# youssefg7/dl-sound-classification

Measured on AMD Instinct MI355X. Metric: training clips/sec (EnvNet-v2, ESC-50 shape), higher is better.
Workload: dtype bf16; 1 GPU; EnvNet-v2 train step (BC-mix, fwd, soft-CE, bwd, clip, Adam), ESC-50 shape; global_batch=256, per_gpu_batch=256, clip_samples=220500, parallelism=dp1, model=envnet_v2

## Files before the change

dl-sound-classification_amd/csrc/conv3w.hip:

```cpp
#include "common.h"

namespace {

typedef unsigned u32x4 __attribute__((ext_vector_type(4)));
typedef unsigned u32x2 __attribute__((ext_vector_type(2)));
typedef short s16x8 __attribute__((ext_vector_type(8)));

struct W3Args {
  const bf16* x;
  const bf16* dy;
  float* part;
  int n, h, wd, oh, ow, nseg;
  const bf16* ya;
  bf16* dyo;
  float* bpart;
  const float *gamma, *scale, *shift, *mean, *invstd, *dgamma, *dbeta;
  int64_t P;
};

__device__ __forceinline__ bf16x8 tr_frag(const char* p0, int stride) {
  const s16x4 lo = __builtin_amdgcn_ds_read_tr16_b64_v4i16((MIA_LDS s16x4*)(p0));
  const s16x4 hi = __builtin_amdgcn_ds_read_tr16_b64_v4i16((MIA_LDS s16x4*)(p0 + 4 * stride));
  const s16x8 c = {lo[0], lo[1], lo[2], lo[3], hi[0], hi[1], hi[2], hi[3]};
  return __builtin_bit_cast(bf16x8, c);
}

template <bool BN>
__global__ __launch_bounds__(256) void conv3_wgrad_kernel(W3Args g) {
  constexpr int ROWB = 80, CPYB = 704;
  __shared__ __attribute__((aligned(16))) char strip[4][4 * CPYB];
  __shared__ __attribute__((aligned(16))) char dyt[4][32 * 64];
  const int lane = threadIdx.x & 63, wv = threadIdx.x >> 6;
  const int gw = blockIdx.x * 4 + wv, nw = gridDim.x * 4;
  const int items = g.n * g.oh * g.nseg;
  char* sg = strip[wv];
  char* dt = dyt[wv];
  f32x16 acc[2];
#pragma unroll
  for (int i = 0; i < 16; ++i) { acc[0][i] = 0.f; acc[1][i] = 0.f; }

  struct Raw { u32x2 v[3]; u32x4 d[2]; u32x4 y[BN ? 2 : 1]; uint32_t ok; };
  __shared__ __attribute__((aligned(16))) float bnp[7][32];
  float bs1[8];
  if constexpr (BN) {
    if (threadIdx.x < 32) {
      const int c = threadIdx.x;
      const float invP = 1.f / (float)g.P;
      const float is = g.invstd[c];
      bnp[0][c] = g.scale[c];
      bnp[1][c] = g.shift[c];
      bnp[2][c] = (g.gamma ? g.gamma[c] : 1.f) * is;
      bnp[3][c] = g.mean[c];
      bnp[4][c] = is;
      bnp[5][c] = g.dbeta[c] * invP;
      bnp[6][c] = g.dgamma[c] * invP;
    }
#pragma unroll
    for (int i = 0; i < 8; ++i) bs1[i] = 0.f;
    __syncthreads();
  }
  auto load = [&](int it) __attribute__((always_inline)) {
    Raw R;
    it = it < items ? it : items - 1;
    const int seg = it % g.nseg, rest = it / g.nseg;
    const int oy = rest % g.oh, b = rest / g.oh;
    const int l = lane < 40 ? lane : lane - 40;
    const int r = l / 5, q = l % 5;
    const int col = seg * 32 + 8 * q;
    const bf16* src = g.x + ((int64_t)b * g.h + oy + r) * g.wd;
#pragma unroll
    for (int k = 0; k < 3; ++k) {
      const int c = col + 4 * k;
      R.v[k] = c + 4 <= g.wd ? *reinterpret_cast<const u32x2*>(src + c) : u32x2{0u, 0u};
    }
    const int64_t drow = ((int64_t)b * g.oh + oy) * g.ow * 32;
    R.ok = 0;
#pragma unroll
    for (int s = 0; s < 2; ++s) {
      const int qq = lane + 64 * s;
      const int px = seg * 32 + (qq >> 2);
      const int64_t off = drow + (int64_t)px * 32 + (qq & 3) * 8;
      R.d[s] = px < g.ow ? *reinterpret_cast<const u32x4*>(g.dy + off) : u32x4{0u, 0u, 0u, 0u};
      if constexpr (BN) R.y[s] = px < g.ow ? *reinterpret_cast<const u32x4*>(g.ya + off) : u32x4{0u, 0u, 0u, 0u};
      R.ok |= (uint32_t)(px < g.ow) << s;
    }
    (void)drow;
    return R;
  };
  const int i16 = lane & 15, gq = lane >> 4, h = lane >> 5;
  const int n = lane & 31;
  auto bn_chunk = [&](const Raw& R, int s, int it) __attribute__((always_inline)) -> u32x4 {
    if (!((R.ok >> s) & 1u)) return u32x4{0u, 0u, 0u, 0u};
    uint32_t o[4];
#pragma unroll
    for (int k = 0; k < 4; ++k) {
      const uint32_t dw = R.d[s][k], yw = R.y[s][k];
      float gv[2] = {__uint_as_float(dw << 16), __uint_as_float(dw & 0xffff0000u)};
      const float xv[2] = {__uint_as_float(yw << 16), __uint_as_float(yw & 0xffff0000u)};
#pragma unroll
      for (int j = 0; j < 2; ++j) {
        const int i = 2 * k + j, c = (lane & 3) * 8 + i;
        gv[j] = fmaf(xv[j], bnp[0][c], bnp[1][c]) > 0.f ? gv[j] : 0.f;
        gv[j] = bnp[2][c] * (gv[j] - bnp[5][c] - (xv[j] - bnp[3][c]) * bnp[4][c] * bnp[6][c]);
        bs1[i] += gv[j];
      }
      o[k] = pk_bf16(gv[0], gv[1]);
    }
    const int seg = it % g.nseg, rest = it / g.nseg;
    const int oy = rest % g.oh, b = rest / g.oh;
    const int qq = lane + 64 * s;
    const int px = seg * 32 + (qq >> 2);
    const u32x4 v = {o[0], o[1], o[2], o[3]};
    *reinterpret_cast<u32x4*>(g.dyo + (((int64_t)b * g.oh + oy) * g.ow + px) * 32 + (qq & 3) * 8) = v;
    return v;
  };
  auto run = [&](const Raw& R, int it) __attribute__((always_inline)) {
    u32x4 dv[2] = {R.d[0], R.d[1]};
    if constexpr (BN) {
      dv[0] = bn_chunk(R, 0, it);
      dv[1] = bn_chunk(R, 1, it);
    }
    wave_sync();
    if (lane < 40) {
      const int l = lane;
      const int r = l / 5, q = l % 5;
      const uint32_t d[6] = {R.v[0][0], R.v[0][1], R.v[1][0], R.v[1][1], R.v[2][0], R.v[2][1]};
#pragma unroll
      for (int c = 0; c < 4; ++c) {
        uint32_t o[4];
#pragma unroll
        for (int i = 0; i < 4; ++i) {
          const int e = c + 2 * i;
          o[i] = (e & 1) ? ((d[e >> 1] >> 16) | (d[(e >> 1) + 1] << 16)) : d[e >> 1];
        }
        *reinterpret_cast<u32x4*>(sg + c * CPYB + r * ROWB + 16 * q) = u32x4{o[0], o[1], o[2], o[3]};
      }
    }
#pragma unroll
    for (int s = 0; s < 2; ++s) {
      const int qq = lane + 64 * s;
      *reinterpret_cast<u32x4*>(dt + (qq >> 2) * 64 + (qq & 3) * 16) = dv[s];
    }
    wave_sync();
    const int kx = n & 7, cp = kx & 3;
#pragma unroll
    for (int ks = 0; ks < 2; ++ks) {
      const int kr = ks * 16 + 8 * (gq >> 1) + (i16 >> 2);
      const int c4 = 16 * (gq & 1) + 4 * (i16 & 3);
      const bf16x8 fa = tr_frag(dt + kr * 64 + c4 * 2, 64);
#pragma unroll
      for (int nt = 0; nt < 2; ++nt) {
        const int ky = 4 * nt + (n >> 3);
        const char* src = sg + cp * CPYB + ky * ROWB + 2 * (16 * ks + 8 * h + (kx & 4));
        const u32x2 p0 = *reinterpret_cast<const u32x2*>(src);
        const u32x2 p1 = *reinterpret_cast<const u32x2*>(src + 8);
        const u32x4 f = {p0[0], p0[1], p1[0], p1[1]};
        acc[nt] = __builtin_amdgcn_mfma_f32_32x32x16_bf16(fa, __builtin_bit_cast(bf16x8, f), acc[nt], 0, 0, 0);
      }
    }
  };

  int it = gw;
  if (it < items) {
    Raw ra = load(it), rb;
    for (;;) {
      rb = load(it + nw);
      run(ra, it);
      it += nw;
      if (it >= items) break;
      ra = load(it + nw);
      run(rb, it);
      it += nw;
      if (it >= items) break;
    }
  }
  float* dst = g.part + (int64_t)gw * 2048;
#pragma unroll
  for (int nt = 0; nt < 2; ++nt)
#pragma unroll
    for (int r = 0; r < 16; ++r) {
      const int co = (r & 3) + 8 * (r >> 2) + 4 * h;
      dst[co * 64 + nt * 32 + n] = acc[nt][r];
    }
  if constexpr (BN) {
#pragma unroll
    for (int i = 0; i < 8; ++i)
#pragma unroll
      for (int m = 4; m < 64; m <<= 1) bs1[i] += __shfl_xor(bs1[i], m, 64);
    if (lane < 4) {
#pragma unroll
      for (int i = 0; i < 8; ++i) g.bpart[(int64_t)gw * 32 + lane * 8 + i] = bs1[i];
    }
  }
}

__global__ void conv3_bias_final_kernel(const float* __restrict__ bpart, int nw, float* __restrict__ dbias) {
  const double s = block_sum_strided(bpart + blockIdx.x, nw, 32);
  if (threadIdx.x == 0) dbias[blockIdx.x] = (float)s;
}

constexpr int C3_G = 64;
__global__ __launch_bounds__(256) void conv3_wgrad_reduce1_kernel(const float* __restrict__ part, int nslab,
                                                                  double* __restrict__ tmp) {
  const int e = blockIdx.x * 256 + threadIdx.x, gi = blockIdx.y;
  const int per = (nslab + C3_G - 1) / C3_G;
  const int w0 = gi * per, w1 = min(nslab, w0 + per);
  double s = 0.0;
  for (int w = w0; w < w1; ++w) s += (double)part[(int64_t)w * 2048 + e];
  tmp[gi * 2048 + e] = s;
}
__global__ __launch_bounds__(256) void conv3_wgrad_reduce2_kernel(const double* __restrict__ tmp, float* __restrict__ dw) {
  const int e = blockIdx.x * 256 + threadIdx.x;
  double s = 0.0;
#pragma unroll 8
  for (int g = 0; g < C3_G; ++g) s += tmp[g * 2048 + e];
  dw[e] = (float)s;
}

}

extern "C" int mia_conv3_wgrad(const void* x, const void* dy, float* dw, float* part, int32_t nwaves, int32_t n,
                               int32_t h, int32_t wd, mia_stream_t stream) {
  MIA_CHECK_ARG(x && dy && dw && part && n > 0 && h >= 8 && wd >= 8, "conv3_wgrad: bad arguments");
  MIA_CHECK_ARG(nwaves > 0 && nwaves % 4 == 0, "conv3_wgrad: nwaves must be a positive multiple of 4");
  MIA_CHECK_ARG(wd % 4 == 0, "conv3_wgrad: image width must be a multiple of 4 (8-byte row alignment)");
  MIA_CHECK_ARG((reinterpret_cast<uintptr_t>(dy) & 15) == 0 && (reinterpret_cast<uintptr_t>(x) & 7) == 0,
                "conv3_wgrad: dy must be 16-byte and x 8-byte aligned");
  W3Args a{reinterpret_cast<const bf16*>(x), reinterpret_cast<const bf16*>(dy), part, n, h, wd, h - 7, wd - 7,
           (int)cdiv(wd - 7, 32)};
  MIA_CHECK_ARG((int64_t)n * a.oh * a.nseg < (1ll << 31), "conv3_wgrad: too many items");
  hipStream_t s = as_stream(stream);
  conv3_wgrad_kernel<false><<<nwaves / 4, 256, 0, s>>>(a);
  MIA_LAUNCH_CHECK("conv3_wgrad");
  double* tmp = reinterpret_cast<double*>(part + (int64_t)nwaves * 2048);
  conv3_wgrad_reduce1_kernel<<<dim3(8, C3_G), 256, 0, s>>>(part, nwaves, tmp);
  conv3_wgrad_reduce2_kernel<<<8, 256, 0, s>>>(tmp, dw);
  MIA_LAUNCH_CHECK("conv3_wgrad_reduce");
  return 0;
}

extern "C" int64_t mia_conv3_wgrad_workspace_bytes(int32_t nwaves) {
  return (int64_t)nwaves * 2048 * 4 + (int64_t)C3_G * 2048 * 8 + (int64_t)nwaves * 32 * 4;
}

extern "C" int mia_conv3_wgrad_bn(const void* x, const void* da, const void* ya, void* dy, float* dw, float* dbias,
                                  float* part, int32_t nwaves, int32_t n, int32_t h, int32_t wd, const float* gamma,
                                  const float* scale, const float* shift, const float* mean, const float* invstd,
                                  const float* dgamma, const float* dbeta, mia_stream_t stream) {
  MIA_CHECK_ARG(x && da && ya && dy && dw && dbias && part && n > 0 && h >= 8 && wd >= 8,
                "conv3_wgrad_bn: bad arguments");
  MIA_CHECK_ARG(scale && shift && mean && invstd && dgamma && dbeta, "conv3_wgrad_bn: null BN statistics");
  MIA_CHECK_ARG(nwaves > 0 && nwaves % 4 == 0, "conv3_wgrad_bn: nwaves must be a positive multiple of 4");
  MIA_CHECK_ARG(wd % 4 == 0, "conv3_wgrad_bn: image width must be a multiple of 4 (8-byte row alignment)");
  MIA_CHECK_ARG(((reinterpret_cast<uintptr_t>(da) | reinterpret_cast<uintptr_t>(ya) | reinterpret_cast<uintptr_t>(dy)) &
                 15) == 0 && (reinterpret_cast<uintptr_t>(x) & 7) == 0,
                "conv3_wgrad_bn: da / ya / dy must be 16-byte and x 8-byte aligned");
  W3Args a{reinterpret_cast<const bf16*>(x), reinterpret_cast<const bf16*>(da), part, n, h, wd, h - 7, wd - 7,
           (int)cdiv(wd - 7, 32), reinterpret_cast<const bf16*>(ya), reinterpret_cast<bf16*>(dy), nullptr,
           gamma, scale, shift, mean, invstd, dgamma, dbeta, (int64_t)n * (h - 7) * (wd - 7)};
  MIA_CHECK_ARG((int64_t)n * a.oh * a.nseg < (1ll << 31), "conv3_wgrad_bn: too many items");
  double* tmp = reinterpret_cast<double*>(part + (int64_t)nwaves * 2048);
  a.bpart = reinterpret_cast<float*>(tmp + (int64_t)C3_G * 2048);
  hipStream_t s = as_stream(stream);
  conv3_wgrad_kernel<true><<<nwaves / 4, 256, 0, s>>>(a);
  MIA_LAUNCH_CHECK("conv3_wgrad_bn");
  conv3_wgrad_reduce1_kernel<<<dim3(8, C3_G), 256, 0, s>>>(part, nwaves, tmp);
  conv3_wgrad_reduce2_kernel<<<8, 256, 0, s>>>(tmp, dw);
  conv3_bias_final_kernel<<<32, 256, 0, s>>>(a.bpart, nwaves, dbias);
  MIA_LAUNCH_CHECK("conv3_wgrad_bn reduce");
  return 0;
}
```

dl-sound-classification_amd/csrc/feconv.hip:

```cpp
#include "common.h"

#include <type_traits>

namespace {

constexpr int F1_DEPTH = 4;
constexpr int FE_NT = 256;
constexpr int FE_BM = 128;
constexpr int FE_N = 64;

typedef unsigned u32x4 __attribute__((ext_vector_type(4)));

template <int CIN, int KW, int S>
struct FeCfg {
  static constexpr int CG = CIN / 8;
  static constexpr int WPX = (FE_BM - 1) * S + KW;
  static constexpr int HALF = (WPX + 1) / 2;
  static constexpr int NSLOT = S == 1 ? WPX : 2 * HALF;
  static constexpr int PSB = CIN * 2 + 16;
  static constexpr int WBYTES = NSLOT * PSB;
  static constexpr int NCH = WPX * CG;
  static constexpr int LCH = (NCH + FE_NT - 1) / FE_NT;
  static constexpr int KS = KW * CIN / 16;
  static_assert(FE_NT % CG == 0, "channel chunk must be constant per thread");
// ... 624 lines not shown
      }
    const int seg = it % g.nseg, rest = it / g.nseg;
    const int oy = rest % g.oh, b = rest / g.oh;
    const int ox0 = seg * 32, ox = ox0 + o;
    char* stg = stage[wv];
#pragma unroll
    for (int h = 0; h < 2; ++h) {
      uint32_t w4[4];
#pragma unroll
      for (int i = 0; i < 4; ++i) {
        const int e = 8 * h + 2 * i;
        w4[i] = pk_bf16(v[e] + bv[e], v[e + 1] + bv[e + 1]);
        if constexpr (STATS) {
          if (ox < g.ow) {
            const float d0 = __uint_as_float(w4[i] << 16) - bv[e], d1 = __uint_as_float(w4[i] & 0xffff0000u) - bv[e + 1];
            s1[e] += d0; s2[e] = fmaf(d0, d0, s2[e]);
            s1[e + 1] += d1; s2[e + 1] = fmaf(d1, d1, s2[e + 1]);
          }
        }
      }
      const int k = (lane >> 5) + 2 * h;
      *reinterpret_cast<u32x4*>(stg + o * 64 + ((k ^ ((o >> 1) & 3)) << 4)) = u32x4{w4[0], w4[1], w4[2], w4[3]};
    }
    wave_sync();
    bf16* yrow = g.y + (((int64_t)b * g.oh + oy) * g.ow + ox0) * 32;
#pragma unroll
    for (int h = 0; h < 2; ++h) {
      const int r = 16 * h + (lane >> 2), k = lane & 3;
      const u32x4 q = *reinterpret_cast<const u32x4*>(stg + r * 64 + ((k ^ ((r >> 1) & 3)) << 4));
      if (ox0 + r < g.ow) __builtin_nontemporal_store(q, reinterpret_cast<u32x4*>(yrow + r * 32 + 8 * k));
    }
  };

  int it = gw;
  if (it < items) {
    Raw ra = load(it), rb;
    for (;;) {
      rb = load(it + nw);
      run(it, ra);
      it += nw;
      if (it >= items) break;
      ra = load(it + nw);
      run(it, rb);
      it += nw;
      if (it >= items) break;
    }
  }
  if constexpr (STATS) {
#pragma unroll
    for (int i = 0; i < 16; ++i) {
#pragma unroll
      for (int m = 1; m < 32; m <<= 1) {
        s1[i] += __shfl_xor(s1[i], m, 64);
        s2[i] += __shfl_xor(s2[i], m, 64);
      }
    }
    if ((lane & 31) == 0) {
      float* dst = g.part + (int64_t)gw * 64;
#pragma unroll
      for (int i = 0; i < 8; ++i) {
        dst[(c0 + i) * 2] = s1[i];
        dst[(c0 + i) * 2 + 1] = s2[i];
        dst[(c0 + 16 + i) * 2] = s1[8 + i];
        dst[(c0 + 16 + i) * 2 + 1] = s2[8 + i];
      }
    }
  }
}

constexpr int FW_NT = 512;
constexpr int FW_BP = 128;

struct FwArgs {
  const bf16* dy;
  const bf16* x;
  const float* ps;
  const float* pt;
  int n, win, wout, nitem;
  float* ws;
};

typedef short s16x8 __attribute__((ext_vector_type(8)));

__device__ __forceinline__ bf16x8 fw_tr(const char* p0, int stride) {
  const s16x4 lo = __builtin_amdgcn_ds_read_tr16_b64_v4i16((MIA_LDS s16x4*)(p0));
  const s16x4 hi = __builtin_amdgcn_ds_read_tr16_b64_v4i16((MIA_LDS s16x4*)(p0 + 4 * stride));
  const s16x8 c = {lo[0], lo[1], lo[2], lo[3], hi[0], hi[1], hi[2], hi[3]};
  return __builtin_bit_cast(bf16x8, c);
}

template <bool PRE>
__global__ __launch_bounds__(FW_NT) __attribute__((amdgpu_waves_per_eu(2, 2))) void fe_wgrad_kernel(FwArgs g) {
  constexpr int C = 32, KW = 16;
  constexpr int WPX = (FW_BP - 1) * 2 + KW;
  constexpr int HALF = (WPX + 1) / 2;
  constexpr int PSB = 64;
  constexpr int DSB = 192;
  constexpr int WBY = 2 * HALF * PSB;
  constexpr int DBY = FW_BP * DSB;
  constexpr int BUF = WBY + DBY;
  constexpr int WCH = WPX * 4;
  constexpr int WL = (WCH + FW_NT - 1) / FW_NT;
  constexpr int DL = FW_BP * 8 / FW_NT;
  __shared__ __attribute__((aligned(16))) char smem[2 * BUF];
  __shared__ __attribute__((aligned(16))) float spre[2][C];
  const int t = threadIdx.x, lane = t & 63, wave = t >> 6;
  const int items = g.n * g.nitem;
  if (PRE && t < C) {
    spre[0][t] = g.ps[t];
    spre[1][t] = g.pt[t];
  }
  const int cgw = t & 3;
  const __amdgpu_buffer_rsrc_t xr = __builtin_amdgcn_make_buffer_rsrc(
      const_cast<bf16*>(g.x), (short)0, (int)((int64_t)g.n * g.win * C * 2), 0x00020000);
  const __amdgpu_buffer_rsrc_t dr = __builtin_amdgcn_make_buffer_rsrc(
      const_cast<bf16*>(g.dy), (short)0, (int)((int64_t)g.n * g.wout * 64 * 2), 0x00020000);

  u32x4 wa[WL], wb[WL], da[DL], db[DL];
  auto load = [&](int it, u32x4 (&w)[WL], u32x4 (&d)[DL]) __attribute__((always_inline)) {
    it = it < items ? it : items - 1;
    const int b = it / g.nitem;
    const int o0 = (it - b * g.nitem) * FW_BP;
#pragma unroll
    for (int s = 0; s < WL; ++s) {
      const int q = t + FW_NT * s;
      const int p = q >> 2;
      const int ix = 2 * o0 + p;
      const bool ok = q < WCH && ix < g.win;
      const unsigned off = ok ? (unsigned)((b * g.win + ix) * 4 + cgw) * 16u : 0x80000000u;
      w[s] = __builtin_bit_cast(u32x4, __builtin_amdgcn_raw_buffer_load_b128(xr, off, 0, 0));
    }
#pragma unroll
    for (int s = 0; s < DL; ++s) {
      const int q = t + FW_NT * s;
      const int p = q >> 3, cc = q & 7;
      const bool ok = o0 + p < g.wout;
      const unsigned off = ok ? (unsigned)((b * g.wout + o0 + p) * 8 + cc) * 16u : 0x80000000u;
      d[s] = __builtin_bit_cast(u32x4, __builtin_amdgcn_raw_buffer_load_b128(dr, off, 0, 0));
    }
  };
  auto store = [&](int it, int buf, const u32x4 (&w)[WL], const u32x4 (&d)[DL]) __attribute__((always_inline)) {
    it = it < items ? it : items - 1;
    const int b = it / g.nitem;
    const int o0 = (it - b * g.nitem) * FW_BP;
    char* win = smem + buf * BUF;
    char* dyt = win + WBY;
    float sc[8], sh[8];
    if constexpr (PRE) {
#pragma unroll
      for (int h = 0; h < 2; ++h) {
        const f32x4 a = *reinterpret_cast<const f32x4*>(&spre[0][cgw * 8 + 4 * h]);
        const f32x4 c = *reinterpret_cast<const f32x4*>(&spre[1][cgw * 8 + 4 * h]);
#pragma unroll
        for (int q = 0; q < 4; ++q) { sc[4 * h + q] = a[q]; sh[4 * h + q] = c[q]; }
      }
    }
#pragma unroll
    for (int s = 0; s < WL; ++s) {
      const int q = t + FW_NT * s;
      const int p = q >> 2;
      if (q < WCH) {
        u32x4 v = w[s];
        if constexpr (PRE) {
          if (2 * o0 + p < g.win) {
            uint32_t w4[4];
#pragma unroll
            for (int i = 0; i < 4; ++i) {
              const float lo = fmaxf(fmaf(__uint_as_float(v[i] << 16), sc[2 * i], sh[2 * i]), 0.f);
              const float hi = fmaxf(fmaf(__uint_as_float(v[i] & 0xffff0000u), sc[2 * i + 1], sh[2 * i + 1]), 0.f);
              w4[i] = pk_bf16(lo, hi);
            }
            v = u32x4{w4[0], w4[1], w4[2], w4[3]};
          }
        }
        const int slot = (p & 1) * HALF + (p >> 1);
        *reinterpret_cast<u32x4*>(win + slot * PSB + cgw * 16) = v;
      }
    }
#pragma unroll
    for (int s = 0; s < DL; ++s) {
      const int q = t + FW_NT * s;
      *reinterpret_cast<u32x4*>(dyt + (q >> 3) * DSB + (q & 7) * 16) = d[s];
    }
  };

  f32x16 acc[2][2];
#pragma unroll
  for (int i = 0; i < 2; ++i)
#pragma unroll
    for (int j = 0; j < 2; ++j)
#pragma unroll
      for (int r = 0; r < 16; ++r) acc[i][j][r] = 0.f;

  const int i16 = lane & 15, gq = lane >> 4;
  auto compute = [&](int buf) __attribute__((always_inline)) {
    const char* win = smem + buf * BUF;
    const char* dyt = win + WBY;
    constexpr int KS = FW_BP / 16;
    auto frags = [&](int ks, bf16x8 (&fa)[2], bf16x8 (&fb)[2]) __attribute__((always_inline)) {
      const int kr = ks * 16 + 8 * (gq >> 1) + (i16 >> 2);
#pragma unroll
      for (int mt = 0; mt < 2; ++mt)
        fa[mt] = fw_tr(dyt + kr * DSB + (mt * 32 + 16 * (gq & 1) + 4 * (i16 & 3)) * 2, DSB);
#pragma unroll
      for (int j = 0; j < 2; ++j) {
        const int kx = 2 * wave + j;
        const int ci = 16 * (gq & 1) + 4 * (i16 & 3);
        const int slot = (kx & 1) * HALF + kr + (kx >> 1);
        fb[j] = fw_tr(win + slot * PSB + ci * 2, PSB);
      }
    };
    bf16x8 fa[2][2], fb[2][2];
    frags(0, fa[0], fb[0]);
#pragma unroll
    for (int ks = 0; ks < KS; ++ks) {
      const int c = ks & 1;
      if (ks + 1 < KS) frags(ks + 1, fa[c ^ 1], fb[c ^ 1]);
#pragma unroll
      for (int mt = 0; mt < 2; ++mt)
#pragma unroll
        for (int j = 0; j < 2; ++j)
          acc[mt][j] = __builtin_amdgcn_mfma_f32_32x32x16_bf16(fa[c][mt], fb[c][j], acc[mt][j], 0, 0, 0);
    }
    __builtin_amdgcn_sched_group_barrier(0x100, 8, 0);
#pragma unroll
    for (int ks = 0; ks < KS; ++ks) {
      if (ks + 1 < KS) {
#pragma unroll
        for (int q = 0; q < 4; ++q) {
          __builtin_amdgcn_sched_group_barrier(0x008, 1, 0);
          __builtin_amdgcn_sched_group_barrier(0x100, 2, 0);
        }
      } else {
        __builtin_amdgcn_sched_group_barrier(0x008, 4, 0);
      }
    }
  };

  const int G = gridDim.x;
  int item = blockIdx.x;
  if (item < items) {
    load(item, wa, da);
    load(item + G, wb, db);
    __syncthreads();
    store(item, 0, wa, da);
    __syncthreads();
    for (;;) {
      load(item + 2 * G, wa, da);
      compute(0);
      store(item + G, 1, wb, db);
      __builtin_amdgcn_s_waitcnt(0xC07F);
      __builtin_amdgcn_s_barrier();
      item += G;
      if (item >= items) break;
      load(item + 2 * G, wb, db);
      compute(1);
      store(item + G, 0, wa, da);
      __builtin_amdgcn_s_waitcnt(0xC07F);
      __builtin_amdgcn_s_barrier();
      item += G;
      if (item >= items) break;
    }
  }
  float* dst = g.ws + (int64_t)blockIdx.x * 64 * 512;
#pragma unroll
  for (int mt = 0; mt < 2; ++mt)
#pragma unroll
    for (int j = 0; j < 2; ++j) {
      const int n = (2 * wave + j) * 32 + (lane & 31);
#pragma unroll
      for (int r = 0; r < 16; ++r) {
        const int m = mt * 32 + (r & 3) + 8 * (r >> 2) + 4 * (lane >> 5);
        dst[(int64_t)m * 512 + n] = acc[mt][j][r];
      }
    }
}

int fe_grid(int items) {
  static int ncu = 0;
  if (!ncu) {
    int dev = 0;
    if (hipGetDevice(&dev) != hipSuccess || hipDeviceGetAttribute(&ncu, hipDeviceAttributeMultiprocessorCount, dev) != hipSuccess)
      ncu = 256;
  }
  return items < 2 * ncu ? items : 2 * ncu;
}

int fe_clips_per_launch(int64_t clip_bytes) { return (int)(((1ll << 31) - 1) / clip_bytes); }

int fe_grid1(int items) {
  const int two = fe_grid(1 << 30);
  return items < two / 2 ? items : two / 2;
}

__global__ __launch_bounds__(256) void fw_reduce_kernel(const float* __restrict__ ws, int slabs, int len,
                                                        float* __restrict__ out) {
  const int e = blockIdx.x * 256 + threadIdx.x;
  if (e >= len) return;
  float acc = 0.f;
  for (int k = 0; k < slabs; ++k) acc += ws[(int64_t)k * len + e];
  out[e] = acc;
}

bool aligned16(const void* p) { return (reinterpret_cast<uintptr_t>(p) & 15) == 0; }

bool fe_ws() { const char* e = getenv("MIA_FECONV_WS"); return !(e && e[0] == '0'); }

}

extern "C" int mia_fe_conv2_fwd(const void* y1, const float* scale, const float* shift, const void* w,
                                const float* bias, void* y2, int32_t n, int32_t w1, int32_t w2,
                                mia_stream_t stream) {
  MIA_CHECK_ARG(y1 && w && y2 && n > 0 && w1 >= 16, "fe_conv2_fwd: bad arguments");
  MIA_CHECK_ARG(!scale == !shift, "fe_conv2_fwd: scale and shift go together");
  MIA_CHECK_ARG(w2 == (w1 - 16) / 2 + 1, "fe_conv2_fwd: w2 must be (w1-16)/2+1 (got w1=%d w2=%d)", w1, w2);
  MIA_CHECK_ARG(aligned16(y1) && aligned16(w) && aligned16(y2), "fe_conv2_fwd: operands must be 16-byte aligned");
  hipStream_t s = as_stream(stream);
  const int per = fe_clips_per_launch((int64_t)w1 * 32 * 2);
  MIA_CHECK_ARG(per > 0, "fe_conv2_fwd: one clip exceeds 2 GB");
  for (int c = 0; c < n; c += per) {
    const int nc = n - c < per ? n - c : per;
    FeArgs a{reinterpret_cast<const bf16*>(y1) + (int64_t)c * w1 * 32, scale, shift, reinterpret_cast<const bf16*>(w),
             bias, reinterpret_cast<bf16*>(y2) + (int64_t)c * w2 * FE_N, nc, w1, w2, 0, (int)cdiv(w2, FE_BM),
             (int64_t)w2 * FE_N, (int64_t)w2 * FE_N};
    if (fe_ws()) {
      const int grid = fe_grid1(nc * a.nitem);
      if (scale) feconv_ws_kernel<32, 16, 2, true><<<grid, FS_NT, 0, s>>>(a);
      else feconv_ws_kernel<32, 16, 2, false><<<grid, FS_NT, 0, s>>>(a);
    } else {
      const int grid = fe_grid(nc * a.nitem);
      if (scale) feconv_kernel<32, 16, 2, true><<<grid, FE_NT, 0, s>>>(a);
      else feconv_kernel<32, 16, 2, false><<<grid, FE_NT, 0, s>>>(a);
    }
    MIA_LAUNCH_CHECK("fe_conv2_fwd");
  }
  return 0;
}

extern "C" int mia_fe_conv2_dgrad(const void* dy2, const void* wpar, void* da1, int32_t n, int32_t w1,
                                  int32_t w2, mia_stream_t stream) {
  MIA_CHECK_ARG(dy2 && wpar && da1 && n > 0 && w1 >= 16, "fe_conv2_dgrad: bad arguments");
  MIA_CHECK_ARG(w2 == (w1 - 16) / 2 + 1, "fe_conv2_dgrad: w2 must be (w1-16)/2+1 (got w1=%d w2=%d)", w1, w2);
  MIA_CHECK_ARG(aligned16(dy2) && aligned16(wpar) && aligned16(da1), "fe_conv2_dgrad: operands must be 16-byte aligned");
  MIA_CHECK_ARG(((int64_t)w1 * 32) % 8 == 0, "fe_conv2_dgrad: clip stride must keep 16-byte alignment");
  const int wout = (w1 + 1) / 2;
  const int per = fe_clips_per_launch((int64_t)w2 * 64 * 2);
  MIA_CHECK_ARG(per > 0, "fe_conv2_dgrad: one clip exceeds 2 GB");
  for (int c = 0; c < n; c += per) {
    const int nc = n - c < per ? n - c : per;
    FeArgs a{reinterpret_cast<const bf16*>(dy2) + (int64_t)c * w2 * 64, nullptr, nullptr,
             reinterpret_cast<const bf16*>(wpar), nullptr, reinterpret_cast<bf16*>(da1) + (int64_t)c * w1 * 32, nc,
             w2, wout, 7, (int)cdiv(wout, FE_BM), (int64_t)w1 * 32, (int64_t)w1 * 32};
#ifdef FS_DGRAD
    feconv_ws_kernel<64, 8, 1, false><<<fe_grid1(nc * a.nitem), FS_NT, 0, as_stream(stream)>>>(a);
#else
    feconv_kernel<64, 8, 1, false><<<fe_grid(nc * a.nitem), FE_NT, 0, as_stream(stream)>>>(a);
#endif
    MIA_LAUNCH_CHECK("fe_conv2_dgrad");
  }
  return 0;
}

extern "C" int mia_fe_conv2_wgrad(const void* dy2, const void* y1, const float* scale, const float* shift,
                                  float* dw, int32_t n, int32_t w1, int32_t w2, void* workspace, int64_t ws_bytes,
                                  mia_stream_t stream) {
  MIA_CHECK_ARG(dy2 && y1 && dw && workspace && n > 0 && w1 >= 16, "fe_conv2_wgrad: bad arguments");
  MIA_CHECK_ARG(!scale == !shift, "fe_conv2_wgrad: scale and shift go together");
  MIA_CHECK_ARG(w2 == (w1 - 16) / 2 + 1, "fe_conv2_wgrad: w2 must be (w1-16)/2+1 (got w1=%d w2=%d)", w1, w2);
  MIA_CHECK_ARG(aligned16(dy2) && aligned16(y1), "fe_conv2_wgrad: operands must be 16-byte aligned");
  hipStream_t s = as_stream(stream);
  const int per = fe_clips_per_launch((int64_t)w1 * 32 * 2);
  MIA_CHECK_ARG(per > 0, "fe_conv2_wgrad: one clip exceeds 2 GB");
  const int nitem = (int)cdiv(w2, FW_BP);
  int slabs = 0;
  for (int c = 0; c < n; c += per) slabs += fe_grid1(((n - c) < per ? (n - c) : per) * nitem);
  MIA_CHECK_ARG((int64_t)slabs * 64 * 512 * 4 <= ws_bytes, "fe_conv2_wgrad: workspace too small (%lld B needed)",
                (long long)slabs * 64 * 512 * 4);
  int slab0 = 0;
  for (int c = 0; c < n; c += per) {
    const int nc = n - c < per ? n - c : per;
    FwArgs a{reinterpret_cast<const bf16*>(dy2) + (int64_t)c * w2 * 64, reinterpret_cast<const bf16*>(y1) + (int64_t)c * w1 * 32,
             scale, shift, nc, w1, w2, nitem, reinterpret_cast<float*>(workspace) + (int64_t)slab0 * 64 * 512};
    const int grid = fe_grid1(nc * nitem);
    if (scale) fe_wgrad_kernel<true><<<grid, FW_NT, 0, s>>>(a);
    else fe_wgrad_kernel<false><<<grid, FW_NT, 0, s>>>(a);
    MIA_LAUNCH_CHECK("fe_conv2_wgrad");
    slab0 += grid;
  }
  fw_reduce_kernel<<<64 * 512 / 256, 256, 0, s>>>(reinterpret_cast<const float*>(workspace), slabs, 64 * 512, dw);
  MIA_LAUNCH_CHECK("fe_conv2_wgrad reduce");
  return 0;
}

extern "C" int mia_fe_conv1_fwd(const float* x, const void* w, const float* bias, void* y1, float* partial,
                                int32_t nwaves, int32_t n, int32_t t, mia_stream_t stream) {
  MIA_CHECK_ARG(x && w && bias && y1 && n > 0 && t >= 64 && t % 2 == 0, "fe_conv1_fwd: bad arguments");
  MIA_CHECK_ARG(nwaves > 0 && nwaves % 4 == 0, "fe_conv1_fwd: nwaves must be a positive multiple of 4");
  MIA_CHECK_ARG(aligned16(w) && aligned16(y1) && (reinterpret_cast<uintptr_t>(x) & 7) == 0,
                "fe_conv1_fwd: y1/w must be 16-byte and x 8-byte aligned");
  const int w1 = (t - 64) / 2 + 1;
  F1Args a{x, reinterpret_cast<const bf16*>(w), bias, reinterpret_cast<bf16*>(y1), partial, n, t, w1,
           (int)cdiv(w1, 32)};
  MIA_CHECK_ARG((int64_t)n * a.nitem < (1ll << 31), "fe_conv1_fwd: too many items");
  if (partial) fe_conv1_kernel<true><<<nwaves / 4, 256, 0, as_stream(stream)>>>(a);
  else fe_conv1_kernel<false><<<nwaves / 4, 256, 0, as_stream(stream)>>>(a);
  MIA_LAUNCH_CHECK("fe_conv1_fwd");
  return 0;
}

extern "C" int mia_fe_conv3_fwd(const void* x, const void* w, const float* bias, void* y, float* partial,
                                int32_t nwaves, int32_t n, int32_t h, int32_t wd, mia_stream_t stream) {
  MIA_CHECK_ARG(x && w && bias && y && n > 0 && h >= 8 && wd >= 8, "fe_conv3_fwd: bad arguments");
  MIA_CHECK_ARG(nwaves > 0 && nwaves % 4 == 0, "fe_conv3_fwd: nwaves must be a positive multiple of 4");
  MIA_CHECK_ARG(wd % 4 == 0, "fe_conv3_fwd: image width must be a multiple of 4 (8-byte row alignment)");
  MIA_CHECK_ARG(aligned16(w) && aligned16(y) && (reinterpret_cast<uintptr_t>(x) & 7) == 0,
                "fe_conv3_fwd: w/y must be 16-byte and x 8-byte aligned");
  F3Args a{reinterpret_cast<const bf16*>(x), reinterpret_cast<const bf16*>(w), bias, reinterpret_cast<bf16*>(y),
           partial, n, h, wd, h - 7, wd - 7, (int)cdiv(wd - 7, 32)};
  MIA_CHECK_ARG((int64_t)n * a.oh * a.nseg < (1ll << 31), "fe_conv3_fwd: too many items");
  if (partial) fe_conv3_kernel<true><<<nwaves / 4, 256, 0, as_stream(stream)>>>(a);
  else fe_conv3_kernel<false><<<nwaves / 4, 256, 0, as_stream(stream)>>>(a);
  MIA_LAUNCH_CHECK("fe_conv3_fwd");
  return 0;
}

#ifdef FE_STAMP
extern "C" int mia_fe_stamps_copy(void* dst, int64_t bytes) {
  return hipMemcpyFromSymbol(dst, HIP_SYMBOL(g_fe_st), (size_t)bytes, 0, hipMemcpyDeviceToHost) == hipSuccess ? 0 : -1;
}
#endif
```

dl-sound-classification_amd/csrc/mgemm.hip:

```cpp
#include "common.h"
#include "gemm_common.h"

namespace {

constexpr int MG_NT = 512;
constexpr int MG_BM = 256, MG_BN = 256, MG_BK = 64;
constexpr int MG_HALF = 16384;
constexpr int MG_STAGE = 4 * MG_HALF;
constexpr int MG_LDS = 2 * MG_STAGE;

enum { MG_KC = MIA_LAYOUT_KC, MG_RC = MIA_LAYOUT_RC };
enum { EPI_PLAIN = 0, EPI_GELU = 1, EPI_GELU_SAVE = 2, EPI_ADD_AUX = 3, EPI_DGELU = 4, EPI_SLAB = 5, EPI_GELU_SAVE_D = 6,
       EPI_DMUL = 7 };

typedef short s16x8 __attribute__((ext_vector_type(8)));
typedef __attribute__((address_space(3))) void* lds_vp;

struct MArgs {
  const bf16* a;
  const bf16* b;
  int64_t lda, ldb, M, N, K, kper;
  int nbm, nbn, split;
  void* out;
  int64_t ldc;
  int out_f32;
  const float* bias;
  const void* aux;
  int64_t ldaux;
  float* ws;
  float* colsum_part;
  float* acs_part;
  uint8_t* mxq;
  uint8_t* mxs;
  int64_t drop_w;
  int group_m;
};

typedef unsigned mg_u32x4 __attribute__((ext_vector_type(4)));
__device__ __forceinline__ void mg_st16(void* p, uint4 v) {
  __builtin_nontemporal_store(__builtin_bit_cast(mg_u32x4, v), reinterpret_cast<mg_u32x4*>(p));
}

__device__ __forceinline__ __amdgpu_buffer_rsrc_t rsrc_of(const void* base, int64_t bytes) {
  const uint32_t n = bytes <= 0 ? 0u : (bytes >= 0xFFFFFFFFll ? 0xFFFFFFFFu : (uint32_t)bytes);
  return __builtin_amdgcn_make_buffer_rsrc(const_cast<void*>(base), 0, (int)n, 0x00020000);
}

__device__ __forceinline__ int rc_swz(int k) { return (k & 3) | (((k >> 3) & 1) << 2); }

template <int L>
struct Loader {
  __amdgpu_buffer_rsrc_t rsrc;
  uint32_t voff[4];
  uint32_t kstep;
  __device__ __forceinline__ void init(const bf16* p, int64_t ld, int64_t rows, int64_t r0, int64_t kbeg,
                                       int64_t kend, int wave, int lane) {
    if constexpr (L == MG_KC) {
      const bf16* base = p + r0 * ld + kbeg;
      const int64_t nrows = rows - r0 < 256 ? rows - r0 : 256;
      rsrc = rsrc_of(base, ((nrows - 1) * ld + (kend - kbeg)) * 2);
#pragma unroll
      for (int i = 0; i < 4; ++i) {
        const int hh = i >> 1, j = 2 * wave + (i & 1);
        const int r = hh * 128 + 8 * j + (lane >> 3);
        const int c = (lane & 7) ^ (r & 7);
        voff[i] = (uint32_t)(((int64_t)r * ld + c * 8) * 2);
      }
      kstep = 128;
    } else {
      const bf16* base = p + kbeg * ld + r0;
      const int64_t ncols = rows - r0 < 256 ? rows - r0 : 256;
      rsrc = rsrc_of(base, ((kend - kbeg - 1) * ld + ncols) * 2);
#pragma unroll
      for (int i = 0; i < 4; ++i) {
        const int hh = i >> 1, j = 2 * wave + (i & 1);
        const int k = 4 * j + (lane >> 4);
        const int s = lane & 15;
        const int c = (s >> 1) ^ rc_swz(k);
        voff[i] = (uint32_t)(((int64_t)k * ld + hh * 128 + c * 16 + (s & 1) * 8) * 2);
      }
      kstep = (uint32_t)(64 * ld * 2);
    }
  }
  __device__ __forceinline__ void issue(char* tile, int kt, int wave) const {
#pragma unroll
    for (int i = 0; i < 4; ++i)
      __builtin_amdgcn_raw_ptr_buffer_load_lds(rsrc, (lds_vp)(tile + (i >> 1) * MG_HALF + (2 * wave + (i & 1)) * 1024),
                                               16, voff[i], kt * kstep, 0, 0);
  }
};

template <int L>
__device__ __forceinline__ bf16x8 frag(const char* half, int r0, int ks, int lane) {
  if constexpr (L == MG_KC) {
    const int r = r0 + (lane & 15);
    const int c = 4 * ks + (lane >> 4);
    return *reinterpret_cast<const bf16x8*>(half + r * 128 + ((c ^ (r & 7)) << 4));
  } else {
    const int i = lane & 15, g = lane >> 4;
    const int k = 32 * ks + 8 * g + (i >> 2);
    const int ch = r0 >> 4;
    const char* p0 = half + k * 256 + ((ch ^ rc_swz(k)) << 5) + (i & 3) * 8;
    const char* p1 = half + (k + 4) * 256 + ((ch ^ rc_swz(k + 4)) << 5) + (i & 3) * 8;
    const s16x4 lo = __builtin_amdgcn_ds_read_tr16_b64_v4i16((MIA_LDS s16x4*)(p0));
    const s16x4 hi = __builtin_amdgcn_ds_read_tr16_b64_v4i16((MIA_LDS s16x4*)(p1));
    const s16x8 cc = {lo[0], lo[1], lo[2], lo[3], hi[0], hi[1], hi[2], hi[3]};
    return __builtin_bit_cast(bf16x8, cc);
  }
}

__device__ __forceinline__ f32x4 mfma_t(bf16x8 a, bf16x8 b, f32x4 c) {
  return __builtin_amdgcn_mfma_f32_16x16x32_bf16(b, a, c, 0, 0, 0);
}

__device__ __forceinline__ float gelu_cdf(float x) {
  const float z = fabsf(x) * 0.70710678118654752f;
  const float t = __builtin_amdgcn_rcpf(fmaf(0.5f, z, 1.f));
  float p = 0.17087277f;
  p = fmaf(p, t, -0.82215223f);
  p = fmaf(p, t, 1.48851587f);
  p = fmaf(p, t, -1.13520398f);
  p = fmaf(p, t, 0.27886807f);
  p = fmaf(p, t, -0.18628806f);
  p = fmaf(p, t, 0.09678418f);
  p = fmaf(p, t, 0.37409196f);
  p = fmaf(p, t, 1.00002368f);
  p = fmaf(p, t, -1.26551223f);
  const float half_erfc = 0.5f * t * __expf(fmaf(-z, z, p));
  return x >= 0.f ? 1.f - half_erfc : half_erfc;
}
__device__ __forceinline__ float gelu_f(float x) { return x * gelu_cdf(x); }
__device__ __forceinline__ float gelu_grad_f(float x) {
  return fmaf(x * 0.39894228040143268f, __expf(-0.5f * x * x), gelu_cdf(x));
}

typedef float f2 __attribute__((ext_vector_type(2)));
__device__ __forceinline__ f2 pfma(f2 a, f2 b, f2 c) { return __builtin_elementwise_fma(a, b, c); }
constexpr float L2E = 1.4426950408889634f;
__device__ __forceinline__ f2 gelu_cdf2(f2 x, f2& zz) {
  const f2 z = __builtin_elementwise_abs(x) * 0.70710678118654752f;
  const f2 d = pfma(z, f2{0.5f, 0.5f}, f2{1.f, 1.f});
  const f2 t = {__builtin_amdgcn_rcpf(d.x), __builtin_amdgcn_rcpf(d.y)};
  f2 p = f2{0.17087277f * L2E, 0.17087277f * L2E};
  p = pfma(p, t, f2{-0.82215223f * L2E, -0.82215223f * L2E});
  p = pfma(p, t, f2{1.48851587f * L2E, 1.48851587f * L2E});
  p = pfma(p, t, f2{-1.13520398f * L2E, -1.13520398f * L2E});
  p = pfma(p, t, f2{0.27886807f * L2E, 0.27886807f * L2E});
  p = pfma(p, t, f2{-0.18628806f * L2E, -0.18628806f * L2E});
  p = pfma(p, t, f2{0.09678418f * L2E, 0.09678418f * L2E});
  p = pfma(p, t, f2{0.37409196f * L2E, 0.37409196f * L2E});
  p = pfma(p, t, f2{1.00002368f * L2E, 1.00002368f * L2E});
  p = pfma(p, t, f2{-1.26551223f * L2E, -1.26551223f * L2E});
  zz = z * z;
  const f2 a = pfma(-zz, f2{L2E, L2E}, p);
  const f2 he = t * f2{0.5f * __builtin_amdgcn_exp2f(a.x), 0.5f * __builtin_amdgcn_exp2f(a.y)};
  return f2{x.x >= 0.f ? 1.f - he.x : he.x, x.y >= 0.f ? 1.f - he.y : he.y};
}
__device__ __forceinline__ f2 gelu2(f2 x) {
  f2 zz;
  return x * gelu_cdf2(x, zz);
}
__device__ __forceinline__ f2 gelu_grad2(f2 x) {
  const f2 z = __builtin_elementwise_abs(x) * 0.70710678118654752f;
  const f2 d = pfma(z, f2{0.3275911f, 0.3275911f}, f2{1.f, 1.f});
  const f2 t = {__builtin_amdgcn_rcpf(d.x), __builtin_amdgcn_rcpf(d.y)};
  f2 p = f2{0.5f * 1.061405429f, 0.5f * 1.061405429f};
  p = pfma(p, t, f2{0.5f * -1.453152027f, 0.5f * -1.453152027f});
  p = pfma(p, t, f2{0.5f * 1.421413741f, 0.5f * 1.421413741f});
  p = pfma(p, t, f2{0.5f * -0.284496736f, 0.5f * -0.284496736f});
  p = pfma(p, t, f2{0.5f * 0.254829592f, 0.5f * 0.254829592f});
  const f2 a = -(z * z) * L2E;
  const f2 e = {__builtin_amdgcn_exp2f(a.x), __builtin_amdgcn_exp2f(a.y)};
  const f2 he = p * t * e;
  const f2 c = {x.x >= 0.f ? 1.f - he.x : he.x, x.y >= 0.f ? 1.f - he.y : he.y};
  return pfma(x * 0.39894228040143268f, e, c);
}
__device__ __forceinline__ f2 gelu_and_grad2(f2 x, f2& d) {
  const f2 z = __builtin_elementwise_abs(x) * 0.70710678118654752f;
  const f2 dd = pfma(z, f2{0.3275911f, 0.3275911f}, f2{1.f, 1.f});
  const f2 t = {__builtin_amdgcn_rcpf(dd.x), __builtin_amdgcn_rcpf(dd.y)};
  f2 p = f2{0.5f * 1.061405429f, 0.5f * 1.061405429f};
  p = pfma(p, t, f2{0.5f * -1.453152027f, 0.5f * -1.453152027f});
  p = pfma(p, t, f2{0.5f * 1.421413741f, 0.5f * 1.421413741f});
  p = pfma(p, t, f2{0.5f * -0.284496736f, 0.5f * -0.284496736f});
  p = pfma(p, t, f2{0.5f * 0.254829592f, 0.5f * 0.254829592f});
  const f2 a = -(z * z) * L2E;
  const f2 e = {__builtin_amdgcn_exp2f(a.x), __builtin_amdgcn_exp2f(a.y)};
  const f2 he = p * t * e;
  const f2 c = {x.x >= 0.f ? 1.f - he.x : he.x, x.y >= 0.f ? 1.f - he.y : he.y};
  d = pfma(x * 0.39894228040143268f, e, c);
  return x * c;
}
__device__ __forceinline__ void gelu4(f32x4& v) {
  const f2 a = gelu2(f2{v[0], v[1]}), b = gelu2(f2{v[2], v[3]});
  v = f32x4{a.x, a.y, b.x, b.y};
}
__device__ __forceinline__ void gelu_d4(f32x4& v, f32x4& d) {
  f2 da, db;
  const f2 a = gelu_and_grad2(f2{v[0], v[1]}, da), b = gelu_and_grad2(f2{v[2], v[3]}, db);
  v = f32x4{a.x, a.y, b.x, b.y};
  d = f32x4{da.x, da.y, db.x, db.y};
}
__device__ __forceinline__ void dgelu4(f32x4& v, f32x4 u) {
  const f2 a = gelu_grad2(f2{u[0], u[1]}), b = gelu_grad2(f2{u[2], u[3]});
  v = f32x4{v[0] * a.x, v[1] * a.y, v[2] * b.x, v[3] * b.y};
}

__device__ __forceinline__ uint2 pack4(f32x4 v) {
  return make_uint2(pk_bf16(v[0], v[1]), pk_bf16(v[2], v[3]));
}
__device__ __forceinline__ f32x4 unpack4(uint2 u) {
  return f32x4{__uint_as_float(u.x << 16), __uint_as_float(u.x & 0xffff0000u), __uint_as_float(u.y << 16),
               __uint_as_float(u.y & 0xffff0000u)};
}

template <int EPI>
__device__ __forceinline__ void mg_epilogue(const MArgs& g, f32x4 (&acc)[8][4], char* smem, int wave, int lane,
                                            int bm, int z, int64_t m0, int64_t n0) {
  const int wr = wave >> 2, wc = wave & 3;
  f32x4 bias4[4];
#pragma unroll
  for (int j = 0; j < 4; ++j) {
    const int64_t n = n0 + wc * 64 + 16 * j + 4 * (lane >> 4);
    if (EPI != EPI_SLAB && EPI != EPI_DGELU && EPI != EPI_DMUL && g.bias && n < g.N)
      bias4[j] = *reinterpret_cast<const f32x4*>(g.bias + n);
    else
      bias4[j] = f32x4{0.f, 0.f, 0.f, 0.f};
  }
  constexpr bool DG = EPI == EPI_DGELU || EPI == EPI_DMUL;
  const bool bf_out = EPI == EPI_GELU || EPI == EPI_GELU_SAVE || EPI == EPI_GELU_SAVE_D || DG ||
                      (EPI == EPI_PLAIN && !g.out_f32);
  if (!bf_out) {
    f32x4 ax[8][4];
    auto ld_row = [&](int i) __attribute__((always_inline)) {
      const int64_t m = m0 + wr * 128 + 16 * i + (lane & 15);
#pragma unroll
      for (int j = 0; j < 4; ++j) {
        const int64_t n = n0 + wc * 64 + 16 * j + 4 * (lane >> 4);
        ax[i][j] = (m < g.M && n < g.N)
                       ? *reinterpret_cast<const f32x4*>(reinterpret_cast<const float*>(g.aux) + m * g.ldaux + n)
                       : f32x4{0.f, 0.f, 0.f, 0.f};
      }
    };
    if constexpr (EPI == EPI_ADD_AUX) {
      ld_row(0);
      ld_row(1);
    }
#pragma unroll
    for (int i = 0; i < 8; ++i) {
      if constexpr (EPI == EPI_ADD_AUX) {
        if (i + 2 < 8) ld_row(i + 2);
      }
      const int64_t m = m0 + wr * 128 + 16 * i + (lane & 15);
      if (m >= g.M) continue;
#pragma unroll
      for (int j = 0; j < 4; ++j) {
        const int64_t n = n0 + wc * 64 + 16 * j + 4 * (lane >> 4);
        if (n >= g.N) continue;
        f32x4 v = acc[i][j] + bias4[j];
        if constexpr (EPI == EPI_ADD_AUX) v += ax[i][j];
        float* dst = EPI == EPI_SLAB ? g.ws + ((int64_t)z * g.M + m) * g.N + n
                                     : reinterpret_cast<float*>(g.out) + m * g.ldc + n;
        *reinterpret_cast<f32x4*>(dst) = v;
      }
    }
    return;
  }
  if constexpr (EPI != EPI_SLAB && EPI != EPI_ADD_AUX) {
    __syncthreads();
    char* img = smem + wave * 16384;
    uint4 ua[16];
    if constexpr (DG) {
#pragma unroll
      for (int it = 0; it < 16; ++it) {
        const int r = 8 * it + (lane >> 3);
        const int64_t m = m0 + wr * 128 + r, n = n0 + wc * 64 + 8 * (lane & 7);
        ua[it] = (m < g.M && n < g.N)
                     ? __builtin_bit_cast(uint4, __builtin_nontemporal_load(reinterpret_cast<const mg_u32x4*>(
                           reinterpret_cast<const bf16*>(g.aux) + m * g.ldaux + n)))
                     : make_uint4(0, 0, 0, 0);
      }
    }
#pragma unroll
    for (int i = 0; i < 8; ++i)
#pragma unroll
      for (int j = 0; j < 4; ++j) {
        const int r = 16 * i + (lane & 15), g4 = lane >> 4;
        const int c = 2 * j + (g4 >> 1);
        *reinterpret_cast<uint2*>(img + r * 128 + ((c ^ (r & 7) ^ ((r >> 3) & 1)) << 4) + (g4 & 1) * 8) =
            pack4(acc[i][j] + bias4[j]);
      }
    asm volatile("s_waitcnt lgkmcnt(0)" ::: "memory");
    __builtin_amdgcn_sched_barrier(0);
    float cs[8];
#pragma unroll
    for (int c = 0; c < 8; ++c) cs[c] = 0.f;
    const int cc = lane & 7;
#pragma unroll
    for (int it = 0; it < 16; ++it) {
      const int r = 8 * it + (lane >> 3);
      const uint4 q = *reinterpret_cast<const uint4*>(img + r * 128 + ((cc ^ (r & 7) ^ ((r >> 3) & 1)) << 4));
      const int64_t m = m0 + wr * 128 + r, n = n0 + wc * 64 + 8 * cc;
// ... 167 lines not shown
    }
    if constexpr (ACS) {
#pragma unroll
      for (int ks = 0; ks < 2; ++ks) {
        acs0 = frag_sum(frag<LA>(ah, 16 * wc, ks, lane), acs0);
        acs1 = frag_sum(frag<LA>(ah, 64 + 16 * wc, ks, lane), acs1);
      }
    }
    if (t + 1 < nk) {
      la.issue((t & 1) ? st0 : st1, t + 1, wave);
      asm volatile("s_waitcnt vmcnt(4) lgkmcnt(0)" ::: "memory");
    } else {
      asm volatile("s_waitcnt vmcnt(0) lgkmcnt(0)" ::: "memory");
    }
    __builtin_amdgcn_sched_barrier(0);
    __builtin_amdgcn_s_barrier();
    __builtin_amdgcn_sched_barrier(0);
    __builtin_amdgcn_s_setprio(1);
#pragma unroll
    for (int ks = 0; ks < 2; ++ks)
#pragma unroll
      for (int i = 0; i < 4; ++i)
#pragma unroll
        for (int j = 0; j < 4; ++j) acc[i][j] = mfma_t(af[ks][i], bfr[ks][j], acc[i][j]);
    __builtin_amdgcn_s_setprio(0);
    __builtin_amdgcn_sched_barrier(0);
    __builtin_amdgcn_s_barrier();
    __builtin_amdgcn_sched_barrier(0);
#pragma unroll
    for (int ks = 0; ks < 2; ++ks)
#pragma unroll
      for (int i = 0; i < 4; ++i) af[ks][i] = frag<LA>(ah, 64 + 16 * i, ks, lane);
    if (t + 2 < nk) {
      lb.issue(const_cast<char*>(cur) + 2 * MG_HALF, t + 2, wave);
      asm volatile("s_waitcnt vmcnt(4) lgkmcnt(0)" ::: "memory");
    } else {
      asm volatile("s_waitcnt vmcnt(0) lgkmcnt(0)" ::: "memory");
    }
    __builtin_amdgcn_sched_barrier(0);
    __builtin_amdgcn_s_barrier();
    __builtin_amdgcn_sched_barrier(0);
    __builtin_amdgcn_s_setprio(1);
#pragma unroll
    for (int ks = 0; ks < 2; ++ks)
#pragma unroll
      for (int i = 0; i < 4; ++i)
#pragma unroll
        for (int j = 0; j < 4; ++j) acc[4 + i][j] = mfma_t(af[ks][i], bfr[ks][j], acc[4 + i][j]);
    __builtin_amdgcn_s_setprio(0);
    __builtin_amdgcn_sched_barrier(0);
    __builtin_amdgcn_s_barrier();
    __builtin_amdgcn_sched_barrier(0);
  }
  if (wr == 0) __builtin_amdgcn_s_barrier();
  if constexpr (ACS) {
    acs0 += __shfl_xor(acs0, 16, 64);
    acs0 += __shfl_xor(acs0, 32, 64);
    acs1 += __shfl_xor(acs1, 16, 64);
    acs1 += __shfl_xor(acs1, 32, 64);
    if (bn == 0 && lane < 16) {
      const int64_t m = m0 + wr * 128 + 16 * wc + lane;
      if (m < g.M) g.acs_part[(int64_t)z * g.M + m] = acs0;
      if (m + 64 < g.M) g.acs_part[(int64_t)z * g.M + m + 64] = acs1;
    }
  }
  mg_epilogue<EPI>(g, acc, smem, wave, lane, bm, z, m0, n0);
}

template __global__ void mgemm_kernel<0, 0, 0>(MArgs);
template __global__ void mgemm_kernel<0, 0, 1>(MArgs);
template __global__ void mgemm_kernel<0, 0, 2>(MArgs);
template __global__ void mgemm_kernel<0, 0, 3>(MArgs);
template __global__ void mgemm_kernel<0, 0, 4>(MArgs);
template __global__ void mgemm_kernel<0, 0, 5>(MArgs);
template __global__ void mgemm_kernel<0, 1, 0>(MArgs);
template __global__ void mgemm_kernel<0, 1, 1>(MArgs);
template __global__ void mgemm_kernel<0, 1, 2>(MArgs);
template __global__ void mgemm_kernel<0, 1, 3>(MArgs);
template __global__ void mgemm_kernel<0, 1, 4>(MArgs);
template __global__ void mgemm_kernel<0, 1, 5>(MArgs);
template __global__ void mgemm_kernel<1, 0, 0>(MArgs);
template __global__ void mgemm_kernel<1, 0, 1>(MArgs);
template __global__ void mgemm_kernel<1, 0, 2>(MArgs);
template __global__ void mgemm_kernel<1, 0, 3>(MArgs);
template __global__ void mgemm_kernel<1, 0, 4>(MArgs);
template __global__ void mgemm_kernel<1, 0, 5>(MArgs);
template __global__ void mgemm_kernel<1, 1, 0>(MArgs);
template __global__ void mgemm_kernel<1, 1, 1>(MArgs);
template __global__ void mgemm_kernel<1, 1, 2>(MArgs);
template __global__ void mgemm_kernel<1, 1, 3>(MArgs);
template __global__ void mgemm_kernel<1, 1, 4>(MArgs);
template __global__ void mgemm_kernel<1, 1, 5>(MArgs);
template __global__ void mgemm_kernel<1, 1, 5, true>(MArgs);
template __global__ void mgemm_kernel<1, 0, 5, true>(MArgs);
template __global__ void mgemm_kernel<1, 1, 0, true>(MArgs);
template __global__ void mgemm_kernel<1, 0, 0, true>(MArgs);

typedef int i32x8 __attribute__((ext_vector_type(8)));
typedef int i32x4v __attribute__((ext_vector_type(4)));
constexpr int MX_SC = MG_LDS;

struct MxArgs {
  const uint8_t* sa;
  const uint8_t* sb;
};

__device__ __forceinline__ i32x8 mx_frag(const char* half, int r0, int lane) {
  const int r = r0 + (lane & 15), g = lane >> 4;
  const i32x4v lo = *reinterpret_cast<const i32x4v*>(half + r * 128 + ((g ^ (r & 7)) << 4));
  const i32x4v hi = *reinterpret_cast<const i32x4v*>(half + r * 128 + (((4 + g) ^ (r & 7)) << 4));
  return i32x8{lo[0], lo[1], lo[2], lo[3], hi[0], hi[1], hi[2], hi[3]};
}
__device__ __forceinline__ int mx_scale(const char* sbuf, int r0, int lane) {
  return *reinterpret_cast<const uint8_t*>(sbuf + (r0 + (lane & 15)) * 4 + (lane >> 4));
}

template <int EPI>
__global__ __launch_bounds__(MG_NT, 2) void mxgemm_kernel(MArgs g, MxArgs x) {
  __shared__ __attribute__((aligned(1024))) char smem[MG_LDS + 4096];
  const int lane = threadIdx.x & 63;
  const int wave = __builtin_amdgcn_readfirstlane(threadIdx.x >> 6);
  const int wr = wave >> 2, wc = wave & 3;
  const int nwg = (int)gridDim.x;
  const int orig = blockIdx.x;
  const int xcd = orig & 7, q8 = nwg >> 3, r8 = nwg & 7;
  const int lid = (xcd < r8 ? xcd * (q8 + 1) : r8 * (q8 + 1) + (xcd - r8) * q8) + (orig >> 3);
  int bm, bn;
  mg_tile_of(g, lid, bm, bn);
  const int64_t m0 = (int64_t)bm * MG_BM, n0 = (int64_t)bn * MG_BN;
  const int nk = (int)(g.K >> 7);
  Loader<MG_KC> la, lb;
  la.init(g.a, g.lda, g.M, m0, 0, g.K >> 1, wave, lane);
  lb.init(g.b, g.ldb, g.N, n0, 0, g.K >> 1, wave, lane);
  const int64_t kb32 = g.K >> 5;
  const int srow = 64 * (wave & 3) + lane;
  const uint8_t* sbase = wr == 0 ? x.sa + m0 * kb32 : x.sb + n0 * kb32;
  const int64_t srows = wr == 0 ? g.M - m0 : g.N - n0;
  const __amdgpu_buffer_rsrc_t srsrc = rsrc_of(sbase, (srows < 256 ? srows : 256) * kb32);
  const uint32_t svoff = (uint32_t)(srow * kb32);
  char* const sdst0 = smem + MX_SC + wr * 1024 + (wave & 3) * 256;
  auto sissue = [&](int kt) __attribute__((always_inline)) {
    __builtin_amdgcn_raw_ptr_buffer_load_lds(srsrc, (lds_vp)(sdst0 + (kt & 1) * 2048), 4, svoff, kt * 4, 0, 0);
  };

  f32x4 acc[8][4];
#pragma unroll
  for (int i = 0; i < 8; ++i)
#pragma unroll
    for (int j = 0; j < 4; ++j) acc[i][j] = f32x4{0.f, 0.f, 0.f, 0.f};

  char* const st0 = smem;
  char* const st1 = smem + MG_STAGE;
  if (nk > 0) {
    la.issue(st0, 0, wave);
    sissue(0);
    lb.issue(st0 + 2 * MG_HALF, 0, wave);
  }
  if (nk > 1) {
    lb.issue(st1 + 2 * MG_HALF, 1, wave);
    asm volatile("s_waitcnt vmcnt(4)" ::: "memory");
  } else {
    asm volatile("s_waitcnt vmcnt(0)" ::: "memory");
  }
  __builtin_amdgcn_s_barrier();
  if (wr == 1) __builtin_amdgcn_s_barrier();
  __builtin_amdgcn_sched_barrier(0);

  const int bhalf = wc >> 1;
  const int bcol = 64 * (wc & 1);
  i32x8 af[4], bfr[4];
  int sa[4], sb[4];
  for (int t = 0; t < nk; ++t) {
    const char* cur = (t & 1) ? st1 : st0;
    const char* ah = cur + wr * MG_HALF;
    const char* bh = cur + (2 + bhalf) * MG_HALF;
    const char* scur = smem + MX_SC + (t & 1) * 2048;
#pragma unroll
    for (int i = 0; i < 4; ++i) { af[i] = mx_frag(ah, 16 * i, lane); sa[i] = mx_scale(scur, 128 * wr + 16 * i, lane); }
#pragma unroll
    for (int j = 0; j < 4; ++j) {
      bfr[j] = mx_frag(bh, bcol + 16 * j, lane);
      sb[j] = mx_scale(scur + 1024, 128 * bhalf + bcol + 16 * j, lane);
    }
    if (t + 1 < nk) {
      la.issue((t & 1) ? st0 : st1, t + 1, wave);
      sissue(t + 1);
      asm volatile("s_waitcnt vmcnt(5) lgkmcnt(0)" ::: "memory");
    } else {
      asm volatile("s_waitcnt vmcnt(0) lgkmcnt(0)" ::: "memory");
    }
    __builtin_amdgcn_sched_barrier(0);
    __builtin_amdgcn_s_barrier();
    __builtin_amdgcn_sched_barrier(0);
    __builtin_amdgcn_s_setprio(1);
#pragma unroll
    for (int i = 0; i < 4; ++i)
#pragma unroll
      for (int j = 0; j < 4; ++j)
        acc[i][j] = __builtin_amdgcn_mfma_scale_f32_16x16x128_f8f6f4(bfr[j], af[i], acc[i][j], 0, 0, 0, sb[j], 0, sa[i]);
    __builtin_amdgcn_s_setprio(0);
    __builtin_amdgcn_sched_barrier(0);
    __builtin_amdgcn_s_barrier();
    __builtin_amdgcn_sched_barrier(0);
#pragma unroll
    for (int i = 0; i < 4; ++i) {
      af[i] = mx_frag(ah, 64 + 16 * i, lane);
      sa[i] = mx_scale(scur, 128 * wr + 64 + 16 * i, lane);
    }
    if (t + 2 < nk) {
      lb.issue(const_cast<char*>(cur) + 2 * MG_HALF, t + 2, wave);
      asm volatile("s_waitcnt vmcnt(4) lgkmcnt(0)" ::: "memory");
    } else {
      asm volatile("s_waitcnt vmcnt(0) lgkmcnt(0)" ::: "memory");
    }
    __builtin_amdgcn_sched_barrier(0);
    __builtin_amdgcn_s_barrier();
    __builtin_amdgcn_sched_barrier(0);
    __builtin_amdgcn_s_setprio(1);
#pragma unroll
    for (int i = 0; i < 4; ++i)
#pragma unroll
      for (int j = 0; j < 4; ++j)
        acc[4 + i][j] =
            __builtin_amdgcn_mfma_scale_f32_16x16x128_f8f6f4(bfr[j], af[i], acc[4 + i][j], 0, 0, 0, sb[j], 0, sa[i]);
    __builtin_amdgcn_s_setprio(0);
    __builtin_amdgcn_sched_barrier(0);
    __builtin_amdgcn_s_barrier();
    __builtin_amdgcn_sched_barrier(0);
  }
  if (wr == 0) __builtin_amdgcn_s_barrier();
  mg_epilogue<EPI>(g, acc, smem, wave, lane, bm, 0, m0, n0);
}
template __global__ void mxgemm_kernel<0>(MArgs, MxArgs);
template __global__ void mxgemm_kernel<1>(MArgs, MxArgs);
template __global__ void mxgemm_kernel<2>(MArgs, MxArgs);
template __global__ void mxgemm_kernel<3>(MArgs, MxArgs);
template __global__ void mxgemm_kernel<7>(MArgs, MxArgs);

template <typename T>
__global__ __launch_bounds__(256) void mx_quant_kernel(const T* __restrict__ x, int64_t rows, int64_t cols, int64_t ldx,
                                                       uint8_t* __restrict__ q, int64_t ldq, uint8_t* __restrict__ sc) {
  const int64_t per_row = cols >> 3;
  const int64_t total = rows * per_row;
  for (int64_t i = (int64_t)blockIdx.x * 256 + threadIdx.x; i < total; i += (int64_t)gridDim.x * 256) {
    const int64_t r = i / per_row, c = (i - r * per_row) * 8;
    float v[8];
    if constexpr (sizeof(T) == 2) {
      const uint4 u = *reinterpret_cast<const uint4*>(x + r * ldx + c);
      const uint32_t w[4] = {u.x, u.y, u.z, u.w};
#pragma unroll
      for (int k = 0; k < 4; ++k) { v[2 * k] = __uint_as_float(w[k] << 16); v[2 * k + 1] = __uint_as_float(w[k] & 0xffff0000u); }
    } else {
      const float4 a = *reinterpret_cast<const float4*>(x + r * ldx + c);
      const float4 b = *reinterpret_cast<const float4*>(x + r * ldx + c + 4);
      v[0] = a.x; v[1] = a.y; v[2] = a.z; v[3] = a.w; v[4] = b.x; v[5] = b.y; v[6] = b.z; v[7] = b.w;
    }
    const int e = mx_exponent_4lanes(v);
    *reinterpret_cast<uint2*>(q + r * ldq + c) = mx_pack8(v, e);
    if ((c & 31) == 0) sc[r * (cols >> 5) + (c >> 5)] = (uint8_t)(e + 127);
  }
}

template <typename T>
__global__ __launch_bounds__(256) void mx_quant_t_kernel(const T* __restrict__ x, int64_t rows, int64_t cols,
                                                         int64_t ldx, uint8_t* __restrict__ q, int64_t ldq,
                                                         uint8_t* __restrict__ sc) {
  const int64_t nb = rows >> 5;
  const int64_t total = nb * cols;
  for (int64_t i = (int64_t)blockIdx.x * 256 + threadIdx.x; i < total; i += (int64_t)gridDim.x * 256) {
    const int64_t blk = i / cols, c = i - blk * cols;
    float v[32];
    float am = 0.f;
#pragma unroll
    for (int k = 0; k < 32; ++k) {
      v[k] = (float)x[(blk * 32 + k) * ldx + c];
      am = fmaxf(am, fabsf(v[k]));
    }
    const int e = mx_exponent(am);
    uint2* dst = reinterpret_cast<uint2*>(q + c * ldq + blk * 32);
#pragma unroll
    for (int k = 0; k < 4; ++k) dst[k] = mx_pack8(v + 8 * k, e);
    sc[c * nb + blk] = (uint8_t)(e + 127);
  }
}

__global__ __launch_bounds__(256) void mg_splitk_reduce_kernel(const float* __restrict__ ws, int split, int64_t M,
                                                               int64_t N, void* out, int64_t ldc, int out_f32,
                                                               const float* __restrict__ bias) {
  const int64_t n4 = N >> 2;
  const int64_t total = M * n4;
  for (int64_t i = (int64_t)blockIdx.x * 256 + threadIdx.x; i < total; i += (int64_t)gridDim.x * 256) {
    const int64_t m = i / n4, n = (i - m * n4) * 4;
    f32x4 s = *reinterpret_cast<const f32x4*>(ws + m * N + n);
    for (int zz = 1; zz < split; ++zz) s += *reinterpret_cast<const f32x4*>(ws + ((int64_t)zz * M + m) * N + n);
    if (bias) {
#pragma unroll
      for (int c = 0; c < 4; ++c) s[c] += bias[n + c];
    }
    if (out_f32) *reinterpret_cast<f32x4*>(reinterpret_cast<float*>(out) + m * ldc + n) = s;
    else *reinterpret_cast<uint2*>(reinterpret_cast<bf16*>(out) + m * ldc + n) = pack4(s);
  }
}

__global__ __launch_bounds__(256) void mg_acs_reduce_kernel(const float* __restrict__ part, int split, int64_t M,
                                                            float* __restrict__ out) {
  const int64_t m = (int64_t)blockIdx.x * 256 + threadIdx.x;
  if (m >= M) return;
  float acc = 0.f;
  for (int z = 0; z < split; ++z) acc += part[(int64_t)z * M + m];
  out[m] = acc;
}

__global__ __launch_bounds__(256) void mg_colsum_final_kernel(const double* __restrict__ part2, int N, float* out) {
  const int c = blockIdx.x * 256 + threadIdx.x;
  if (c < N) out[c] = (float)colsum_slices(part2, N, c);
}

template <int LA, int LB>
hipError_t launch_epi(const MArgs& a, int epi, hipStream_t s) {
  const unsigned grid = (unsigned)((int64_t)a.nbm * a.nbn * a.split);
  if constexpr (LA == MG_RC) {
    if (a.acs_part) {
      if (epi == EPI_SLAB) mgemm_kernel<LA, LB, EPI_SLAB, true><<<grid, MG_NT, 0, s>>>(a);
      else mgemm_kernel<LA, LB, EPI_PLAIN, true><<<grid, MG_NT, 0, s>>>(a);
      return hipGetLastError();
    }
  }
  switch (epi) {
    case EPI_PLAIN: mgemm_kernel<LA, LB, EPI_PLAIN><<<grid, MG_NT, 0, s>>>(a); break;
    case EPI_GELU: mgemm_kernel<LA, LB, EPI_GELU><<<grid, MG_NT, 0, s>>>(a); break;
    case EPI_GELU_SAVE: mgemm_kernel<LA, LB, EPI_GELU_SAVE><<<grid, MG_NT, 0, s>>>(a); break;
    case EPI_ADD_AUX: mgemm_kernel<LA, LB, EPI_ADD_AUX><<<grid, MG_NT, 0, s>>>(a); break;
    case EPI_DGELU: mgemm_kernel<LA, LB, EPI_DGELU><<<grid, MG_NT, 0, s>>>(a); break;
    case EPI_GELU_SAVE_D: mgemm_kernel<LA, LB, EPI_GELU_SAVE_D><<<grid, MG_NT, 0, s>>>(a); break;
    case EPI_DMUL: mgemm_kernel<LA, LB, EPI_DMUL><<<grid, MG_NT, 0, s>>>(a); break;
    default: mgemm_kernel<LA, LB, EPI_SLAB><<<grid, MG_NT, 0, s>>>(a); break;
  }
  return hipGetLastError();
}

bool aligned16(const void* p) { return (reinterpret_cast<uintptr_t>(p) & 15) == 0; }

}

namespace mgemm {

int mg_group_m(int nbm, int nbn, int split, int lb) {
  return split == 1 && lb == MIA_LAYOUT_RC && nbn >= 9 && nbm >= 16 ? 8 : 0;
}

int mg_epi_kind(const MiaEpilogue& E, int64_t N) {
  const bool drop = E.rm_inner && E.rm_offset == MIA_RM_DROP && E.rm_istride == 1 && E.rm_outer == E.rm_inner - 1 &&
                    E.act == MIA_ACT_NONE && E.dtype == MIA_BF16 && !E.mx_q && !E.colsum;
  if (E.accumulate || (E.rm_inner && !drop) || E.sqsum || E.alpha != 1.f || !E.ptr) return -1;
  if (E.mx_q && (!E.mx_scales || E.dtype != MIA_BF16 || E.ldc != N || N % 32 ||
                 (E.colsum && E.act != MIA_DACT_MUL) ||
                 !(E.act == MIA_ACT_NONE || E.act == MIA_ACT_GELU || E.act == MIA_ACT_GELU_SAVE ||
                   E.act == MIA_ACT_GELU_SAVE_D || E.act == MIA_DACT_MUL)))
    return -1;
  const bool bf = E.dtype == MIA_BF16, f32 = E.dtype == MIA_F32;
  if ((E.ldc & 3) || E.ldc < N || (reinterpret_cast<uintptr_t>(E.ptr) & (bf ? 7 : 15)) != 0) return -1;
  if (bf && N % 8) return -1;
  if (E.bias && (reinterpret_cast<uintptr_t>(E.bias) & 15)) return -1;
  const bool aux_ok = E.aux && aligned16(E.aux) && (E.ldaux & 3) == 0 && E.ldaux >= N;
  switch (E.act) {
    case MIA_ACT_NONE: return (bf || f32) && !E.colsum ? EPI_PLAIN : -1;
    case MIA_ACT_GELU: return bf && !E.colsum ? EPI_GELU : -1;
    case MIA_ACT_GELU_SAVE: return bf && aux_ok && E.aux_dtype == MIA_BF16 && !E.colsum ? EPI_GELU_SAVE : -1;
    case MIA_ACT_ADD_AUX: return f32 && aux_ok && E.aux_dtype == MIA_F32 && !E.colsum ? EPI_ADD_AUX : -1;
    case MIA_DACT_GELU: return bf && aux_ok && E.aux_dtype == MIA_BF16 && !E.bias ? EPI_DGELU : -1;
    case MIA_ACT_GELU_SAVE_D: return bf && aux_ok && E.aux_dtype == MIA_BF16 && !E.colsum ? EPI_GELU_SAVE_D : -1;
    case MIA_DACT_MUL: return bf && aux_ok && E.aux_dtype == MIA_BF16 && !E.bias ? EPI_DMUL : -1;
    default: return -1;
  }
}

bool mg_ok(const MiaOperand& A, const MiaOperand& B, const MiaEpilogue& E, int64_t M, int64_t N, int64_t K,
           int compute) {
  if (compute != MIA_BF16 || M < 256 || N < 256 || N % 4 || K < 64) return false;
  if (cdiv(M, MG_BM) * cdiv(N, MG_BN) < 32 && K < 16384) return false;
  if (A.kind != MIA_OP_DENSE || B.kind != MIA_OP_DENSE || A.dtype != MIA_BF16 || B.dtype != MIA_BF16) return false;
  if (A.pre != MIA_PRE_NONE || B.pre != MIA_PRE_NONE || A.ld % 8 || B.ld % 8 || !aligned16(A.ptr) || !aligned16(B.ptr))
    return false;
  if (A.layout == MIA_LAYOUT_KC) { if (A.rows != M || A.cols < K || K % MG_BK) return false; }
  else if (A.rows < K || A.cols != M || M % 8) return false;
  if (B.layout == MIA_LAYOUT_KC) { if (B.rows != N || B.cols < K || K % MG_BK) return false; }
  else if (B.rows < K || B.cols != N || N % 8) return false;
  if (cdiv(M, MG_BM) * cdiv(N, MG_BN) >= (1ll << 24)) return false;
  if (E.a_colsum && (A.layout != MIA_LAYOUT_RC || mg_epi_kind(E, N) != EPI_PLAIN)) return false;
  return mg_epi_kind(E, N) >= 0;
}

int mg_split(int64_t M, int64_t N, int64_t K) {
  const int64_t tiles = cdiv(M, MG_BM) * cdiv(N, MG_BN);
  if (tiles >= 512 || K < 4096) return 1;
  int64_t s = 256 / tiles;
  const int64_t smax = K / 1024;
  if (s > smax) s = smax;
  return (int)(s < 1 ? 1 : s);
}

static void mg_geometry(int64_t M, int64_t N, int64_t K, int& split, int64_t& kper) {
  split = mg_split(M, N, K);
  kper = cdiv(cdiv(K, split), 64) * 64;
  split = (int)cdiv(K, kper);
}

int64_t mg_workspace_bytes(int64_t M, int64_t N, int64_t K, int colsum, int a_colsum) {
  int split;
  int64_t kper;
  mg_geometry(M, N, K, split, kper);
  int64_t b = split > 1 ? (int64_t)split * M * N * 4 : 0;
  b = cdiv(b, 256) * 256;
  if (colsum) b += cdiv(cdiv(M, MG_BM) * N * 4, 256) * 256 + colsum_part2_bytes((int)N);
  if (a_colsum) b += cdiv((int64_t)split * M * 4, 256) * 256;
  return b;
}

int mg_run(const MiaOperand& A, const MiaOperand& B, const MiaEpilogue& E, int64_t M, int64_t N, int64_t K,
           void* workspace, hipStream_t s) {
  const int epi = mg_epi_kind(E, N);
  MArgs a;
  memset(&a, 0, sizeof(a));
  a.a = reinterpret_cast<const bf16*>(A.ptr);
  a.b = reinterpret_cast<const bf16*>(B.ptr);
  a.lda = A.ld; a.ldb = B.ld; a.M = M; a.N = N; a.K = K;
  mg_geometry(M, N, K, a.split, a.kper);
  a.nbm = (int)cdiv(M, MG_BM); a.nbn = (int)cdiv(N, MG_BN);
  a.group_m = mg_group_m(a.nbm, a.nbn, a.split, B.layout);
  a.out = E.ptr; a.ldc = E.ldc; a.out_f32 = E.dtype == MIA_F32;
  a.drop_w = E.rm_inner && E.rm_offset == MIA_RM_DROP ? E.rm_inner : 0;
  a.bias = E.bias; a.aux = E.aux; a.ldaux = E.ldaux;
  a.mxq = reinterpret_cast<uint8_t*>(E.mx_q); a.mxs = reinterpret_cast<uint8_t*>(E.mx_scales);
  const int need_ws = a.split > 1 || E.colsum || E.a_colsum;
  MIA_CHECK_ARG(!need_ws || workspace, "gemm: the 256x128 path needs the workspace of mia_gemm_workspace_bytes_ex");
  char* ws = reinterpret_cast<char*>(workspace);
  int kind = epi;
  if (a.split > 1) {
    MIA_CHECK_ARG(epi == EPI_PLAIN && !E.colsum, "gemm: split-K weight gradients take a plain epilogue");
    a.ws = reinterpret_cast<float*>(ws);
    a.bias = nullptr;
    kind = EPI_SLAB;
    ws += cdiv((int64_t)a.split * M * N * 4, 256) * 256;
  }
  if (E.colsum) {
    a.colsum_part = reinterpret_cast<float*>(ws);
    ws += cdiv((int64_t)a.nbm * N * 4, 256) * 256;
  }
  if (E.a_colsum) a.acs_part = reinterpret_cast<float*>(ws);
  hipError_t err;
  const int la = A.layout, lb = B.layout;
  if (la == MIA_LAYOUT_KC && lb == MIA_LAYOUT_KC) err = launch_epi<MG_KC, MG_KC>(a, kind, s);
  else if (la == MIA_LAYOUT_KC) err = launch_epi<MG_KC, MG_RC>(a, kind, s);
  else if (lb == MIA_LAYOUT_RC) err = launch_epi<MG_RC, MG_RC>(a, kind, s);
  else err = launch_epi<MG_RC, MG_KC>(a, kind, s);
  if (err != hipSuccess) return mia::fail(-(int)err, "mgemm launch: %s", hipGetErrorString(err));
  if (a.split > 1) {
    const int64_t total = M * (N / 4);
    const int blocks = (int)std::min<int64_t>(cdiv(total, 256), 4096);
    mg_splitk_reduce_kernel<<<blocks, 256, 0, s>>>(a.ws, a.split, M, N, E.ptr, E.ldc, E.dtype == MIA_F32, E.bias);
    MIA_LAUNCH_CHECK("mgemm splitk reduce");
  }
  if (E.a_colsum) {
    mg_acs_reduce_kernel<<<(unsigned)cdiv(M, 256), 256, 0, s>>>(a.acs_part, a.split, M, E.a_colsum);
    MIA_LAUNCH_CHECK("mgemm a_colsum");
  }
  if (E.colsum && (kind == EPI_DGELU || kind == EPI_DMUL)) {
    double* part2 = reinterpret_cast<double*>(ws);
    colsum_pass1(a.colsum_part, a.nbm, (int)N, N, part2, s);
    mg_colsum_final_kernel<<<(unsigned)cdiv(N, 256), 256, 0, s>>>(part2, (int)N, E.colsum);
    MIA_LAUNCH_CHECK("mgemm colsum");
  }
  return 0;
}

}

extern "C" int mia_mx_quantize(const void* x, int32_t x_dtype, int64_t rows, int64_t cols, int64_t ldx, void* q,
                               int64_t ldq, void* scales, mia_stream_t stream) {
  MIA_CHECK_ARG(x_dtype == MIA_BF16 || x_dtype == MIA_F32, "mx_quantize: input must be bf16 or f32");
  MIA_CHECK_ARG(rows >= 0 && cols >= 0 && cols % 32 == 0, "mx_quantize: cols must be a multiple of 32");
  MIA_CHECK_ARG(ldx >= cols && ldq >= cols && ldq % 8 == 0 && ldx % 8 == 0, "mx_quantize: bad leading dimension");
  MIA_CHECK_ARG((reinterpret_cast<uintptr_t>(x) & 15) == 0 && (reinterpret_cast<uintptr_t>(q) & 7) == 0,
                "mx_quantize: x must be 16-B and q 8-B aligned");
  if (rows == 0 || cols == 0) return 0;
  const int64_t total = rows * (cols / 8);
  const unsigned blocks = (unsigned)std::min<int64_t>(cdiv(total, 256), 16384);
  hipStream_t s = as_stream(stream);
  if (x_dtype == MIA_BF16)
    mx_quant_kernel<bf16><<<blocks, 256, 0, s>>>(reinterpret_cast<const bf16*>(x), rows, cols, ldx,
                                                 reinterpret_cast<uint8_t*>(q), ldq, reinterpret_cast<uint8_t*>(scales));
  else
    mx_quant_kernel<float><<<blocks, 256, 0, s>>>(reinterpret_cast<const float*>(x), rows, cols, ldx,
                                                  reinterpret_cast<uint8_t*>(q), ldq, reinterpret_cast<uint8_t*>(scales));
  MIA_LAUNCH_CHECK("mx_quantize");
  return 0;
}

extern "C" int mia_mx_quantize_t(const void* x, int32_t x_dtype, int64_t rows, int64_t cols, int64_t ldx, void* q,
                                 int64_t ldq, void* scales, mia_stream_t stream) {
  MIA_CHECK_ARG(x_dtype == MIA_BF16 || x_dtype == MIA_F32, "mx_quantize_t: input must be bf16 or f32");
  MIA_CHECK_ARG(rows >= 0 && cols >= 0 && rows % 32 == 0, "mx_quantize_t: rows must be a multiple of 32");
  MIA_CHECK_ARG(ldx >= cols && ldq >= rows && ldq % 8 == 0, "mx_quantize_t: bad leading dimension");
  MIA_CHECK_ARG((reinterpret_cast<uintptr_t>(q) & 7) == 0, "mx_quantize_t: q must be 8-B aligned");
  if (rows == 0 || cols == 0) return 0;
  const int64_t total = (rows / 32) * cols;
  const unsigned blocks = (unsigned)std::min<int64_t>(cdiv(total, 256), 16384);
  hipStream_t s = as_stream(stream);
  if (x_dtype == MIA_BF16)
    mx_quant_t_kernel<bf16><<<blocks, 256, 0, s>>>(reinterpret_cast<const bf16*>(x), rows, cols, ldx,
                                                   reinterpret_cast<uint8_t*>(q), ldq, reinterpret_cast<uint8_t*>(scales));
  else
    mx_quant_t_kernel<float><<<blocks, 256, 0, s>>>(reinterpret_cast<const float*>(x), rows, cols, ldx,
                                                    reinterpret_cast<uint8_t*>(q), ldq, reinterpret_cast<uint8_t*>(scales));
  MIA_LAUNCH_CHECK("mx_quantize_t");
  return 0;
}

extern "C" int64_t mia_gemm_mxfp8_workspace_bytes(int64_t M, int64_t N, int32_t colsum) {
  return colsum ? cdiv(cdiv(M, MG_BM) * N * 4, 256) * 256 + colsum_part2_bytes((int)N) : 0;
}

extern "C" int mia_gemm_mxfp8(const void* a, const void* a_scales, int64_t lda, const void* b, const void* b_scales,
                              int64_t ldb, const MiaEpilogue* E, int64_t M, int64_t N, int64_t K, mia_stream_t stream) {
  return mia_gemm_mxfp8_ex(a, a_scales, lda, b, b_scales, ldb, E, M, N, K, nullptr, stream);
}

extern "C" int mia_gemm_mxfp8_ex(const void* a, const void* a_scales, int64_t lda, const void* b, const void* b_scales,
                                 int64_t ldb, const MiaEpilogue* E, int64_t M, int64_t N, int64_t K, void* workspace,
                                 mia_stream_t stream) {
  MIA_CHECK_ARG(a && b && a_scales && b_scales && E && E->ptr, "gemm_mxfp8: null operand");
  MIA_CHECK_ARG(M > 0 && N > 0 && K > 0 && K % 128 == 0, "gemm_mxfp8: K must be a positive multiple of 128");
  MIA_CHECK_ARG(lda >= K && ldb >= K && lda % 16 == 0 && ldb % 16 == 0, "gemm_mxfp8: lda / ldb (bytes) must be >= K and 16-B multiples");
  MIA_CHECK_ARG((reinterpret_cast<uintptr_t>(a) & 15) == 0 && (reinterpret_cast<uintptr_t>(b) & 15) == 0 &&
                    (reinterpret_cast<uintptr_t>(a_scales) & 3) == 0 && (reinterpret_cast<uintptr_t>(b_scales) & 3) == 0,
                "gemm_mxfp8: operands 16-B and scales 4-B aligned");
  MIA_CHECK_ARG(N % 4 == 0 && (E->dtype != MIA_BF16 || N % 8 == 0) && cdiv(M, MG_BM) * cdiv(N, MG_BN) < (1ll << 24),
                "gemm_mxfp8: N must be a multiple of 4 (of 8 for a bf16 output)");
  const int epi = mgemm::mg_epi_kind(*E, N);
  MIA_CHECK_ARG(epi == EPI_PLAIN || epi == EPI_GELU || epi == EPI_GELU_SAVE || epi == EPI_GELU_SAVE_D || epi == EPI_ADD_AUX ||
                    epi == EPI_DMUL,
                "gemm_mxfp8: epilogue must be plain / bias / GELU / GELU_SAVE(_D) / f32 residual / x saved gelu' "
                "(row-major, aligned)");
  MIA_CHECK_ARG(!E->colsum || (epi == EPI_DMUL && workspace),
                "gemm_mxfp8: column sums ride the x-gelu' epilogue and need mia_gemm_mxfp8_workspace_bytes");
  MArgs g;
  memset(&g, 0, sizeof(g));
  g.a = reinterpret_cast<const bf16*>(a);
  g.b = reinterpret_cast<const bf16*>(b);
  g.lda = lda / 2; g.ldb = ldb / 2;
  g.M = M; g.N = N; g.K = K; g.kper = K; g.split = 1;
  g.nbm = (int)cdiv(M, MG_BM); g.nbn = (int)cdiv(N, MG_BN);
  g.group_m = 0;
  g.out = E->ptr; g.ldc = E->ldc; g.out_f32 = E->dtype == MIA_F32;
  g.bias = E->bias; g.aux = E->aux; g.ldaux = E->ldaux;
  g.mxq = reinterpret_cast<uint8_t*>(E->mx_q); g.mxs = reinterpret_cast<uint8_t*>(E->mx_scales);
  MxArgs x{reinterpret_cast<const uint8_t*>(a_scales), reinterpret_cast<const uint8_t*>(b_scales)};
  const unsigned grid = (unsigned)((int64_t)g.nbm * g.nbn);
  hipStream_t s = as_stream(stream);
  if (E->colsum) g.colsum_part = reinterpret_cast<float*>(workspace);
  switch (epi) {
    case EPI_PLAIN: mxgemm_kernel<EPI_PLAIN><<<grid, MG_NT, 0, s>>>(g, x); break;
    case EPI_GELU: mxgemm_kernel<EPI_GELU><<<grid, MG_NT, 0, s>>>(g, x); break;
    case EPI_GELU_SAVE: mxgemm_kernel<EPI_GELU_SAVE><<<grid, MG_NT, 0, s>>>(g, x); break;
    case EPI_GELU_SAVE_D: mxgemm_kernel<EPI_GELU_SAVE_D><<<grid, MG_NT, 0, s>>>(g, x); break;
    case EPI_DMUL: mxgemm_kernel<EPI_DMUL><<<grid, MG_NT, 0, s>>>(g, x); break;
    default: mxgemm_kernel<EPI_ADD_AUX><<<grid, MG_NT, 0, s>>>(g, x); break;
  }
  MIA_LAUNCH_CHECK("gemm_mxfp8");
  if (E->colsum) {
    double* part2 = reinterpret_cast<double*>(reinterpret_cast<char*>(workspace) + cdiv((int64_t)g.nbm * N * 4, 256) * 256);
    colsum_pass1(g.colsum_part, g.nbm, (int)N, N, part2, s);
    mg_colsum_final_kernel<<<(unsigned)cdiv(N, 256), 256, 0, s>>>(part2, (int)N, E->colsum);
    MIA_LAUNCH_CHECK("gemm_mxfp8 colsum");
  }
  return 0;
}
```

dl-sound-classification_amd/csrc/misc.hip:

```cpp
#include "common.h"

namespace {

constexpr int NT = 256;

__global__ void pack_weight_kernel(const float* __restrict__ src, void* dst, int dtype, int cout, int cin, int kh,
                                   int kw, int mode) {
  const int64_t total = (int64_t)cout * cin * kh * kw;
  for (int64_t i = (int64_t)blockIdx.x * blockDim.x + threadIdx.x; i < total; i += (int64_t)gridDim.x * blockDim.x) {
    if (mode == 0) {
      const int ci = (int)(i % cin); int64_t q = i / cin;
      const int kx = (int)(q % kw); q /= kw;
      const int ky = (int)(q % kh); const int co = (int)(q / kh);
      st_elem(dst, dtype, i, src[(((int64_t)co * cin + ci) * kh + ky) * kw + kx]);
    } else if (mode == 1) {
      const int co = (int)(i % cout); int64_t q = i / cout;
      const int kx = (int)(q % kw); q /= kw;
      const int ky = (int)(q % kh); const int ci = (int)(q / kh);
      st_elem(dst, dtype, i, src[(((int64_t)co * cin + ci) * kh + (kh - 1 - ky)) * kw + (kw - 1 - kx)]);
    } else if (mode == 2) {
      const int half = kw / 2;
      const int co = (int)(i % cout); int64_t q = i / cout;
      const int j = (int)(q % half); q /= half;
      const int ci = (int)(q % cin); const int p = (int)(q / cin);
      st_elem(dst, dtype, i, src[((int64_t)co * cin + ci) * kw + 2 * (half - 1 - j) + p]);
    } else if (mode == 3) {
      const int co = (int)(i % cout); int64_t q = i / cout;
      const int j = (int)(q % kw); const int ky = (int)(q / kw);
      st_elem(dst, dtype, i, src[((int64_t)co * kh + ky) * kw + (kw - 1 - j)]);
    } else {
      const int kx = (int)(i % kw); int64_t q = i / kw;
      const int ky = (int)(q % kh); q /= kh;
      const int ci = (int)(q % cin); const int co = (int)(q / cin);
      st_elem(dst, dtype, i, src[(((int64_t)co * kh + ky) * kw + kx) * cin + ci]);
    }
  }
}

struct PackBatch {
  MiaPackJob job[MIA_PACK_BATCH];
  int64_t begin[MIA_PACK_BATCH + 1];
  int n;
};
__global__ void pack_weight_batch_kernel(PackBatch b) {
  const int64_t total = b.begin[b.n];
  for (int64_t i = (int64_t)blockIdx.x * blockDim.x + threadIdx.x; i < total; i += (int64_t)gridDim.x * blockDim.x) {
    int j = 0;
    while (j + 1 < b.n && i >= b.begin[j + 1]) ++j;
    const MiaPackJob& J = b.job[j];
    const int64_t e = i - b.begin[j];
    const int cout = J.cout, cin = J.cin, kh = J.kh, kw = J.kw;
    const float* src = J.src;
    float v;
    if (J.mode == 0) {
      const int ci = (int)(e % cin); int64_t q = e / cin;
      const int kx = (int)(q % kw); q /= kw;
      const int ky = (int)(q % kh); const int co = (int)(q / kh);
      v = src[(((int64_t)co * cin + ci) * kh + ky) * kw + kx];
    } else if (J.mode == 1) {
      const int co = (int)(e % cout); int64_t q = e / cout;
      const int kx = (int)(q % kw); q /= kw;
      const int ky = (int)(q % kh); const int ci = (int)(q / kh);
      v = src[(((int64_t)co * cin + ci) * kh + (kh - 1 - ky)) * kw + (kw - 1 - kx)];
    } else if (J.mode == 2) {
      const int half = kw / 2;
      const int co = (int)(e % cout); int64_t q = e / cout;
      const int jj = (int)(q % half); q /= half;
      const int ci = (int)(q % cin); const int p = (int)(q / cin);
      v = src[((int64_t)co * cin + ci) * kw + 2 * (half - 1 - jj) + p];
    } else {
      const int co = (int)(e % cout); int64_t q = e / cout;
      const int jj = (int)(q % kw); const int ky = (int)(q / kw);
      v = src[((int64_t)co * kh + ky) * kw + (kw - 1 - jj)];
    }
    st_elem(J.dst, J.dtype, e, v);
  }
}

constexpr int CE_NT = 1024;
__global__ __launch_bounds__(CE_NT) void soft_ce_kernel(const float* __restrict__ logits, const float* __restrict__ y,
                                                        int B, int C, int input_sigmoid, float* loss_out,
                                                        float* __restrict__ dlogits, int* correct_out) {
  __shared__ double wl[CE_NT / 64];
  __shared__ int wc[CE_NT / 64];
  const int lane = threadIdx.x & 63, wave = threadIdx.x >> 6;
  double lsum = 0.0;
  int hits = 0;
  const float invB = 1.f / (float)B;
  for (int b = wave; b < B; b += CE_NT / 64) {
    const float* zr = logits + (int64_t)b * C;
    const float* yr = y + (int64_t)b * C;
    float mx = -INFINITY, bestz = -INFINITY, besty = -INFINITY;
    int az = 1 << 30, ay = 1 << 30;
    for (int c = lane; c < C; c += 64) {
      const float l = zr[c];
      const float z = input_sigmoid ? 1.f / (1.f + __expf(-l)) : l;
      mx = fmaxf(mx, z);
      if (l > bestz) { bestz = l; az = c; }
      if (yr[c] > besty) { besty = yr[c]; ay = c; }
    }
    mx = wave_max(mx);
#pragma unroll
    for (int o = 32; o > 0; o >>= 1) {
      const float bz = __shfl_xor(bestz, o, 64); const int iz = __shfl_xor(az, o, 64);
      if (bz > bestz || (bz == bestz && iz < az)) { bestz = bz; az = iz; }
      const float by = __shfl_xor(besty, o, 64); const int iy = __shfl_xor(ay, o, 64);
      if (by > besty || (by == besty && iy < ay)) { besty = by; ay = iy; }
    }
    float se = 0.f;
    for (int c = lane; c < C; c += 64) {
      const float l = zr[c];
      const float z = input_sigmoid ? 1.f / (1.f + __expf(-l)) : l;
      se += expf(z - mx);
    }
    se = wave_sum(se);
    float lrow = 0.f, R = 0.f;
    for (int c = lane; c < C; c += 64) {
      const float l = zr[c];
      const float z = input_sigmoid ? 1.f / (1.f + __expf(-l)) : l;
      const float p = expf(z - mx) / se;
      lrow += yr[c] * logf(p + 1e-8f);
      R += yr[c] * p / (p + 1e-8f);
    }
    lrow = wave_sum(lrow);
    R = wave_sum(R);
    for (int c = lane; c < C; c += 64) {
      const float l = zr[c];
      const float s = input_sigmoid ? 1.f / (1.f + __expf(-l)) : l;
      const float p = expf(s - mx) / se;
      float g = (p * R - yr[c] * p / (p + 1e-8f)) * invB;
      if (input_sigmoid) g *= s * (1.f - s);
      dlogits[(int64_t)b * C + c] = g;
    }
    if (lane == 0) { lsum += -(double)lrow; hits += (az == ay); }
  }
  if (lane == 0) { wl[wave] = lsum; wc[wave] = hits; }
  __syncthreads();
  if (threadIdx.x == 0) {
    double tl = 0.0;
    int tc = 0;
    for (int w = 0; w < CE_NT / 64; ++w) { tl += wl[w]; tc += wc[w]; }
    loss_out[0] = (float)(tl / (double)B);
    if (correct_out) correct_out[0] = tc;
  }
}

constexpr int ADAM_PARTS = 1024;
constexpr int NF_NT = 1024;

__global__ __launch_bounds__(NT) void sqnorm_kernel(void* const* __restrict__ grads, const int64_t* __restrict__ sizes,
                                                    const void* const* __restrict__ pre_sq,
                                                    const int64_t* __restrict__ pre_n, float* __restrict__ ws) {
  const int tsr = blockIdx.y;
  const float* g = reinterpret_cast<const float*>(grads[tsr]);
  const int64_t n = sizes[tsr];
  const int64_t tid = (int64_t)blockIdx.x * NT + threadIdx.x, nthr = (int64_t)gridDim.x * NT;
  const double* pre = pre_sq ? reinterpret_cast<const double*>(pre_sq[tsr]) : nullptr;
  double s = 0.0;
  float fs = 0.f;
  int cnt = 0;
  if (pre) {
    for (int64_t i = tid; i < pre_n[tsr]; i += nthr) s += pre[i];
  } else if ((reinterpret_cast<uintptr_t>(g) & 15) == 0) {
    const int64_t n4 = n >> 2;
    const float4* g4 = reinterpret_cast<const float4*>(g);
    for (int64_t i = tid; i < n4; i += nthr) {
      const float4 v = g4[i];
      fs = fmaf(v.x, v.x, fs); fs = fmaf(v.y, v.y, fs); fs = fmaf(v.z, v.z, fs); fs = fmaf(v.w, v.w, fs);
      if (++cnt == 64) { s += fs; fs = 0.f; cnt = 0; }
    }
    for (int64_t i = (n4 << 2) + tid; i < n; i += nthr) fs = fmaf(g[i], g[i], fs);
  } else {
    for (int64_t i = tid; i < n; i += nthr) {
      fs = fmaf(g[i], g[i], fs);
      if (++cnt == 256) { s += fs; fs = 0.f; cnt = 0; }
    }
  }
  s += fs;
  s = wave_sum_d(s);
  __shared__ double red[4];
  if ((threadIdx.x & 63) == 0) red[threadIdx.x >> 6] = s;
  __syncthreads();
  if (threadIdx.x == 0)
    reinterpret_cast<double*>(ws)[(int64_t)tsr * ADAM_PARTS + blockIdx.x] = red[0] + red[1] + red[2] + red[3];
}

__global__ __launch_bounds__(NF_NT) void norm_final_kernel(double* ws, int ntensors, int nparts, float clip,
                                                           float* total_out, float* coef_out) {
  double s = 0.0;
  const int total = ntensors * nparts;
  for (int i = threadIdx.x; i < total; i += NF_NT) {
    const int tsr = i / nparts, p = i % nparts;
    s += ws[(int64_t)tsr * ADAM_PARTS + p];
  }
  s = wave_sum_d(s);
  __shared__ double red[NF_NT / 64];
  if ((threadIdx.x & 63) == 0) red[threadIdx.x >> 6] = s;
  __syncthreads();
  if (threadIdx.x == 0) {
    double acc = 0.0;
    for (int w = 0; w < NF_NT / 64; ++w) acc += red[w];
    const double tot = sqrt(acc);
    const float totalf = (float)tot;
    float coef = 1.f;
    if (clip > 0.f) {
      coef = clip / (totalf + 1e-6f);
      if (coef > 1.f) coef = 1.f;
    }
    if (total_out) total_out[0] = totalf;
    coef_out[0] = coef;
  }
}

__global__ __launch_bounds__(NT) void adam_kernel(void* const* __restrict__ params, void* const* __restrict__ grads,
                                                  void* const* __restrict__ m1, void* const* __restrict__ m2,
                                                  void* const* __restrict__ shadow,
                                                  const int64_t* __restrict__ sizes, const float* __restrict__ coef_p,
                                                  float lr_over_bc1, float bc2_sqrt, float beta1, float beta2, float eps,
                                                  float wd, const int32_t* __restrict__ steps, float lr) {
  const int tsr = blockIdx.y;
  if (!grads[tsr]) return;
  if (steps) {
    const double st = (double)steps[tsr];
    lr_over_bc1 = (float)(lr / (1.0 - pow((double)beta1, st)));
    bc2_sqrt = (float)sqrt(1.0 - pow((double)beta2, st));
  }
  float* p = reinterpret_cast<float*>(params[tsr]);
  const float* g = reinterpret_cast<const float*>(grads[tsr]);
  float* m = reinterpret_cast<float*>(m1[tsr]);
  float* v = reinterpret_cast<float*>(m2[tsr]);
  bf16* sw = shadow ? reinterpret_cast<bf16*>(shadow[tsr]) : nullptr;
  const int64_t n = sizes[tsr];
  const float coef = coef_p[0];
  auto upd = [&](float pv, float gv, float& mv, float& vv) {
    gv = fmaf(wd, pv, gv * coef);
    mv = mv + (1.f - beta1) * (gv - mv);
    vv = fmaf((1.f - beta2) * gv, gv, vv * beta2);
    const float denom = sqrtf(vv) / bc2_sqrt + eps;
    return pv - lr_over_bc1 * (mv / denom);
  };
  const int64_t tid = (int64_t)blockIdx.x * NT + threadIdx.x, nthr = (int64_t)gridDim.x * NT;
  const bool al = ((reinterpret_cast<uintptr_t>(p) | reinterpret_cast<uintptr_t>(g) | reinterpret_cast<uintptr_t>(m) |
                    reinterpret_cast<uintptr_t>(v)) & 15) == 0 && (reinterpret_cast<uintptr_t>(sw) & 7) == 0;
  int64_t done = 0;
  if (al) {
    const int64_t n4 = n >> 2;
    constexpr int U = 4;
    f32x4* p4 = reinterpret_cast<f32x4*>(p);
    const f32x4* g4 = reinterpret_cast<const f32x4*>(g);
    f32x4* m4 = reinterpret_cast<f32x4*>(m);
    f32x4* v4 = reinterpret_cast<f32x4*>(v);
    auto step4 = [&](int64_t i, f32x4 pv, f32x4 gv, f32x4 mv, f32x4 vv) __attribute__((always_inline)) {
#pragma unroll
      for (int e = 0; e < 4; ++e) {
        float a = mv[e], b = vv[e];
        pv[e] = upd(pv[e], gv[e], a, b);
        mv[e] = a;
        vv[e] = b;
      }
      __builtin_nontemporal_store(pv, p4 + i);
      __builtin_nontemporal_store(mv, m4 + i);
      __builtin_nontemporal_store(vv, v4 + i);
      if (sw) {
        const bf16x4 b4 = {(bf16)pv[0], (bf16)pv[1], (bf16)pv[2], (bf16)pv[3]};
        __builtin_nontemporal_store(b4, reinterpret_cast<bf16x4*>(sw) + i);
      }
    };
    int64_t i = tid;
    for (; i + (U - 1) * nthr < n4; i += U * nthr) {
      f32x4 pv[U], gv[U], mv[U], vv[U];
#pragma unroll
      for (int u = 0; u < U; ++u) {
        const int64_t j = i + u * nthr;
        pv[u] = __builtin_nontemporal_load(p4 + j);
        gv[u] = __builtin_nontemporal_load(g4 + j);
        mv[u] = __builtin_nontemporal_load(m4 + j);
        vv[u] = __builtin_nontemporal_load(v4 + j);
      }
#pragma unroll
      for (int u = 0; u < U; ++u) step4(i + u * nthr, pv[u], gv[u], mv[u], vv[u]);
    }
    for (; i < n4; i += nthr) step4(i, p4[i], g4[i], m4[i], v4[i]);
    done = n4 << 2;
  }
  for (int64_t i = done + tid; i < n; i += nthr) {
    float mv = m[i], vv = v[i];
    p[i] = upd(p[i], g[i], mv, vv);
    m[i] = mv;
    v[i] = vv;
    if (sw) sw[i] = (bf16)p[i];
  }
}

__global__ void dropout_kernel(void* x, int dtype, int64_t n, float p, uint64_t seed) {
  const float scale = 1.f / (1.f - p);
  for (int64_t i = (int64_t)blockIdx.x * blockDim.x + threadIdx.x; i < n; i += (int64_t)gridDim.x * blockDim.x) {
    const float u = hash_u01(seed, (uint64_t)i);
    const float v = u >= p ? ld_elem(x, dtype, i) * scale : 0.f;
    st_elem(x, dtype, i, v);
  }
}

__global__ void dropout_apply_kernel(const void* src, int sd, const float* res, void* dst, int dd, int64_t n, float p,
                                     uint64_t seed) {
  const float scale = 1.f / (1.f - p);
  for (int64_t i = (int64_t)blockIdx.x * blockDim.x + threadIdx.x; i < n; i += (int64_t)gridDim.x * blockDim.x) {
    const float u = hash_u01(seed, (uint64_t)i);
    float v = u >= p ? ld_elem(src, sd, i) * scale : 0.f;
    if (res) v += res[i];
    st_elem(dst, dd, i, v);
  }
}

__global__ void cast_kernel(const void* src, int sd, void* dst, int dd, int64_t n) {
  for (int64_t i = (int64_t)blockIdx.x * blockDim.x + threadIdx.x; i < n; i += (int64_t)gridDim.x * blockDim.x)
    st_elem(dst, dd, i, ld_elem(src, sd, i));
}

__global__ void add_inplace_kernel(float* x, const void* y, int yd, int64_t n) {
  for (int64_t i = (int64_t)blockIdx.x * blockDim.x + threadIdx.x; i < n; i += (int64_t)gridDim.x * blockDim.x)
    x[i] += ld_elem(y, yd, i);
}

__global__ void tokens_fwd_kernel(const float* __restrict__ patches, const float* __restrict__ cls,
                                  const float* __restrict__ pos, float* __restrict__ out, int B, int Np, int D) {
  const int64_t total = (int64_t)B * (Np + 1) * D;
  for (int64_t i = (int64_t)blockIdx.x * blockDim.x + threadIdx.x; i < total; i += (int64_t)gridDim.x * blockDim.x) {
    const int d = (int)(i % D);
    const int64_t q = i / D;
    const int tkn = (int)(q % (Np + 1));
    const int b = (int)(q / (Np + 1));
    const float base = tkn == 0 ? cls[d] : patches[((int64_t)b * Np + tkn - 1) * D + d];
    out[i] = base + pos[(int64_t)tkn * D + d];
  }
}

__global__ void tokens_fwd_inplace_kernel(float4* __restrict__ x, const float4* __restrict__ cls,
                                          const float4* __restrict__ pos, int N, int D4) {
  const int64_t row = blockIdx.x;
  const int tkn = (int)(row % N), d = threadIdx.x;
  const float4 p = pos[(int64_t)tkn * D4 + d];
  float4 v = tkn == 0 ? cls[d] : x[row * D4 + d];
  v.x += p.x; v.y += p.y; v.z += p.z; v.w += p.w;
  x[row * D4 + d] = v;
}

__global__ void ast_patches_kernel(const float* __restrict__ spec, int B, int Fm, int Tf, int ps, int st, int gw,
                                   int N, uint4* __restrict__ out) {
  const int k8 = ps * ps / 8;
  const int64_t total = (int64_t)B * N * k8;
  for (int64_t i = (int64_t)blockIdx.x * blockDim.x + threadIdx.x; i < total; i += (int64_t)gridDim.x * blockDim.x) {
    const int c = (int)(i % k8);
    const int64_t row = i / k8;
    const int tkn = (int)(row % N);
    const int b = (int)(row / N);
    uint32_t w[4] = {0u, 0u, 0u, 0u};
    if (tkn > 0) {
      const int p = tkn - 1, gy = p / gw, gx = p - gy * gw;
      const int k0 = 8 * c, ky = k0 / ps, kx = k0 - ky * ps;
      const float* src = spec + ((int64_t)b * Fm + gy * st + ky) * Tf + gx * st + kx;
#pragma unroll
      for (int j = 0; j < 4; ++j) {
        w[j] = pk_bf16(src[2 * j], src[2 * j + 1]);
      }
    }
    out[i] = uint4{w[0], w[1], w[2], w[3]};
  }
}

__global__ void tokens_bwd_kernel(const float* __restrict__ dout, float* __restrict__ dpatches, float* __restrict__ dcls,
                                  float* __restrict__ dpos, int B, int Np, int D) {
  const int64_t total = (int64_t)(Np + 1) * D;
  for (int64_t i = (int64_t)blockIdx.x * blockDim.x + threadIdx.x; i < total; i += (int64_t)gridDim.x * blockDim.x) {
    const int d = (int)(i % D);
    const int tkn = (int)(i / D);
    float s = 0.f;
    for (int b = 0; b < B; ++b) {
      const float v = dout[((int64_t)b * (Np + 1) + tkn) * D + d];
      s += v;
      if (tkn > 0 && dpatches) dpatches[((int64_t)b * Np + tkn - 1) * D + d] = v;
    }
    if (dpos) dpos[i] = s;
    if (tkn == 0 && dcls) dcls[d] = s;
  }
}

__global__ void tokens_bwd_vec_kernel(const float4* __restrict__ dout, float4* __restrict__ dpatches,
                                      float4* __restrict__ dcls, float4* __restrict__ dpos, int B, int Np, int D4) {
  const int64_t total = (int64_t)(Np + 1) * D4;
  for (int64_t i = (int64_t)blockIdx.x * blockDim.x + threadIdx.x; i < total; i += (int64_t)gridDim.x * blockDim.x) {
    const int d = (int)(i % D4);
    const int tkn = (int)(i / D4);
    float4 s = {0.f, 0.f, 0.f, 0.f};
#pragma unroll 4
    for (int b = 0; b < B; ++b) {
      const float4 v = dout[((int64_t)b * (Np + 1) + tkn) * D4 + d];
      s.x += v.x; s.y += v.y; s.z += v.z; s.w += v.w;
      if (tkn > 0 && dpatches) dpatches[((int64_t)b * Np + tkn - 1) * D4 + d] = v;
    }
    if (dpos) dpos[i] = s;
    if (tkn == 0 && dcls) dcls[d] = s;
  }
}

constexpr int MS_NT = 1024;
__global__ __launch_bounds__(MS_NT) void clip_ms_kernel(const float* __restrict__ x, int64_t T, const int* __restrict__ idx,
                                                        float* __restrict__ ms) {
  int row = blockIdx.x;
  if (idx) {
    row = idx[blockIdx.x];
    if (row < 0) { if (threadIdx.x == 0) ms[blockIdx.x] = 0.f; return; }
  }
  const float* r = x + (int64_t)row * T;
  float fs = 0.f;
  if ((reinterpret_cast<uintptr_t>(r) & 15) == 0) {
    const int64_t n4 = T >> 2;
    for (int64_t i = threadIdx.x; i < n4; i += MS_NT) {
      const float4 v = reinterpret_cast<const float4*>(r)[i];
      fs = fmaf(v.x, v.x, fs); fs = fmaf(v.y, v.y, fs); fs = fmaf(v.z, v.z, fs); fs = fmaf(v.w, v.w, fs);
    }
    for (int64_t i = (n4 << 2) + threadIdx.x; i < T; i += MS_NT) fs = fmaf(r[i], r[i], fs);
  } else {
    for (int64_t i = threadIdx.x; i < T; i += MS_NT) fs = fmaf(r[i], r[i], fs);
  }
  double s = wave_sum_d((double)fs);
  __shared__ double red[MS_NT / 64];
  if ((threadIdx.x & 63) == 0) red[threadIdx.x >> 6] = s;
  __syncthreads();
  if (threadIdx.x == 0) {
    double t = 0.0;
    for (int w = 0; w < MS_NT / 64; ++w) t += red[w];
    ms[blockIdx.x] = (float)(t / (double)T);
  }
}

__device__ __forceinline__ float spl_db(float ms) {
  const float rms = __fsqrt_rn(ms);
  return rms > 0.f ? __fadd_rn(__fmul_rn(20.f, log10f(rms)), 94.f) : -80.f;
}

__global__ void bc_coef_kernel(const float* __restrict__ ms, const float* __restrict__ msq,
                               const int* __restrict__ partner, const float* __restrict__ r,
                               const int64_t* __restrict__ labels, const int64_t* __restrict__ pool_labels, int B,
                               int C, float* __restrict__ p_out, float* __restrict__ yout) {
  const int b = blockIdx.x * blockDim.x + threadIdx.x;
  if (b >= B) return;
  const int q = partner[b];
  const float rr = r[b];
  float p = 1.f;
  if (q >= 0) {
    const double d = (double)spl_db(ms[b]) - (double)spl_db(msq[b]);
    double pd = (double)rr;
    if (fabs(d) > 10.0) {
      const double adj = fmin(fabs(d) / 40.0, 0.3);
      pd = d > 0.0 ? pd * (1.0 - adj) : pd * (1.0 + adj);
    }
    p = fminf(fmaxf((float)pd, 0.f), 1.f);
  }
  p_out[b] = p;
  if (yout) {
    for (int c = 0; c < C; ++c) yout[(int64_t)b * C + c] = 0.f;
    if (q >= 0) {
      yout[(int64_t)b * C + labels[b]] = rr;
      yout[(int64_t)b * C + pool_labels[q]] = 1.f - rr;
    } else {
      yout[(int64_t)b * C + labels[b]] = 1.f;
    }
  }
}

__global__ void bc_mix_kernel(const float* __restrict__ x, const float* __restrict__ pool, int64_t T, int B,
                              const int* __restrict__ partner, const float* __restrict__ p_in, float* __restrict__ out) {
  const int b = blockIdx.y;
  const int q = partner[b];
  const float p = p_in[b];
  const double pd = (double)p;
  const float norm = __fsqrt_rn((float)(pd * pd + (1.0 - pd) * (1.0 - pd)));
  const float q1 = 1.f - p;
  const float* xa = x + (int64_t)b * T;
  const float* xb = pool + (int64_t)(q >= 0 ? q : 0) * T;
  float* o = out + (int64_t)b * T;
  for (int64_t i = (int64_t)blockIdx.x * blockDim.x + threadIdx.x; i < T; i += (int64_t)gridDim.x * blockDim.x)
    o[i] = q >= 0 ? __fdiv_rn(__fadd_rn(__fmul_rn(p, xa[i]), __fmul_rn(q1, xb[i])), norm) : xa[i];
}

constexpr int PT_NT = 256;
__global__ __launch_bounds__(PT_NT) void bc_partner_kernel(const int64_t* __restrict__ labels,
                                                           const int64_t* __restrict__ pool_labels, int N,
                                                           const float* __restrict__ u, int* __restrict__ partner) {
  __shared__ int wcnt[PT_NT / 64];
  const int b = blockIdx.x, lane = threadIdx.x & 63, wave = threadIdx.x >> 6;
  const int64_t l = labels[b];
  int ndiff = 0;
  for (int c = 0; c < N; c += PT_NT) {
    const int i = c + threadIdx.x;
    ndiff += __syncthreads_count(i < N && pool_labels[i] != l);
  }
  if (ndiff == 0) {
    if (threadIdx.x == 0) partner[b] = -1;
    return;
  }
  const int k = min((int)floorf(u[b] * (float)ndiff), ndiff - 1);
  int base = 0;
  for (int c = 0; c < N; c += PT_NT) {
    const int i = c + threadIdx.x;
    const bool f = i < N && pool_labels[i] != l;
    const uint64_t m = __ballot(f);
    if (lane == 0) wcnt[wave] = __popcll(m);
    __syncthreads();
    int before = base;
    for (int w = 0; w < wave; ++w) before += wcnt[w];
    const int rank = before + __popcll(m & ((1ull << lane) - 1ull));
    if (f && rank == k) partner[b] = i;
    int tot = 0;
    for (int w = 0; w < PT_NT / 64; ++w) tot += wcnt[w];
    base += tot;
    __syncthreads();
    if (base > k) break;
  }
}

__global__ void stretch_gain_kernel(const float* __restrict__ x, int64_t T, const double* __restrict__ factor,
                                    const float* __restrict__ gain, float* __restrict__ out) {
  const int b = blockIdx.y;
  const double fac = factor ? factor[b] : 0.0;
  const int64_t m = fac > 0.0 ? (int64_t)((double)T / fac) : T;
  const float g = gain ? gain[b] : 1.f;
  const float scale = (float)T / (float)m;
  const float* xr = x + (int64_t)b * T;
  float* o = out + (int64_t)b * T;
  for (int64_t i = (int64_t)blockIdx.x * blockDim.x + threadIdx.x; i < T; i += (int64_t)gridDim.x * blockDim.x) {
    float v;
    if (i >= m) {
      v = 0.f;
    } else if (m == T) {
      v = xr[i];
    } else {
      float src = __fsub_rn(__fmul_rn(scale, (float)i + 0.5f), 0.5f);
      src = src < 0.f ? 0.f : src;
      const int64_t i0 = min((int64_t)floorf(src), T - 1);
      const float l1 = fminf(fmaxf(src - (float)i0, 0.f), 1.f);
      const float l0 = 1.f - l1;
      const int64_t i1 = i0 + (i0 < T - 1 ? 1 : 0);
      v = __fadd_rn(__fmul_rn(xr[i0], l0), __fmul_rn(xr[i1], l1));
    }
    o[i] = gain ? __fmul_rn(v, g) : v;
  }
}

__global__ void specaug_mixup_kernel(const float* __restrict__ spec, const float* __restrict__ pool,
                                     float* __restrict__ out, int B, int F, int T, const int* t0, const int* tl,
                                     const int* f0, const int* fl, const int* partner, const float* lam) {
  const int b = blockIdx.y;
  const int64_t per = (int64_t)F * T;
  const int q = partner ? partner[b] : -1;
  const float l = (lam && q >= 0) ? lam[b] : 1.f;
  const int ts = t0 ? t0[b] : 0, te = ts + (tl ? tl[b] : 0);
  const int fs = f0 ? f0[b] : 0, fe = fs + (fl ? fl[b] : 0);
  for (int64_t i = (int64_t)blockIdx.x * blockDim.x + threadIdx.x; i < per; i += (int64_t)gridDim.x * blockDim.x) {
    const int t = (int)(i % T), f = (int)(i / T);
    float v = spec[(int64_t)b * per + i];
    if ((t >= ts && t < te) || (f >= fs && f < fe)) v = 0.f;
    if (q >= 0) v = __fadd_rn(__fmul_rn(l, v), __fmul_rn(1.f - l, pool[(int64_t)q * per + i]));
    out[(int64_t)b * per + i] = v;
  }
}

int blocks_for(int64_t n, int per = 256, int cap = 16384) {
  int64_t b = cdiv(n, per);
  if (b > cap) b = cap;
  if (b < 1) b = 1;
  return (int)b;
}

}

extern "C" int mia_pack_weight(const float* src, void* dst, int32_t dtype, int32_t cout, int32_t cin, int32_t kh,
                               int32_t kw, int32_t mode, mia_stream_t stream) {
  MIA_CHECK_ARG(src && dst && cout > 0 && cin > 0 && kh > 0 && kw > 0 && mode >= 0 && mode <= 4, "pack_weight: args");
  if (mode == 2) MIA_CHECK_ARG(kh == 1 && kw % 2 == 0, "pack_weight: parity mode needs kh == 1 and even kw");
  if (mode == 3) MIA_CHECK_ARG(cin == 1, "pack_weight: row-split mode needs cin == 1");
  const int64_t total = (int64_t)cout * cin * kh * kw;
  pack_weight_kernel<<<blocks_for(total), 256, 0, as_stream(stream)>>>(src, dst, dtype, cout, cin, kh, kw, mode);
  MIA_LAUNCH_CHECK("pack_weight");
  return 0;
}

extern "C" int mia_pack_weights(const MiaPackJob* jobs, int32_t n, mia_stream_t stream) {
  MIA_CHECK_ARG(jobs && n > 0 && n <= MIA_PACK_BATCH, "pack_weights: 1..%d jobs", MIA_PACK_BATCH);
  PackBatch b;
  memset(&b, 0, sizeof(b));
  b.n = n;
  b.begin[0] = 0;
  for (int j = 0; j < n; ++j) {
    const MiaPackJob& J = jobs[j];
    MIA_CHECK_ARG(J.src && J.dst && J.cout > 0 && J.cin > 0 && J.kh > 0 && J.kw > 0 && J.mode >= 0 && J.mode <= 3 &&
                      (J.dtype == MIA_BF16 || J.dtype == MIA_F32),
                  "pack_weights: job %d: bad arguments (modes 0-3, bf16 / f32)", j);
    if (J.mode == 2) MIA_CHECK_ARG(J.kh == 1 && J.kw % 2 == 0, "pack_weights: job %d: parity mode needs kh == 1, even kw", j);
    if (J.mode == 3) MIA_CHECK_ARG(J.cin == 1, "pack_weights: job %d: row-split mode needs cin == 1", j);
    b.job[j] = J;
    b.begin[j + 1] = b.begin[j] + (int64_t)J.cout * J.cin * J.kh * J.kw;
  }
  pack_weight_batch_kernel<<<blocks_for(b.begin[n]), 256, 0, as_stream(stream)>>>(b);
  MIA_LAUNCH_CHECK("pack_weights");
  return 0;
}

extern "C" int mia_soft_ce(const float* logits, const float* y, int32_t B, int32_t C, int32_t input_sigmoid, float* loss,
                           float* dlogits, int32_t* correct, mia_stream_t stream) {
  MIA_CHECK_ARG(logits && y && loss && dlogits && B > 0 && C > 0, "soft_ce: args");
  soft_ce_kernel<<<1, CE_NT, 0, as_stream(stream)>>>(logits, y, B, C, input_sigmoid, loss, dlogits, correct);
  MIA_LAUNCH_CHECK("soft_ce");
  return 0;
}

extern "C" int64_t mia_adam_workspace_bytes(int32_t ntensors) {
  return ((int64_t)ntensors * ADAM_PARTS + 2) * 8;
}

extern "C" int64_t mia_adam_coef_offset(int32_t ntensors) { return (int64_t)ntensors * ADAM_PARTS * 8; }

extern "C" int mia_clip_adam(void* const* params, void* const* grads, void* const* exp_avg, void* const* exp_avg_sq,
                             void* const* shadow_bf16, const int64_t* sizes, int32_t ntensors, int64_t max_numel,
                             int64_t max_norm_numel, float lr, float beta1,
                             float beta2, float eps, float weight_decay, int32_t step, float clip,
                             float* total_norm_out, void* sqnorm_ws, const void* const* pre_sq,
                             const int64_t* pre_n, const int32_t* steps, mia_stream_t stream) {
  MIA_CHECK_ARG(params && grads && exp_avg && exp_avg_sq && sizes && sqnorm_ws, "clip_adam: null table");
  MIA_CHECK_ARG(ntensors > 0 && ntensors < 65536 && step >= 1, "clip_adam: ntensors/step");
  MIA_CHECK_ARG(!pre_sq || pre_n, "clip_adam: pre_sq needs pre_n");
  hipStream_t s = as_stream(stream);
  double* ws = reinterpret_cast<double*>(sqnorm_ws);
  float* coef = reinterpret_cast<float*>(ws + (int64_t)ntensors * ADAM_PARTS);
  const int parts = (int)std::min<int64_t>(ADAM_PARTS, std::max<int64_t>(1, cdiv(max_norm_numel, 256 * 256)));
  sqnorm_kernel<<<dim3(parts, ntensors), NT, 0, s>>>(grads, sizes, pre_sq, pre_n, reinterpret_cast<float*>(ws));
  MIA_LAUNCH_CHECK("sqnorm");
  norm_final_kernel<<<1, NF_NT, 0, s>>>(ws, ntensors, parts, clip, total_norm_out, coef);
  MIA_LAUNCH_CHECK("norm_final");
  const double bc1 = 1.0 - pow((double)beta1, (double)step);
  const double bc2 = 1.0 - pow((double)beta2, (double)step);
  const int ablocks = (int)std::min<int64_t>(8192, std::max<int64_t>(1, cdiv(max_numel, 256 * 32)));
  adam_kernel<<<dim3(ablocks, ntensors), NT, 0, s>>>(params, grads, exp_avg, exp_avg_sq, shadow_bf16, sizes, coef,
                                                     (float)(lr / bc1), (float)sqrt(bc2), beta1, beta2, eps,
                                                     weight_decay, steps, lr);
  MIA_LAUNCH_CHECK("adam");
  return 0;
}

extern "C" int mia_dropout(void* x, int32_t dtype, int64_t numel, float p, uint64_t seed, mia_stream_t stream) {
  MIA_CHECK_ARG(x && p >= 0.f && p < 1.f, "dropout: args");
  if (p == 0.f || numel == 0) return 0;
  dropout_kernel<<<blocks_for(numel), 256, 0, as_stream(stream)>>>(x, dtype, numel, p, seed);
  MIA_LAUNCH_CHECK("dropout");
  return 0;
}

extern "C" int mia_dropout_apply(const void* src, int32_t sdtype, const float* res, void* dst, int32_t ddtype,
                                 int64_t numel, float p, uint64_t seed, mia_stream_t stream) {
  MIA_CHECK_ARG(src && dst && p >= 0.f && p < 1.f, "dropout_apply: args");
  MIA_CHECK_ARG((sdtype == MIA_F32 || sdtype == MIA_BF16) && (ddtype == MIA_F32 || ddtype == MIA_BF16),
                "dropout_apply: dtype");
  if (numel == 0) return 0;
  dropout_apply_kernel<<<blocks_for(numel), 256, 0, as_stream(stream)>>>(src, sdtype, res, dst, ddtype, numel, p, seed);
  MIA_LAUNCH_CHECK("dropout_apply");
  return 0;
}

extern "C" int mia_cast(const void* src, int32_t sdtype, void* dst, int32_t ddtype, int64_t numel, mia_stream_t stream) {
  MIA_CHECK_ARG(src && dst, "cast: null");
  if (numel == 0) return 0;
  cast_kernel<<<blocks_for(numel), 256, 0, as_stream(stream)>>>(src, sdtype, dst, ddtype, numel);
  MIA_LAUNCH_CHECK("cast");
  return 0;
}

extern "C" int mia_add_inplace(float* x, const void* y, int32_t ydtype, int64_t numel, mia_stream_t stream) {
  MIA_CHECK_ARG(x && y, "add_inplace: null");
  if (numel == 0) return 0;
  add_inplace_kernel<<<blocks_for(numel), 256, 0, as_stream(stream)>>>(x, y, ydtype, numel);
  MIA_LAUNCH_CHECK("add_inplace");
  return 0;
}

extern "C" int mia_tokens_fwd(const float* patches, const float* cls, const float* pos, float* out, int32_t B,
                              int32_t Np, int32_t D, mia_stream_t stream) {
  MIA_CHECK_ARG(patches && cls && pos && out && B > 0 && Np > 0 && D > 0, "tokens_fwd: args");
  tokens_fwd_kernel<<<blocks_for((int64_t)B * (Np + 1) * D), 256, 0, as_stream(stream)>>>(patches, cls, pos, out, B, Np, D);
  MIA_LAUNCH_CHECK("tokens_fwd");
  return 0;
}

extern "C" int mia_tokens_fwd_inplace(float* x, const float* cls, const float* pos, int32_t B, int32_t N, int32_t D,
                                      mia_stream_t stream) {
  MIA_CHECK_ARG(x && cls && pos && B > 0 && N > 1 && D > 0 && D % 4 == 0, "tokens_fwd_inplace: args");
  MIA_CHECK_ARG(((reinterpret_cast<uintptr_t>(x) | reinterpret_cast<uintptr_t>(cls) | reinterpret_cast<uintptr_t>(pos)) & 15) == 0,
                "tokens_fwd_inplace: x / cls / pos must be 16-byte aligned");
  MIA_CHECK_ARG(D / 4 <= 1024 && (int64_t)B * N < (1ll << 31), "tokens_fwd_inplace: D <= 4096, B*N < 2^31");
  tokens_fwd_inplace_kernel<<<(unsigned)((int64_t)B * N), D / 4, 0, as_stream(stream)>>>(
      reinterpret_cast<float4*>(x), reinterpret_cast<const float4*>(cls), reinterpret_cast<const float4*>(pos), N, D / 4);
  MIA_LAUNCH_CHECK("tokens_fwd_inplace");
  return 0;
}

extern "C" int mia_ast_patches(const float* spec, int32_t B, int32_t Fm, int32_t Tf, int32_t ps, int32_t st, void* out,
                               mia_stream_t stream) {
  MIA_CHECK_ARG(spec && out && B > 0 && ps > 0 && st > 0 && Fm >= ps && Tf >= ps && ps % 8 == 0,
                "ast_patches: args (ps must be a multiple of 8)");
  MIA_CHECK_ARG((reinterpret_cast<uintptr_t>(out) & 15) == 0, "ast_patches: out must be 16-byte aligned");
  const int gh = (Fm - ps) / st + 1, gw = (Tf - ps) / st + 1, N = gh * gw + 1;
  ast_patches_kernel<<<blocks_for((int64_t)B * N * (ps * ps / 8)), 256, 0, as_stream(stream)>>>(
      spec, B, Fm, Tf, ps, st, gw, N, reinterpret_cast<uint4*>(out));
  MIA_LAUNCH_CHECK("ast_patches");
  return 0;
}

extern "C" int mia_tokens_bwd(const float* dout, float* dpatches, float* dcls, float* dpos, int32_t B, int32_t Np,
                              int32_t D, mia_stream_t stream) {
  MIA_CHECK_ARG(dout && B > 0 && Np > 0 && D > 0, "tokens_bwd: args");
  const bool vec = D % 4 == 0 && ((reinterpret_cast<uintptr_t>(dout) | reinterpret_cast<uintptr_t>(dpatches) |
                                   reinterpret_cast<uintptr_t>(dpos) | reinterpret_cast<uintptr_t>(dcls)) & 15) == 0;
  if (vec)
    tokens_bwd_vec_kernel<<<blocks_for((int64_t)(Np + 1) * (D / 4)), 256, 0, as_stream(stream)>>>(
        reinterpret_cast<const float4*>(dout), reinterpret_cast<float4*>(dpatches), reinterpret_cast<float4*>(dcls),
        reinterpret_cast<float4*>(dpos), B, Np, D / 4);
  else
    tokens_bwd_kernel<<<blocks_for((int64_t)(Np + 1) * D), 256, 0, as_stream(stream)>>>(dout, dpatches, dcls, dpos, B, Np, D);
  MIA_LAUNCH_CHECK("tokens_bwd");
  return 0;
}

extern "C" int mia_bc_mix(const float* x, const float* pool, int64_t T, int32_t B, const int32_t* partner,
                          const float* r, const int64_t* labels, const int64_t* pool_labels, int32_t num_classes,
                          float* out, float* yout, float* p_out, void* workspace, mia_stream_t stream) {
  MIA_CHECK_ARG(x && pool && partner && r && labels && pool_labels && out && p_out && workspace && B > 0 && T > 0,
                "bc_mix: args");
  MIA_CHECK_ARG(out != x && out != pool, "bc_mix: out must not alias the inputs");
  hipStream_t s = as_stream(stream);
  float* ms = reinterpret_cast<float*>(workspace);
  float* msq = ms + B;
  clip_ms_kernel<<<B, MS_NT, 0, s>>>(x, T, nullptr, ms);
  MIA_LAUNCH_CHECK("clip_ms");
  clip_ms_kernel<<<B, MS_NT, 0, s>>>(pool, T, partner, msq);
  MIA_LAUNCH_CHECK("clip_ms(partner)");
  bc_coef_kernel<<<(unsigned)cdiv(B, 256), 256, 0, s>>>(ms, msq, partner, r, labels, pool_labels, B, num_classes,
                                                        p_out, yout);
  MIA_LAUNCH_CHECK("bc_coef");
  bc_mix_kernel<<<dim3((unsigned)std::min<int64_t>(cdiv(T, 256), 512), B), 256, 0, s>>>(x, pool, T, B, partner, p_out,
                                                                                      out);
  MIA_LAUNCH_CHECK("bc_mix");
  return 0;
}

extern "C" int mia_bc_partner(const int64_t* labels, int32_t B, const int64_t* pool_labels, int32_t N, const float* u,
                              int32_t* partner, mia_stream_t stream) {
  MIA_CHECK_ARG(labels && pool_labels && u && partner && B > 0 && N > 0, "bc_partner: args");
  bc_partner_kernel<<<B, PT_NT, 0, as_stream(stream)>>>(labels, pool_labels, N, u, partner);
  MIA_LAUNCH_CHECK("bc_partner");
  return 0;
}

extern "C" int mia_stretch_gain(const float* x, int64_t T, int32_t B, const double* factor, const float* gain,
                                float* out, mia_stream_t stream) {
  MIA_CHECK_ARG(x && out && B > 0 && T > 0 && out != x, "stretch_gain: args");
  stretch_gain_kernel<<<dim3((unsigned)std::min<int64_t>(cdiv(T, 256), 512), B), 256, 0, as_stream(stream)>>>(
      x, T, factor, gain, out);
  MIA_LAUNCH_CHECK("stretch_gain");
  return 0;
}

extern "C" int mia_spec_augment_mixup(const float* spec, const float* pool, float* out, int32_t B, int32_t F,
                                      int32_t T, const int32_t* t0, const int32_t* tlen, const int32_t* f0,
                                      const int32_t* flen, const int32_t* partner, const float* lam,
                                      mia_stream_t stream) {
  MIA_CHECK_ARG(spec && out && B > 0 && F > 0 && T > 0, "spec_augment_mixup: args");
  MIA_CHECK_ARG(!partner || (pool && pool != out), "spec_augment_mixup: mixup needs a pool distinct from out");
  specaug_mixup_kernel<<<dim3((unsigned)std::min<int64_t>(cdiv((int64_t)F * T, 256), 512), B), 256, 0,
                         as_stream(stream)>>>(spec, pool ? pool : spec, out, B, F, T, t0, tlen, f0, flen, partner, lam);
  MIA_LAUNCH_CHECK("spec_augment_mixup");
  return 0;
}

__global__ __launch_bounds__(256) void stream_copy_kernel(const f32x4* __restrict__ src, f32x4* __restrict__ dst,
                                                          int64_t n16) {
  const int64_t stride = (int64_t)gridDim.x * 256 * 4;
  for (int64_t i = (int64_t)blockIdx.x * 1024 + threadIdx.x; i < n16; i += stride) {
    f32x4 v[4];
#pragma unroll
    for (int u = 0; u < 4; ++u)
      if (i + 256 * u < n16) v[u] = __builtin_nontemporal_load(src + i + 256 * u);
#pragma unroll
    for (int u = 0; u < 4; ++u)
      if (i + 256 * u < n16) __builtin_nontemporal_store(v[u], dst + i + 256 * u);
  }
}

extern "C" int mia_stream_copy(const void* src, void* dst, int64_t bytes, mia_stream_t stream) {
  MIA_CHECK_ARG(src && dst && bytes > 0 && bytes % 16 == 0, "stream_copy: bytes must be a positive multiple of 16");
  MIA_CHECK_ARG(((reinterpret_cast<uintptr_t>(src) | reinterpret_cast<uintptr_t>(dst)) & 15) == 0,
                "stream_copy: 16-B aligned pointers");
  const int64_t n16 = bytes / 16;
  const unsigned grid = (unsigned)std::min<int64_t>(cdiv(n16, 1024), (int64_t)mia::cu_count() * 16);
  stream_copy_kernel<<<grid, 256, 0, as_stream(stream)>>>((const f32x4*)src, (f32x4*)dst, n16);
  MIA_LAUNCH_CHECK("stream_copy");
  return 0;
}

__global__ __launch_bounds__(256) void mfma_rate_kernel(int iters, uint32_t seed, float* __restrict__ sink) {
  const int lane = threadIdx.x & 63;
  uint32_t h = seed ^ (blockIdx.x * 256u + threadIdx.x) * 2654435761u;
  bf16x8 a, b;
#pragma unroll
  for (int i = 0; i < 8; ++i) {
    h = h * 1664525u + 1013904223u;
    a[i] = (bf16)((float)(int)(h >> 16 & 0xff) * (1.f / 128.f) - 1.f);
    b[i] = (bf16)((float)(int)(h >> 24) * (1.f / 128.f) - 1.f);
  }
  f32x4 acc[4] = {};
  for (int it = 0; it < iters; ++it) {
#pragma unroll
    for (int r = 0; r < 4; ++r)
#pragma unroll
      for (int q = 0; q < 4; ++q) acc[q] = __builtin_amdgcn_mfma_f32_16x16x32_bf16(a, b, acc[q], 0, 0, 0);
  }
  float v = 0.f;
#pragma unroll
  for (int q = 0; q < 4; ++q) v += acc[q][0] + acc[q][1] + acc[q][2] + acc[q][3];
  sink[blockIdx.x * 256 + threadIdx.x] = v + (float)lane * 0.f;
}

extern "C" int64_t mia_mfma_rate_sink_floats(int32_t waves_per_simd) {
  return (int64_t)mia::cu_count() * (waves_per_simd > 0 ? waves_per_simd : 1) * 256;
}

extern "C" int mia_mfma_rate(float* sink, int32_t iters, int32_t waves_per_simd, mia_stream_t stream) {
  MIA_CHECK_ARG(sink && iters > 0 && waves_per_simd > 0 && waves_per_simd <= 8, "mfma_rate: bad arguments");
  const unsigned grid = (unsigned)(mia::cu_count() * waves_per_simd);
  mfma_rate_kernel<<<grid, 256, 0, as_stream(stream)>>>(iters, 0x9e3779b9u, sink);
  MIA_LAUNCH_CHECK("mfma_rate");
  return 0;
}
```

dl-sound-classification_amd/csrc/pool.hip:

```cpp
#include <cstdlib>

#include "common.h"

namespace {

constexpr int NT = 256;

struct FastDiv {
  uint32_t d, m, l;
};
static FastDiv make_fastdiv(uint32_t d) {
  uint32_t l = 0;
  while ((1u << l) < d) ++l;
  const uint32_t m = (uint32_t)((((uint64_t)1 << 32) * (((uint64_t)1 << l) - d)) / d + 1);
  return FastDiv{d, m, l};
}
__device__ __forceinline__ uint32_t fdiv(uint32_t n, const FastDiv& f) { return (__umulhi(n, f.m) + n) >> f.l; }

__device__ __forceinline__ int64_t out_index(int layout, int b, int oy, int ox, int c, int OH, int OW, int C) {
  if (layout == 0) return (((int64_t)b * OH + oy) * OW + ox) * C + c;
  if (layout == 1) return ((int64_t)b * C + c) * OW + ox;
  return (((int64_t)b * C + c) * OH + oy) * OW + ox;
}

__global__ __launch_bounds__(NT) void pool_fwd_kernel(const void* __restrict__ x, int dtype, int n, int H, int W,
                                                      int C, int kh, int kw, const float* __restrict__ scale,
                                                      const float* __restrict__ shift, void* out, int layout,
                                                      uint8_t* __restrict__ argmax, void* __restrict__ win) {
  const int OH = H / kh, OW = W / kw, G = C / 8;
  const int total = n * OH * OW * G;
  for (int idx = blockIdx.x * NT + threadIdx.x; idx < total; idx += gridDim.x * NT) {
    const int cg = idx % G;
    int p = idx / G;
    const int ox = p % OW;
    p /= OW;
    const int oy = p % OH;
    const int b = p / OH;
    float sc[8], sh[8], best[8], raw[8];
    int arg[8];
#pragma unroll
    for (int i = 0; i < 8; ++i) {
      sc[i] = scale ? scale[cg * 8 + i] : 1.f;
      sh[i] = shift ? shift[cg * 8 + i] : 0.f;
      best[i] = -INFINITY;
      raw[i] = 0.f;
      arg[i] = 0;
    }
    for (int dy = 0; dy < kh; ++dy) {
      const int iy = oy * kh + dy;
      for (int dx = 0; dx < kw; ++dx) {
        const int ix = ox * kw + dx;
        const int64_t off = (((int64_t)b * H + iy) * W + ix) * C + cg * 8;
        float f[8];
        if (dtype == MIA_BF16) {
          uint4 u = *reinterpret_cast<const uint4*>(reinterpret_cast<const bf16*>(x) + off);
          uint32_t w4[4] = {u.x, u.y, u.z, u.w};
#pragma unroll
          for (int i = 0; i < 4; ++i) { f[2 * i] = __uint_as_float(w4[i] << 16); f[2 * i + 1] = __uint_as_float(w4[i] & 0xffff0000u); }
        } else {
          const float4* q = reinterpret_cast<const float4*>(reinterpret_cast<const float*>(x) + off);
          float4 a = q[0], c4 = q[1];
          f[0] = a.x; f[1] = a.y; f[2] = a.z; f[3] = a.w; f[4] = c4.x; f[5] = c4.y; f[6] = c4.z; f[7] = c4.w;
        }
        const int pos = dy * kw + dx;
#pragma unroll
        for (int i = 0; i < 8; ++i) {
          const float v = fmaxf(fmaf(f[i], sc[i], sh[i]), 0.f);
          if (v > best[i]) { best[i] = v; raw[i] = f[i]; arg[i] = pos; }
        }
      }
    }
    const int64_t aoff = (((int64_t)b * OH + oy) * OW + ox) * C + cg * 8;
    uint32_t a0 = 0, a1 = 0;
#pragma unroll
    for (int i = 0; i < 4; ++i) { a0 |= (uint32_t)arg[i] << (8 * i); a1 |= (uint32_t)arg[i + 4] << (8 * i); }
    *reinterpret_cast<uint2*>(argmax + aoff) = make_uint2(a0, a1);
    if (win) store8(win, dtype, aoff, raw);
    if (layout == 0) {
      store8(out, dtype, aoff, best);
    } else {
#pragma unroll
      for (int i = 0; i < 8; ++i) st_elem(out, dtype, out_index(layout, b, oy, ox, cg * 8 + i, OH, OW, C), best[i]);
    }
  }
}

__global__ __launch_bounds__(NT) void pool_raw_stats_kernel(const bf16* __restrict__ x, int n, int H, int W, int C,
                                                            int kh, int kw, const float* __restrict__ gamma,
                                                            const float* __restrict__ kshift, bf16* __restrict__ win,
                                                            uint8_t* __restrict__ argmax, float* __restrict__ partial) {
  const int OH = H / kh, OW = W / kw, G = C / 8;
  const int total = n * OH * OW * G;
  const int cg = threadIdx.x % G;
  float dir[8], ks[8], s1[8], s2[8];
#pragma unroll
  for (int i = 0; i < 8; ++i) {
    const float gv = gamma[cg * 8 + i];
    dir[i] = gv > 0.f ? 1.f : (gv < 0.f ? -1.f : 0.f);
    ks[i] = kshift[cg * 8 + i];
    s1[i] = 0.f; s2[i] = 0.f;
  }
  for (int idx = blockIdx.x * NT + threadIdx.x; idx < total; idx += gridDim.x * NT) {
    int p = idx / G;
    const int ox = p % OW;
    p /= OW;
    const int oy = p % OH;
    const int b = p / OH;
    float best[8], bestraw[8];
    int arg[8];
#pragma unroll
    for (int i = 0; i < 8; ++i) { best[i] = -INFINITY; bestraw[i] = 0.f; arg[i] = 0; }
    for (int dy = 0; dy < kh; ++dy) {
      const int iy = oy * kh + dy;
      const bf16* row = x + (((int64_t)b * H + iy) * W + (int64_t)ox * kw) * C + cg * 8;
#pragma unroll 4
      for (int dx = 0; dx < kw; ++dx) {
        const uint4 u = *reinterpret_cast<const uint4*>(row + (int64_t)dx * C);
        const uint32_t w4[4] = {u.x, u.y, u.z, u.w};
        float f[8];
#pragma unroll
        for (int i = 0; i < 4; ++i) { f[2 * i] = __uint_as_float(w4[i] << 16); f[2 * i + 1] = __uint_as_float(w4[i] & 0xffff0000u); }
        const int pos = dy * kw + dx;
#pragma unroll
        for (int i = 0; i < 8; ++i) {
          const float d = f[i] - ks[i];
          s1[i] += d;
          s2[i] = fmaf(d, d, s2[i]);
          const float key = dir[i] * f[i];
          if (key > best[i]) { best[i] = key; bestraw[i] = f[i]; arg[i] = pos; }
        }
      }
    }
    const int64_t aoff = (((int64_t)b * OH + oy) * OW + ox) * C + cg * 8;
    uint32_t a0 = 0, a1 = 0;
#pragma unroll
    for (int i = 0; i < 4; ++i) { a0 |= (uint32_t)arg[i] << (8 * i); a1 |= (uint32_t)arg[i + 4] << (8 * i); }
    *reinterpret_cast<uint2*>(argmax + aoff) = make_uint2(a0, a1);
    uint32_t o4[4];
#pragma unroll
    for (int i = 0; i < 4; ++i) {
      o4[i] = pk_bf16(bestraw[2 * i], bestraw[2 * i + 1]);
    }
    *reinterpret_cast<uint4*>(win + aoff) = make_uint4(o4[0], o4[1], o4[2], o4[3]);
  }
  const int tailw = W - OW * kw;
  const int ttotal = n * H * tailw * G;
  for (int idx = blockIdx.x * NT + threadIdx.x; idx < ttotal; idx += gridDim.x * NT) {
    int p = idx / G;
    const int tx = p % tailw;
    const int r = p / tailw;
    const uint4 u = *reinterpret_cast<const uint4*>(x + ((int64_t)r * W + OW * kw + tx) * C + cg * 8);
    const uint32_t w4[4] = {u.x, u.y, u.z, u.w};
#pragma unroll
    for (int i = 0; i < 4; ++i) {
      const float lo = __uint_as_float(w4[i] << 16) - ks[2 * i], hi = __uint_as_float(w4[i] & 0xffff0000u) - ks[2 * i + 1];
      s1[2 * i] += lo; s2[2 * i] = fmaf(lo, lo, s2[2 * i]);
      s1[2 * i + 1] += hi; s2[2 * i + 1] = fmaf(hi, hi, s2[2 * i + 1]);
    }
  }
  __shared__ float red[NT][17];
#pragma unroll
  for (int i = 0; i < 8; ++i) { red[threadIdx.x][i] = s1[i]; red[threadIdx.x][8 + i] = s2[i]; }
  __syncthreads();
  if ((int)threadIdx.x < C * 2) {
    const int c = threadIdx.x >> 1, which = threadIdx.x & 1, g = c >> 3, i = c & 7;
    float a = 0.f;
    for (int t = g; t < NT; t += G) a += red[t][which * 8 + i];
    partial[((int64_t)blockIdx.x * C + c) * 2 + which] = a;
  }
}

__global__ __launch_bounds__(NT) void pool_apply_kernel(const bf16* __restrict__ win, int n, int OH, int OW, int C,
                                                        const float* __restrict__ scale, const float* __restrict__ shift,
                                                        void* out, int dtype, int layout) {
  const int64_t total = (int64_t)n * OH * OW * C;
  for (int64_t e = (int64_t)blockIdx.x * NT + threadIdx.x; e < total; e += (int64_t)gridDim.x * NT) {
    const int c = (int)(e % C);
    int64_t p = e / C;
    const int ox = (int)(p % OW);
    p /= OW;
    const int oy = (int)(p % OH), b = (int)(p / OH);
    const float v = fmaxf(fmaf((float)win[e], scale[c], shift[c]), 0.f);
    st_elem(out, dtype, out_index(layout, b, oy, ox, c, OH, OW, C), v);
  }
}

__global__ __launch_bounds__(256) void pool_apply_t64_kernel(const bf16* __restrict__ win, int OW,
                                                             const float* __restrict__ scale,
                                                             const float* __restrict__ shift, bf16* __restrict__ out) {
  __shared__ bf16 tile[64][64 + 4];
  const int tiles = (OW + 63) / 64;
  const int b = blockIdx.x / tiles, p0 = (blockIdx.x - b * tiles) * 64;
  const int t = threadIdx.x;
#pragma unroll
  for (int k = 0; k < 2; ++k) {
    const int q = t + 256 * k, r = q >> 3, ch = q & 7;
    bf16x8 v = {};
    if (p0 + r < OW) v = *reinterpret_cast<const bf16x8*>(win + ((int64_t)b * OW + p0 + r) * 64 + ch * 8);
#pragma unroll
    for (int i = 0; i < 8; ++i) {
      const int c = ch * 8 + i;
      tile[c][r] = (bf16)fmaxf(fmaf((float)v[i], scale[c], shift[c]), 0.f);
    }
  }
  __syncthreads();
#pragma unroll
  for (int k = 0; k < 4; ++k) {
    const int q = t + 256 * k, c = q >> 4, g = q & 15;
    const int p = p0 + 4 * g;
    bf16* dst = out + ((int64_t)b * 64 + c) * OW + p;
    const bf16x4 w4 = *reinterpret_cast<const bf16x4*>(&tile[c][4 * g]);
    if (p + 4 <= OW && (reinterpret_cast<uintptr_t>(dst) & 7) == 0) {
      *reinterpret_cast<bf16x4*>(dst) = w4;
    } else {
#pragma unroll
      for (int i = 0; i < 4; ++i)
        if (p + i < OW) dst[i] = w4[i];
    }
  }
}

__global__ __launch_bounds__(NT) void pool_bwd_kernel(const void* __restrict__ dout, int layout,
                                                      const uint8_t* __restrict__ argmax, const void* __restrict__ x,
                                                      int dtype, int n, int H, int W, int C, int kh, int kw,
                                                      const float* __restrict__ scale, const float* __restrict__ shift,
                                                      const float* __restrict__ mean,
                                                      const float* __restrict__ invstd, void* dz,
                                                      float* __restrict__ partial) {
  const int OH = H / kh, OW = W / kw, G = C / 8;
  const int t = threadIdx.x;
  const int cg = t % G, rs = t / G, rslots = NT / G;
  float sc[8], sh[8], mu[8], is[8];
#pragma unroll
  for (int i = 0; i < 8; ++i) {
    sc[i] = scale[cg * 8 + i]; sh[i] = shift[cg * 8 + i]; mu[i] = mean[cg * 8 + i]; is[i] = invstd[cg * 8 + i];
  }
  float s1[8] = {0}, s2[8] = {0};
  const int P = n * H * W;
  for (int r = blockIdx.x * rslots + rs; r < P; r += gridDim.x * rslots) {
    const int ix = r % W;
    const int q = r / W;
    const int iy = q % H;
    const int b = q / H;
    const int64_t off = (int64_t)r * C + cg * 8;
    float g[8];
#pragma unroll
    for (int i = 0; i < 8; ++i) g[i] = 0.f;
    const int oy = iy / kh, ox = ix / kw;
    if (oy < OH && ox < OW) {
      const int pos = (iy - oy * kh) * kw + (ix - ox * kw);
      const int64_t aoff = (((int64_t)b * OH + oy) * OW + ox) * C + cg * 8;
      const uint2 am = *reinterpret_cast<const uint2*>(argmax + aoff);
      float xv[8];
      if (dtype == MIA_BF16) {
        uint4 u = *reinterpret_cast<const uint4*>(reinterpret_cast<const bf16*>(x) + off);
        uint32_t w4[4] = {u.x, u.y, u.z, u.w};
#pragma unroll
        for (int i = 0; i < 4; ++i) { xv[2 * i] = __uint_as_float(w4[i] << 16); xv[2 * i + 1] = __uint_as_float(w4[i] & 0xffff0000u); }
      } else {
#pragma unroll
        for (int i = 0; i < 8; ++i) xv[i] = reinterpret_cast<const float*>(x)[off + i];
      }
#pragma unroll
      for (int i = 0; i < 8; ++i) {
        const uint32_t word = i < 4 ? am.x : am.y;
        const int a = (int)((word >> (8 * (i & 3))) & 0xffu);
        if (a == pos && fmaf(xv[i], sc[i], sh[i]) > 0.f) {
          g[i] = ld_elem(dout, dtype, out_index(layout, b, oy, ox, cg * 8 + i, OH, OW, C));
          s1[i] += g[i];
          s2[i] = fmaf(g[i], (xv[i] - mu[i]) * is[i], s2[i]);
        }
      }
    }
    store8(dz, dtype, off, g);
  }
  __shared__ float red[NT * 16];
#pragma unroll
  for (int i = 0; i < 8; ++i) { red[t * 16 + i] = s1[i]; red[t * 16 + 8 + i] = s2[i]; }
  __syncthreads();
  for (int e = t; e < 2 * C; e += NT) {
    const int qq = e / C, c = e % C, g2 = c / 8, ci = c % 8;
    float acc = 0.f;
    for (int r2 = 0; r2 < rslots; ++r2) acc += red[(r2 * G + g2) * 16 + qq * 8 + ci];
    partial[((int64_t)blockIdx.x * C + c) * 2 + qq] = acc;
  }
}

__global__ __launch_bounds__(NT) void pool_bwd_sparse_kernel(const void* __restrict__ dout, int layout,
                                                             const uint8_t* __restrict__ argmax,
                                                             const void* __restrict__ x,
                                                             const void* __restrict__ win, int dtype, int n, int H,
                                                             int W, int C, int kh, int kw,
                                                             const float* __restrict__ scale,
                                                             const float* __restrict__ shift,
                                                             const float* __restrict__ mean,
                                                             const float* __restrict__ invstd,
                                                             float* __restrict__ gm,
                                                             float* __restrict__ partial) {
  const int OH = H / kh, OW = W / kw, G = C / 8;
  const int t = threadIdx.x;
  const int cg = t % G, rs = t / G, rslots = NT / G;
  float sc[8], sh[8], mu[8], is[8];
#pragma unroll
  for (int i = 0; i < 8; ++i) {
    sc[i] = scale[cg * 8 + i]; sh[i] = shift[cg * 8 + i]; mu[i] = mean[cg * 8 + i]; is[i] = invstd[cg * 8 + i];
  }
  float s1[8] = {0}, s2[8] = {0};
  const int cells = n * OH * OW;
  for (int cell = blockIdx.x * rslots + rs; cell < cells; cell += gridDim.x * rslots) {
    const int ox = cell % OW;
    const int q = cell / OW;
    const int oy = q % OH;
    const int b = q / OH;
    float xv[8], dv[8];
    if (win) {
      const int64_t off = (int64_t)cell * C + cg * 8;
      load8(win, dtype, off, xv);
#pragma unroll
      for (int i = 0; i < 8; ++i) dv[i] = ld_elem(dout, dtype, out_index(layout, b, oy, ox, cg * 8 + i, OH, OW, C));
    } else {
      const uint2 am = *reinterpret_cast<const uint2*>(argmax + (int64_t)cell * C + cg * 8);
#pragma unroll
      for (int i = 0; i < 8; ++i) {
        const uint32_t word = i < 4 ? am.x : am.y;
        const int a = (int)((word >> (8 * (i & 3))) & 0xffu);
        const int iy = oy * kh + a / kw, ix = ox * kw + a % kw;
        xv[i] = ld_elem(x, dtype, (((int64_t)b * H + iy) * W + ix) * C + cg * 8 + i);
        dv[i] = ld_elem(dout, dtype, out_index(layout, b, oy, ox, cg * 8 + i, OH, OW, C));
      }
    }
    float gv[8];
#pragma unroll
    for (int i = 0; i < 8; ++i) {
      const float g = fmaf(xv[i], sc[i], sh[i]) > 0.f ? dv[i] : 0.f;
      gv[i] = g;
      s1[i] += g;
      s2[i] = fmaf(g, (xv[i] - mu[i]) * is[i], s2[i]);
    }
    float4* gq = reinterpret_cast<float4*>(gm + (int64_t)cell * C + cg * 8);
    gq[0] = make_float4(gv[0], gv[1], gv[2], gv[3]);
    gq[1] = make_float4(gv[4], gv[5], gv[6], gv[7]);
  }
  __shared__ float red[NT * 16];
#pragma unroll
  for (int i = 0; i < 8; ++i) { red[t * 16 + i] = s1[i]; red[t * 16 + 8 + i] = s2[i]; }
  __syncthreads();
  for (int e = t; e < 2 * C; e += NT) {
    const int qq = e / C, c = e % C, g2 = c / 8, ci = c % 8;
    float acc = 0.f;
    for (int r2 = 0; r2 < rslots; ++r2) acc += red[(r2 * G + g2) * 16 + qq * 8 + ci];
    partial[((int64_t)blockIdx.x * C + c) * 2 + qq] = acc;
  }
}

__global__ __launch_bounds__(NT) void pool_bn_bwd_apply_oct_kernel(const float* __restrict__ gm,
                                                                   const uint8_t* __restrict__ argmax,
                                                                   const bf16* __restrict__ x, int n, int H, int W,
                                                                   int C, int kh, int kw, FastDiv dNO, FastDiv dH,
                                                                   FastDiv dG, const float* __restrict__ gamma,
                                                                   const float* __restrict__ mean,
                                                                   const float* __restrict__ invstd,
                                                                   const float* __restrict__ dgamma,
                                                                   const float* __restrict__ dbeta, bf16* dx,
                                                                   float* __restrict__ partial) {
  const int OH = H / kh, OW = W / kw, G = C / 8, NO = (W + 7) / 8;
  const int t = threadIdx.x;
  const int cg = t % G;
  const int P = n * H * W;
  float mu[8], is[8], a[8], mb[8], mg[8];
  const float invP = 1.f / (float)P;
#pragma unroll
  for (int i = 0; i < 8; ++i) {
    const int c = cg * 8 + i;
    mu[i] = mean[c]; is[i] = invstd[c];
    a[i] = (gamma ? gamma[c] : 1.f) * is[i];
    mb[i] = dbeta[c] * invP;
    mg[i] = dgamma[c] * invP;
  }
  float s1[8] = {0};
  const int64_t units = (int64_t)n * H * NO * G;
  for (int64_t u = (int64_t)blockIdx.x * NT + t; u < units; u += (int64_t)gridDim.x * NT) {
    const int rest = (int)fdiv((uint32_t)(u), dG);
    const int rowi = (int)fdiv((uint32_t)rest, dNO);
    const int o8 = rest - rowi * NO;
    const int iy = rowi - (int)fdiv((uint32_t)rowi, dH) * H;
    const int b = (rowi - iy) / H;
    const int ix0 = o8 * 8;
    const int oy = iy / kh, ox = ix0 / kw;
    const bool cell = oy < OH && ox < OW;
    const int64_t coff = cell ? (((int64_t)b * OH + oy) * OW + ox) * C + cg * 8 : 0;
    const uint2 am = *reinterpret_cast<const uint2*>(argmax + coff);
    const float4 g0 = reinterpret_cast<const float4*>(gm + coff)[0];
    const float4 g1 = reinterpret_cast<const float4*>(gm + coff)[1];
    const int64_t xoff = ((int64_t)rowi * W + ix0) * C + cg * 8;
    uint4 xr[8];
#pragma unroll
    for (int j = 0; j < 8; ++j) {
      const int64_t o = ix0 + j < W ? xoff + (int64_t)j * C : xoff;
      xr[j] = *reinterpret_cast<const uint4*>(x + o);
    }
    const float gv[8] = {g0.x, g0.y, g0.z, g0.w, g1.x, g1.y, g1.z, g1.w};
    const int pos0 = (iy - oy * kh) * kw + (ix0 - ox * kw);
#pragma unroll
    for (int j = 0; j < 8; ++j) {
      if (ix0 + j >= W) break;
      const uint32_t w4[4] = {xr[j].x, xr[j].y, xr[j].z, xr[j].w};
      uint32_t o4[4];
#pragma unroll
      for (int q = 0; q < 4; ++q) {
        float g[2];
#pragma unroll
        for (int h = 0; h < 2; ++h) {
          const int i = 2 * q + h;
          const float xv = __uint_as_float(h ? (w4[q] & 0xffff0000u) : (w4[q] << 16));
          const uint32_t word = i < 4 ? am.x : am.y;
          const int av = (int)((word >> (8 * (i & 3))) & 0xffu);
          const float gi = cell && av == pos0 + j ? gv[i] : 0.f;
          g[h] = a[i] * (gi - mb[i] - (xv - mu[i]) * is[i] * mg[i]);
          s1[i] += g[h];
        }
        o4[q] = pk_bf16(g[0], g[1]);
      }
      *reinterpret_cast<uint4*>(dx + xoff + (int64_t)j * C) = uint4{o4[0], o4[1], o4[2], o4[3]};
    }
  }
  if (!partial) return;
  __shared__ float red[NT * 8];
#pragma unroll
  for (int i = 0; i < 8; ++i) red[t * 8 + i] = s1[i];
  __syncthreads();
  const int rslots = NT / G;
  for (int c = t; c < C; c += NT) {
    const int g2 = c / 8, ci = c % 8;
    float acc = 0.f;
    for (int r2 = 0; r2 < rslots; ++r2) acc += red[(r2 * G + g2) * 8 + ci];
    partial[((int64_t)blockIdx.x * C + c) * 2] = acc;
  }
}

template <int KW, int RU>
__global__ __launch_bounds__(NT) void pool_bn_bwd_apply_run_kernel(const float* __restrict__ gm,
                                                                   const uint8_t* __restrict__ argmax,
                                                                   const bf16* __restrict__ x, int n, int H, int W,
                                                                   int C, int kh, FastDiv dNR, FastDiv dH, FastDiv dG,
                                                                   const float* __restrict__ gamma,
                                                                   const float* __restrict__ mean,
                                                                   const float* __restrict__ invstd,
                                                                   const float* __restrict__ dgamma,
                                                                   const float* __restrict__ dbeta, bf16* dx,
                                                                   float* __restrict__ partial) {
  const int OH = H / kh, OW = W / KW, G = C / 8, NR = (W + KW - 1) / KW;
  const int t = threadIdx.x;
  const int cg = t % G;
  const int P = n * H * W;
  float mu[8], is[8], a[8], mb[8], mg[8];
  const float invP = 1.f / (float)P;
#pragma unroll
  for (int i = 0; i < 8; ++i) {
    const int c = cg * 8 + i;
    mu[i] = mean[c]; is[i] = invstd[c];
    a[i] = (gamma ? gamma[c] : 1.f) * is[i];
    mb[i] = dbeta[c] * invP;
    mg[i] = dgamma[c] * invP;
  }
  float s1[8] = {0};
  const int units = n * H * NR * G;
  const int stride = gridDim.x * NT;
  for (int u0 = blockIdx.x * NT + t; u0 < units; u0 += RU * stride) {
    uint4 xr[RU][KW];
    uint2 am[RU];
    float4 g0[RU], g1[RU];
    int64_t xoff[RU];
    int pos0[RU], ix0[RU];
#pragma unroll
    for (int v = 0; v < RU; ++v) {
      const int u = min(u0 + v * stride, units - 1);
      const int rest = (int)fdiv((uint32_t)u, dG);
      const int rowi = (int)fdiv((uint32_t)rest, dNR);
      const int run = rest - rowi * NR;
      const int b = (int)fdiv((uint32_t)rowi, dH);
      const int iy = rowi - b * H;
      ix0[v] = run * KW;
      const int oy = iy / kh;
      const bool cell = oy < OH && run < OW;
      const int64_t coff = cell ? (((int64_t)b * OH + oy) * OW + run) * C + cg * 8 : 0;
      pos0[v] = cell ? (iy - oy * kh) * KW : -256;
      am[v] = *reinterpret_cast<const uint2*>(argmax + coff);
      g0[v] = reinterpret_cast<const float4*>(gm + coff)[0];
      g1[v] = reinterpret_cast<const float4*>(gm + coff)[1];
      xoff[v] = ((int64_t)rowi * W + ix0[v]) * C + cg * 8;
#pragma unroll
      for (int j = 0; j < KW; ++j) {
        const int64_t o = ix0[v] + j < W ? xoff[v] + (int64_t)j * C : xoff[v];
        xr[v][j] = *reinterpret_cast<const uint4*>(x + o);
      }
    }
#pragma unroll
    for (int v = 0; v < RU; ++v) {
      if (u0 + v * stride >= units) break;
      const float gv[8] = {g0[v].x, g0[v].y, g0[v].z, g0[v].w, g1[v].x, g1[v].y, g1[v].z, g1[v].w};
#pragma unroll
      for (int j = 0; j < KW; ++j) {
        if (ix0[v] + j >= W) break;
        const uint32_t w4[4] = {xr[v][j].x, xr[v][j].y, xr[v][j].z, xr[v][j].w};
        uint32_t o4[4];
#pragma unroll
        for (int q = 0; q < 4; ++q) {
          float g[2];
#pragma unroll
          for (int h = 0; h < 2; ++h) {
            const int i = 2 * q + h;
            const float xv = __uint_as_float(h ? (w4[q] & 0xffff0000u) : (w4[q] << 16));
            const uint32_t word = i < 4 ? am[v].x : am[v].y;
            const int av = (int)((word >> (8 * (i & 3))) & 0xffu);
            const float gi = av == pos0[v] + j ? gv[i] : 0.f;
            g[h] = a[i] * (gi - mb[i] - (xv - mu[i]) * is[i] * mg[i]);
            s1[i] += g[h];
          }
          o4[q] = pk_bf16(g[0], g[1]);
        }
        *reinterpret_cast<uint4*>(dx + xoff[v] + (int64_t)j * C) = uint4{o4[0], o4[1], o4[2], o4[3]};
      }
    }
  }
  if (!partial) return;
  __shared__ float red[NT * 8];
#pragma unroll
  for (int i = 0; i < 8; ++i) red[t * 8 + i] = s1[i];
  __syncthreads();
  const int rslots = NT / G;
  for (int c = t; c < C; c += NT) {
    const int g2 = c / 8, ci = c % 8;
    float acc = 0.f;
    for (int r2 = 0; r2 < rslots; ++r2) acc += red[(r2 * G + g2) * 8 + ci];
    partial[((int64_t)blockIdx.x * C + c) * 2] = acc;
  }
}

#ifndef PB_UNROLL
#define PB_UNROLL 4
#endif
#ifndef PB_NB
#define PB_NB 1024
#endif
#ifndef PB_RUNS
#define PB_RUNS 1
#endif
__global__ __launch_bounds__(NT) void pool_bn_bwd_apply_kernel(const float* __restrict__ gm,
                                                               const uint8_t* __restrict__ argmax,
                                                               const void* __restrict__ x, int dtype, int n, int H,
                                                               int W, int C, int kh, int kw, FastDiv dW, FastDiv dH,
                                                               FastDiv dkw, FastDiv dkh,
                                                               const float* __restrict__ gamma,
                                                               const float* __restrict__ mean,
                                                               const float* __restrict__ invstd,
                                                               const float* __restrict__ dgamma,
                                                               const float* __restrict__ dbeta, void* dx,
                                                               float* __restrict__ partial) {
  const int OH = H / kh, OW = W / kw, G = C / 8;
  const int t = threadIdx.x;
  const int cg = t % G, rs = t / G, rslots = NT / G;
  const int P = n * H * W;
  float mu[8], is[8], a[8], mb[8], mg[8];
  const float invP = 1.f / (float)P;
#pragma unroll
  for (int i = 0; i < 8; ++i) {
    const int c = cg * 8 + i;
    mu[i] = mean[c]; is[i] = invstd[c];
    a[i] = (gamma ? gamma[c] : 1.f) * is[i];
    mb[i] = dbeta[c] * invP;
    mg[i] = dgamma[c] * invP;
  }
  float s1[8] = {0};
  const int stride = gridDim.x * rslots;
  for (int r0 = blockIdx.x * rslots + rs; r0 < P; r0 += PB_UNROLL * stride) {
    float xv[PB_UNROLL][8];
    uint2 am[PB_UNROLL];
    float4 g0[PB_UNROLL], g1[PB_UNROLL];
#pragma unroll
    for (int u = 0; u < PB_UNROLL; ++u) {
      const int r = min(r0 + u * stride, P - 1);
      load8(x, dtype, (int64_t)r * C + cg * 8, xv[u]);
      const int q = (int)fdiv(r, dW), ix = r - q * W;
      const int b = (int)fdiv(q, dH), iy = q - b * H;
      const int oy = min((int)fdiv(iy, dkh), OH - 1), ox = min((int)fdiv(ix, dkw), OW - 1);
      const int64_t coff = (((int64_t)b * OH + oy) * OW + ox) * C + cg * 8;
      am[u] = *reinterpret_cast<const uint2*>(argmax + coff);
      g0[u] = reinterpret_cast<const float4*>(gm + coff)[0];
      g1[u] = reinterpret_cast<const float4*>(gm + coff)[1];
    }
#pragma unroll
    for (int u = 0; u < PB_UNROLL; ++u) {
      const int r = r0 + u * stride;
      if (r >= P) break;
      const int q = (int)fdiv(r, dW), ix = r - q * W;
      const int iy = q - (int)fdiv(q, dH) * H;
      const int oy = (int)fdiv(iy, dkh), ox = (int)fdiv(ix, dkw);
      const int pos = oy < OH && ox < OW ? (iy - oy * kh) * kw + (ix - ox * kw) : -1;
      const float gv[8] = {g0[u].x, g0[u].y, g0[u].z, g0[u].w, g1[u].x, g1[u].y, g1[u].z, g1[u].w};
      float g[8];
#pragma unroll
      for (int i = 0; i < 8; ++i) {
        const uint32_t word = i < 4 ? am[u].x : am[u].y;
        const int av = (int)((word >> (8 * (i & 3))) & 0xffu);
        const float gi = av == pos ? gv[i] : 0.f;
        g[i] = a[i] * (gi - mb[i] - (xv[u][i] - mu[i]) * is[i] * mg[i]);
        s1[i] += g[i];
      }
      store8(dx, dtype, (int64_t)r * C + cg * 8, g);
    }
  }
  if (!partial) return;
  __shared__ float red[NT * 8];
#pragma unroll
  for (int i = 0; i < 8; ++i) red[t * 8 + i] = s1[i];
  __syncthreads();
  for (int c = t; c < C; c += NT) {
    const int g2 = c / 8, ci = c % 8;
    float acc = 0.f;
    for (int r2 = 0; r2 < rslots; ++r2) acc += red[(r2 * G + g2) * 8 + ci];
    partial[((int64_t)blockIdx.x * C + c) * 2] = acc;
  }
}

__global__ void partial_final_kernel(const float* __restrict__ partial, int nblk, int C, float* dgamma, float* dbeta) {
  const int c = blockIdx.x;
  const double a = block_sum_strided(partial + (int64_t)c * 2, nblk, (int64_t)C * 2);
  const double b = block_sum_strided(partial + (int64_t)c * 2 + 1, nblk, (int64_t)C * 2);
  if (threadIdx.x != 0) return;
  if (dbeta) dbeta[c] = (float)a;
  if (dgamma) dgamma[c] = (float)b;
}

__global__ void col2im_rows_kernel(const float* __restrict__ p, int n, int ph, int w, int kh, void* out, int dtype) {
  const int H = ph + kh - 1;
  const int total = n * H * w;
  for (int idx = blockIdx.x * blockDim.x + threadIdx.x; idx < total; idx += gridDim.x * blockDim.x) {
    const int iw = idx % w;
    const int q = idx / w;
    const int ih = q % H;
    const int b = q / H;
    float s = 0.f;
    for (int ky = 0; ky < kh; ++ky) {
      const int r = ih - ky;
      if (r >= 0 && r < ph) s += p[(((int64_t)b * ph + r) * w + iw) * kh + ky];
    }
    st_elem(out, dtype, idx, s);
  }
}

}

extern "C" int mia_pool_fwd(const void* x, int32_t dtype, int32_t n, int32_t h, int32_t w, int32_t c, int32_t kh,
                            int32_t kw, const float* scale, const float* shift, void* out, int32_t out_layout,
                            uint8_t* argmax, void* win, mia_stream_t stream) {
  MIA_CHECK_ARG(x && out && argmax, "pool_fwd: null pointer");
  MIA_CHECK_ARG(!win || (reinterpret_cast<uintptr_t>(win) & 15) == 0, "pool_fwd: win alignment");
  MIA_CHECK_ARG(((reinterpret_cast<uintptr_t>(x) | (out_layout == 0 ? reinterpret_cast<uintptr_t>(out) : 0)) & 15) == 0,
                "pool_fwd: x (and an NHWC out) must be 16-byte aligned");
  MIA_CHECK_ARG(c % 8 == 0 && kh > 0 && kw > 0 && kh * kw <= 256 && h >= kh && w >= kw, "pool_fwd: bad geometry");
  MIA_CHECK_ARG(out_layout >= 0 && out_layout <= 2 && (out_layout != 1 || h / kh == 1), "pool_fwd: bad layout");
  MIA_CHECK_ARG((int64_t)n * h * w * (c / 8) < (1ll << 31), "pool_fwd: too many elements for 32-bit indexing");
  const int64_t total = (int64_t)n * (h / kh) * (w / kw) * (c / 8);
  const int nb = (int)std::min<int64_t>(cdiv(total, NT), 16384);
  pool_fwd_kernel<<<nb, NT, 0, as_stream(stream)>>>(x, dtype, n, h, w, c, kh, kw, scale, shift, out, out_layout, argmax,
                                                    win);
  MIA_LAUNCH_CHECK("pool_fwd");
  return 0;
}

extern "C" int mia_pool_raw_stats(const void* x, int32_t n, int32_t h, int32_t w, int32_t c, int32_t kh, int32_t kw,
                                  const float* gamma, const float* kshift, void* win, uint8_t* argmax, float* partial,
                                  int32_t nblocks, mia_stream_t stream) {
  MIA_CHECK_ARG(x && gamma && kshift && win && argmax && partial && nblocks > 0, "pool_raw_stats: null pointer");
  MIA_CHECK_ARG(c % 8 == 0 && c >= 8 && c * 2 <= NT && (NT % (c / 8)) == 0, "pool_raw_stats: channels");
  MIA_CHECK_ARG(h % kh == 0 && w >= kw && kh * kw <= 256, "pool_raw_stats: window geometry");
  MIA_CHECK_ARG((int64_t)n * h * w * (c / 8) < (1ll << 31), "pool_raw_stats: too many elements for 32-bit indexing");
  MIA_CHECK_ARG((reinterpret_cast<uintptr_t>(x) | reinterpret_cast<uintptr_t>(win)) % 16 == 0 &&
                reinterpret_cast<uintptr_t>(argmax) % 8 == 0, "pool_raw_stats: alignment");
  pool_raw_stats_kernel<<<nblocks, NT, 0, as_stream(stream)>>>(reinterpret_cast<const bf16*>(x), n, h, w, c, kh, kw,
                                                               gamma, kshift, reinterpret_cast<bf16*>(win), argmax,
                                                               partial);
  MIA_LAUNCH_CHECK("pool_raw_stats");
  return 0;
}

extern "C" int mia_pool_apply(const void* win, int32_t n, int32_t oh, int32_t ow, int32_t c, const float* scale,
                              const float* shift, void* out, int32_t dtype, int32_t out_layout, mia_stream_t stream) {
  MIA_CHECK_ARG(win && scale && shift && out && n > 0 && oh > 0 && ow > 0 && c > 0, "pool_apply: bad arguments");
  if (out_layout == 1 && oh == 1 && c == 64 && dtype == MIA_BF16 && (reinterpret_cast<uintptr_t>(win) & 15) == 0 &&
      (int64_t)n * cdiv(ow, 64) < (1ll << 31)) {
    pool_apply_t64_kernel<<<(unsigned)(n * cdiv(ow, 64)), 256, 0, as_stream(stream)>>>(
        reinterpret_cast<const bf16*>(win), ow, scale, shift, reinterpret_cast<bf16*>(out));
    MIA_LAUNCH_CHECK("pool_apply_t64");
    return 0;
  }
  const int64_t total = (int64_t)n * oh * ow * c;
  const int nb = (int)std::min<int64_t>(cdiv(total, NT), 16384);
  pool_apply_kernel<<<nb, NT, 0, as_stream(stream)>>>(reinterpret_cast<const bf16*>(win), n, oh, ow, c, scale, shift,
                                                      out, dtype, out_layout);
  MIA_LAUNCH_CHECK("pool_apply");
  return 0;
}

extern "C" int mia_pool_bwd_bn_relu_reduce(const void* dout, int32_t out_layout, const uint8_t* argmax, const void* x,
                                           int32_t dtype, int32_t n, int32_t h, int32_t w, int32_t c, int32_t kh,
                                           int32_t kw, const float* scale, const float* shift, const float* mean,
                                           const float* invstd, void* dz, float* dgamma, float* dbeta, void* partial,
                                           mia_stream_t stream) {
  MIA_CHECK_ARG(dout && argmax && x && scale && shift && mean && invstd && dz && dgamma && dbeta && partial,
                "pool_bwd: null pointer");
  MIA_CHECK_ARG(c % 8 == 0 && c >= 8 && (NT % (c / 8)) == 0, "pool_bwd: channels");
  MIA_CHECK_ARG((int64_t)n * h * w < (1ll << 31), "pool_bwd: too many pixels for 32-bit indexing");
  const int rslots = NT / (c / 8);
  const int64_t P = (int64_t)n * h * w;
  hipStream_t s = as_stream(stream);
  const int nb = (int)std::max<int64_t>(1, std::min<int64_t>(cdiv(P, (int64_t)rslots * 8), 1024));
  pool_bwd_kernel<<<nb, NT, 0, s>>>(dout, out_layout, argmax, x, dtype, n, h, w, c, kh, kw, scale, shift, mean,
                                    invstd, dz, (float*)partial);
  MIA_LAUNCH_CHECK("pool_bwd");
  partial_final_kernel<<<(unsigned)c, 256, 0, s>>>((const float*)partial, nb, c, dgamma, dbeta);
  MIA_LAUNCH_CHECK("pool_bwd_final");
  return 0;
}

extern "C" int mia_pool_bwd_gather(const void* dout, int32_t out_layout, const uint8_t* argmax, const void* x,
                                   const void* win, int32_t dtype, int32_t n, int32_t h, int32_t w, int32_t c, int32_t kh, int32_t kw,
                                   const float* scale, const float* shift, const float* mean, const float* invstd,
                                   float* gm, float* dgamma, float* dbeta, void* partial, mia_stream_t stream) {
  MIA_CHECK_ARG(dout && argmax && x && scale && shift && mean && invstd && gm && dgamma && dbeta && partial,
                "pool_bwd_gather: null pointer");
  MIA_CHECK_ARG(c % 8 == 0 && c >= 8 && (NT % (c / 8)) == 0, "pool_bwd_gather: channels");
  MIA_CHECK_ARG((int64_t)n * h * w < (1ll << 31), "pool_bwd_gather: too many pixels for 32-bit indexing");
  MIA_CHECK_ARG(h >= kh && w >= kw && kh * kw <= 256 && (reinterpret_cast<uintptr_t>(gm) & 15) == 0,
                "pool_bwd_gather: bad geometry / alignment");
  const int rslots = NT / (c / 8);
  const int64_t cells = (int64_t)n * (h / kh) * (w / kw);
  const int nb = (int)std::max<int64_t>(1, std::min<int64_t>(cdiv(cells, (int64_t)rslots * 2), 1024));
  hipStream_t s = as_stream(stream);
  MIA_CHECK_ARG(!win || (reinterpret_cast<uintptr_t>(win) & 15) == 0, "pool_bwd_gather: win alignment");
  pool_bwd_sparse_kernel<<<nb, NT, 0, s>>>(dout, out_layout, argmax, x, win, dtype, n, h, w, c, kh, kw, scale, shift, mean,
                                           invstd, gm, (float*)partial);
  MIA_LAUNCH_CHECK("pool_bwd_gather");
  partial_final_kernel<<<(unsigned)c, 256, 0, s>>>((const float*)partial, nb, c, dgamma, dbeta);
  MIA_LAUNCH_CHECK("pool_bwd_gather_final");
  return 0;
}

extern "C" int mia_pool_bn_relu_bwd_apply(const float* gm, const uint8_t* argmax, const void* x, int32_t dtype,
                                          int32_t n, int32_t h, int32_t w, int32_t c, int32_t kh, int32_t kw,
                                          const float* gamma, const float* mean, const float* invstd,
                                          const float* dgamma, const float* dbeta, void* dx, float* dbias,
                                          void* partial, mia_stream_t stream) {
  MIA_CHECK_ARG(gm && argmax && x && mean && invstd && dgamma && dbeta && dx, "pool_bn_bwd_apply: null pointer");
  MIA_CHECK_ARG(!dbias || partial, "pool_bn_bwd_apply: dbias needs the partial workspace");
  MIA_CHECK_ARG(c % 8 == 0 && c >= 8 && (NT % (c / 8)) == 0, "pool_bn_bwd_apply: channels");
  MIA_CHECK_ARG((int64_t)n * h * w < (1ll << 31), "pool_bn_bwd_apply: too many pixels for 32-bit indexing");
  MIA_CHECK_ARG(h >= kh && w >= kw && kh * kw <= 256, "pool_bn_bwd_apply: bad geometry");
  const int rslots = NT / (c / 8);
  const int64_t P = (int64_t)n * h * w;
  hipStream_t s = as_stream(stream);
  const int64_t units = (int64_t)n * h * ((w + 7) / 8) * (c / 8);
  if (kw % 8 == 0 && dtype == MIA_BF16 && units < (1ll << 31) &&
      ((reinterpret_cast<uintptr_t>(x) | reinterpret_cast<uintptr_t>(dx)) & 15) == 0) {
    const int nb = (int)std::max<int64_t>(1, std::min<int64_t>(cdiv(units, NT), 1024));
    pool_bn_bwd_apply_oct_kernel<<<nb, NT, 0, s>>>(gm, argmax, reinterpret_cast<const bf16*>(x), n, h, w, c, kh, kw,
                                                   make_fastdiv((w + 7) / 8), make_fastdiv(h), make_fastdiv(c / 8),
                                                   gamma, mean, invstd, dgamma, dbeta, reinterpret_cast<bf16*>(dx),
                                                   dbias ? (float*)partial : nullptr);
    MIA_LAUNCH_CHECK("pool_bn_bwd_apply");
    if (dbias) {
      partial_final_kernel<<<(unsigned)c, 256, 0, s>>>((const float*)partial, nb, c, nullptr, dbias);
      MIA_LAUNCH_CHECK("pool_bn_bwd_apply_final");
    }
    return 0;
  }
  const int64_t runs = (int64_t)n * h * cdiv(w, kw) * (c / 8);
  static const bool per_pixel = getenv("MIA_POOL_BWD_PIXEL") != nullptr;
  if (kw >= 2 && kw <= 4 && dtype == MIA_BF16 && runs < (1ll << 31) && !per_pixel &&
      ((reinterpret_cast<uintptr_t>(x) | reinterpret_cast<uintptr_t>(dx)) & 15) == 0) {
    constexpr int RU = PB_RUNS;
    const int nb = (int)std::max<int64_t>(1, std::min<int64_t>(cdiv(runs, (int64_t)NT * RU), PB_NB));
    const FastDiv dNR = make_fastdiv((int)cdiv(w, kw)), dH = make_fastdiv(h), dG = make_fastdiv(c / 8);
    float* part = dbias ? (float*)partial : nullptr;
    const bf16* xb = reinterpret_cast<const bf16*>(x);
    bf16* dxb = reinterpret_cast<bf16*>(dx);
    if (kw == 2)
      pool_bn_bwd_apply_run_kernel<2, RU><<<nb, NT, 0, s>>>(gm, argmax, xb, n, h, w, c, kh, dNR, dH, dG, gamma, mean,
                                                            invstd, dgamma, dbeta, dxb, part);
    else if (kw == 3)
      pool_bn_bwd_apply_run_kernel<3, RU><<<nb, NT, 0, s>>>(gm, argmax, xb, n, h, w, c, kh, dNR, dH, dG, gamma, mean,
                                                            invstd, dgamma, dbeta, dxb, part);
    else
      pool_bn_bwd_apply_run_kernel<4, RU><<<nb, NT, 0, s>>>(gm, argmax, xb, n, h, w, c, kh, dNR, dH, dG, gamma, mean,
                                                            invstd, dgamma, dbeta, dxb, part);
    MIA_LAUNCH_CHECK("pool_bn_bwd_apply_run");
    if (dbias) {
      partial_final_kernel<<<(unsigned)c, 256, 0, s>>>((const float*)partial, nb, c, nullptr, dbias);
      MIA_LAUNCH_CHECK("pool_bn_bwd_apply_final");
    }
    return 0;
  }
  const int nb = (int)std::max<int64_t>(1, std::min<int64_t>(cdiv(P, (int64_t)rslots * 8), 1024));
  pool_bn_bwd_apply_kernel<<<nb, NT, 0, s>>>(gm, argmax, x, dtype, n, h, w, c, kh, kw, make_fastdiv(w), make_fastdiv(h),
                                             make_fastdiv(kw), make_fastdiv(kh), gamma, mean, invstd, dgamma,
                                             dbeta, dx, dbias ? (float*)partial : nullptr);
  MIA_LAUNCH_CHECK("pool_bn_bwd_apply");
  if (dbias) {
    partial_final_kernel<<<(unsigned)c, 256, 0, s>>>((const float*)partial, nb, c, nullptr, dbias);
    MIA_LAUNCH_CHECK("pool_bn_bwd_apply_final");
  }
  return 0;
}

extern "C" int mia_col2im_rows(const float* p, int32_t n, int32_t ph, int32_t w, int32_t kh, void* out, int32_t dtype,
                               mia_stream_t stream) {
  MIA_CHECK_ARG(p && out && n > 0 && ph > 0 && w > 0 && kh > 0, "col2im_rows: bad arguments");
  MIA_CHECK_ARG((int64_t)n * (ph + kh - 1) * w < (1ll << 31), "col2im_rows: too many elements");
  const int64_t total = (int64_t)n * (ph + kh - 1) * w;
  const int nb = (int)std::min<int64_t>(cdiv(total, 256), 16384);
  col2im_rows_kernel<<<nb, 256, 0, as_stream(stream)>>>(p, n, ph, w, kh, out, dtype);
  MIA_LAUNCH_CHECK("col2im_rows");
  return 0;
}
```

Baseline: 15440 clips/s.

## Unroll split reductions, parallelize soft-CE rows, add transposing pool kernels

Several reduction kernels (conv3 wgrad reduce1, feconv wgrad reduce, mgemm split-K reduce) are replaced by variants that issue 8–16 independent loads per thread before accumulating, so more memory requests are in flight. Soft cross-entropy moves from a single 1024-thread block to one wave per row across many blocks, followed by a small final reduction through device globals. The pool forward and backward-gather paths get templated fixed-window and transposing (tiled via LDS) kernels with XCD-aware block remapping, so NCHW/NHWC layout conversions are done in-kernel with coalesced access. Each new path sits behind env-var fallbacks to the old kernels. The cost is more code, an extra kernel launch for soft-CE, and the bookkeeping risk of the new pool tiling.

```diff
diff --git a/dl-sound-classification_amd/csrc/conv3w.hip b/dl-sound-classification_amd/csrc/conv3w.hip
--- a/dl-sound-classification_amd/csrc/conv3w.hip
+++ b/dl-sound-classification_amd/csrc/conv3w.hip
@@ -1,3 +1,5 @@
+#include <cstdlib>
+
 #include "common.h"
 
 namespace {
@@ -209,6 +211,29 @@
   for (int w = w0; w < w1; ++w) s += (double)part[(int64_t)w * 2048 + e];
   tmp[gi * 2048 + e] = s;
 }
+__global__ __launch_bounds__(256) void conv3_wgrad_reduce1x16_kernel(const float* __restrict__ part, int nslab,
+                                                                     double* __restrict__ tmp) {
+  const int e = blockIdx.x * 256 + threadIdx.x, gi = blockIdx.y;
+  const int per = (nslab + C3_G - 1) / C3_G;
+  const int w0 = gi * per, w1 = min(nslab, w0 + per);
+  const float* p = part + e;
+  double s = 0.0;
+  int w = w0;
+  for (; w + 16 <= w1; w += 16) {
+    float v[16];
+#pragma unroll
+    for (int u = 0; u < 16; ++u) v[u] = p[(int64_t)(w + u) * 2048];
+#pragma unroll
+    for (int u = 0; u < 16; ++u) s += (double)v[u];
+  }
+  for (; w < w1; ++w) s += (double)p[(int64_t)w * 2048];
+  tmp[gi * 2048 + e] = s;
+}
+void conv3_wgrad_reduce1(const float* part, int nslab, double* tmp, hipStream_t s) {
+  const char* v1 = getenv("MIA_REDUCE_V1");
+  if (v1 && v1[0] == '1') conv3_wgrad_reduce1_kernel<<<dim3(8, C3_G), 256, 0, s>>>(part, nslab, tmp);
+  else conv3_wgrad_reduce1x16_kernel<<<dim3(8, C3_G), 256, 0, s>>>(part, nslab, tmp);
+}
 __global__ __launch_bounds__(256) void conv3_wgrad_reduce2_kernel(const double* __restrict__ tmp, float* __restrict__ dw) {
   const int e = blockIdx.x * 256 + threadIdx.x;
   double s = 0.0;
@@ -233,7 +258,7 @@
   conv3_wgrad_kernel<false><<<nwaves / 4, 256, 0, s>>>(a);
   MIA_LAUNCH_CHECK("conv3_wgrad");
   double* tmp = reinterpret_cast<double*>(part + (int64_t)nwaves * 2048);
-  conv3_wgrad_reduce1_kernel<<<dim3(8, C3_G), 256, 0, s>>>(part, nwaves, tmp);
+  conv3_wgrad_reduce1(part, nwaves, tmp, s);
   conv3_wgrad_reduce2_kernel<<<8, 256, 0, s>>>(tmp, dw);
   MIA_LAUNCH_CHECK("conv3_wgrad_reduce");
   return 0;
@@ -264,7 +289,7 @@
   hipStream_t s = as_stream(stream);
   conv3_wgrad_kernel<true><<<nwaves / 4, 256, 0, s>>>(a);
   MIA_LAUNCH_CHECK("conv3_wgrad_bn");
-  conv3_wgrad_reduce1_kernel<<<dim3(8, C3_G), 256, 0, s>>>(part, nwaves, tmp);
+  conv3_wgrad_reduce1(part, nwaves, tmp, s);
   conv3_wgrad_reduce2_kernel<<<8, 256, 0, s>>>(tmp, dw);
   conv3_bias_final_kernel<<<32, 256, 0, s>>>(a.bpart, nwaves, dbias);
   MIA_LAUNCH_CHECK("conv3_wgrad_bn reduce");
diff --git a/dl-sound-classification_amd/csrc/feconv.hip b/dl-sound-classification_amd/csrc/feconv.hip
--- a/dl-sound-classification_amd/csrc/feconv.hip
+++ b/dl-sound-classification_amd/csrc/feconv.hip
@@ -950,6 +950,26 @@
   out[e] = acc;
 }
 
+__global__ __launch_bounds__(64) void fw_reduce16_kernel(const float* __restrict__ ws, int slabs, int len,
+                                                         float* __restrict__ out) {
+  const int e = blockIdx.x * 64 + threadIdx.x;
+  if (e >= len) return;
+  const float* p = ws + e;
+  float acc = 0.f;
+  int k = 0;
+  for (; k + 16 <= slabs; k += 16) {
+    float v[16];
+#pragma unroll
+    for (int u = 0; u < 16; ++u) v[u] = p[(int64_t)(k + u) * len];
+#pragma unroll
+    for (int u = 0; u < 16; ++u) acc += v[u];
+  }
+  for (; k < slabs; ++k) acc += p[(int64_t)k * len];
+  out[e] = acc;
+}
+
+bool reduce_v1() { const char* e = getenv("MIA_REDUCE_V1"); return e && e[0] == '1'; }
+
 bool aligned16(const void* p) { return (reinterpret_cast<uintptr_t>(p) & 15) == 0; }
 
 bool fe_ws() { const char* e = getenv("MIA_FECONV_WS"); return !(e && e[0] == '0'); }
@@ -1035,7 +1055,8 @@
     MIA_LAUNCH_CHECK("fe_conv2_wgrad");
     slab0 += grid;
   }
-  fw_reduce_kernel<<<64 * 512 / 256, 256, 0, s>>>(reinterpret_cast<const float*>(workspace), slabs, 64 * 512, dw);
+  if (reduce_v1()) fw_reduce_kernel<<<64 * 512 / 256, 256, 0, s>>>(reinterpret_cast<const float*>(workspace), slabs, 64 * 512, dw);
+  else fw_reduce16_kernel<<<64 * 512 / 64, 64, 0, s>>>(reinterpret_cast<const float*>(workspace), slabs, 64 * 512, dw);
   MIA_LAUNCH_CHECK("fe_conv2_wgrad reduce");
   return 0;
 }
diff --git a/dl-sound-classification_amd/csrc/mgemm.hip b/dl-sound-classification_amd/csrc/mgemm.hip
--- a/dl-sound-classification_amd/csrc/mgemm.hip
+++ b/dl-sound-classification_amd/csrc/mgemm.hip
@@ -1,3 +1,5 @@
+#include <cstdlib>
+
 #include "common.h"
 #include "gemm_common.h"
 
@@ -771,6 +773,33 @@
   }
 }
 
+__global__ __launch_bounds__(64) void mg_splitk_reduce8_kernel(const float* __restrict__ ws, int split, int64_t M,
+                                                               int64_t N, void* out, int64_t ldc, int out_f32,
+                                                               const float* __restrict__ bias) {
+  const int64_t n4 = N >> 2;
+  const int64_t i = (int64_t)blockIdx.x * 64 + threadIdx.x;
+  if (i >= M * n4) return;
+  const int64_t m = i / n4, n = (i - m * n4) * 4;
+  const float* p = ws + m * N + n;
+  const int64_t slab = M * N;
+  f32x4 s = *reinterpret_cast<const f32x4*>(p);
+  int zz = 1;
+  for (; zz + 8 <= split; zz += 8) {
+    f32x4 v[8];
+#pragma unroll
+    for (int u = 0; u < 8; ++u) v[u] = *reinterpret_cast<const f32x4*>(p + (int64_t)(zz + u) * slab);
+#pragma unroll
+    for (int u = 0; u < 8; ++u) s += v[u];
+  }
+  for (; zz < split; ++zz) s += *reinterpret_cast<const f32x4*>(p + (int64_t)zz * slab);
+  if (bias) {
+#pragma unroll
+    for (int c = 0; c < 4; ++c) s[c] += bias[n + c];
+  }
+  if (out_f32) *reinterpret_cast<f32x4*>(reinterpret_cast<float*>(out) + m * ldc + n) = s;
+  else *reinterpret_cast<uint2*>(reinterpret_cast<bf16*>(out) + m * ldc + n) = pack4(s);
+}
+
 __global__ __launch_bounds__(256) void mg_acs_reduce_kernel(const float* __restrict__ part, int split, int64_t M,
                                                             float* __restrict__ out) {
   const int64_t m = (int64_t)blockIdx.x * 256 + threadIdx.x;
@@ -927,7 +956,12 @@
   if (a.split > 1) {
     const int64_t total = M * (N / 4);
     const int blocks = (int)std::min<int64_t>(cdiv(total, 256), 4096);
-    mg_splitk_reduce_kernel<<<blocks, 256, 0, s>>>(a.ws, a.split, M, N, E.ptr, E.ldc, E.dtype == MIA_F32, E.bias);
+    const char* v1 = getenv("MIA_REDUCE_V1");
+    if ((v1 && v1[0] == '1') || cdiv(total, 64) >= (1ll << 31))
+      mg_splitk_reduce_kernel<<<blocks, 256, 0, s>>>(a.ws, a.split, M, N, E.ptr, E.ldc, E.dtype == MIA_F32, E.bias);
+    else
+      mg_splitk_reduce8_kernel<<<(unsigned)cdiv(total, 64), 64, 0, s>>>(a.ws, a.split, M, N, E.ptr, E.ldc,
+                                                                         E.dtype == MIA_F32, E.bias);
     MIA_LAUNCH_CHECK("mgemm splitk reduce");
   }
   if (E.a_colsum) {
diff --git a/dl-sound-classification_amd/csrc/misc.hip b/dl-sound-classification_amd/csrc/misc.hip
--- a/dl-sound-classification_amd/csrc/misc.hip
+++ b/dl-sound-classification_amd/csrc/misc.hip
@@ -1,3 +1,5 @@
+#include <cstdlib>
+
 #include "common.h"
 
 namespace {
@@ -77,6 +79,55 @@
   }
 }
 
+__device__ __forceinline__ float soft_ce_row(const float* __restrict__ zr, const float* __restrict__ yr, int C,
+                                             int input_sigmoid, float invB, float* __restrict__ drow, int lane,
+                                             bool* hit) {
+  float mx = -INFINITY, bestz = -INFINITY, besty = -INFINITY;
+  int az = 1 << 30, ay = 1 << 30;
+  for (int c = lane; c < C; c += 64) {
+    const float l = zr[c];
+    const float z = input_sigmoid ? 1.f / (1.f + __expf(-l)) : l;
+    mx = fmaxf(mx, z);
+    if (l > bestz) { bestz = l; az = c; }
+    if (yr[c] > besty) { besty = yr[c]; ay = c; }
+  }
+  mx = wave_max(mx);
+#pragma unroll
+  for (int o = 32; o > 0; o >>= 1) {
+    const float bz = __shfl_xor(bestz, o, 64); const int iz = __shfl_xor(az, o, 64);
+    if (bz > bestz || (bz == bestz && iz < az)) { bestz = bz; az = iz; }
+    const float by = __shfl_xor(besty, o, 64); const int iy = __shfl_xor(ay, o, 64);
+    if (by > besty || (by == besty && iy < ay)) { besty = by; ay = iy; }
+  }
+  float se = 0.f;
+  for (int c = lane; c < C; c += 64) {
+    const float l = zr[c];
+    const float z = input_sigmoid ? 1.f / (1.f + __expf(-l)) : l;
+    se += expf(z - mx);
+  }
+  se = wave_sum(se);
+  float lrow = 0.f, R = 0.f;
+  for (int c = lane; c < C; c += 64) {
+    const float l = zr[c];
+    const float z = input_sigmoid ? 1.f / (1.f + __expf(-l)) : l;
+    const float p = expf(z - mx) / se;
+    lrow += yr[c] * logf(p + 1e-8f);
+    R += yr[c] * p / (p + 1e-8f);
+  }
+  lrow = wave_sum(lrow);
+  R = wave_sum(R);
+  for (int c = lane; c < C; c += 64) {
+    const float l = zr[c];
+    const float s = input_sigmoid ? 1.f / (1.f + __expf(-l)) : l;
+    const float p = expf(s - mx) / se;
+    float g = (p * R - yr[c] * p / (p + 1e-8f)) * invB;
+    if (input_sigmoid) g *= s * (1.f - s);
+    drow[c] = g;
+  }
+  *hit = az == ay;
+  return lrow;
+}
+
 constexpr int CE_NT = 1024;
 __global__ __launch_bounds__(CE_NT) void soft_ce_kernel(const float* __restrict__ logits, const float* __restrict__ y,
                                                         int B, int C, int input_sigmoid, float* loss_out,
@@ -88,51 +139,50 @@
   int hits = 0;
   const float invB = 1.f / (float)B;
   for (int b = wave; b < B; b += CE_NT / 64) {
-    const float* zr = logits + (int64_t)b * C;
-    const float* yr = y + (int64_t)b * C;
-    float mx = -INFINITY, bestz = -INFINITY, besty = -INFINITY;
-    int az = 1 << 30, ay = 1 << 30;
-    for (int c = lane; c < C; c += 64) {
-      const float l = zr[c];
-      const float z = input_sigmoid ? 1.f / (1.f + __expf(-l)) : l;
-      mx = fmaxf(mx, z);
-      if (l > bestz) { bestz = l; az = c; }
-      if (yr[c] > besty) { besty = yr[c]; ay = c; }
-    }
-    mx = wave_max(mx);
-#pragma unroll
-    for (int o = 32; o > 0; o >>= 1) {
-      const float bz = __shfl_xor(bestz, o, 64); const int iz = __shfl_xor(az, o, 64);
-      if (bz > bestz || (bz == bestz && iz < az)) { bestz = bz; az = iz; }
-      const float by = __shfl_xor(besty, o, 64); const int iy = __shfl_xor(ay, o, 64);
-      if (by > besty || (by == besty && iy < ay)) { besty = by; ay = iy; }
-    }
-    float se = 0.f;
-    for (int c = lane; c < C; c += 64) {
-      const float l = zr[c];
-      const float z = input_sigmoid ? 1.f / (1.f + __expf(-l)) : l;
-      se += expf(z - mx);
-    }
-    se = wave_sum(se);
-    float lrow = 0.f, R = 0.f;
-    for (int c = lane; c < C; c += 64) {
-      const float l = zr[c];
-      const float z = input_sigmoid ? 1.f / (1.f + __expf(-l)) : l;
-      const float p = expf(z - mx) / se;
-      lrow += yr[c] * logf(p + 1e-8f);
-      R += yr[c] * p / (p + 1e-8f);
-    }
-    lrow = wave_sum(lrow);
-    R = wave_sum(R);
-    for (int c = lane; c < C; c += 64) {
-      const float l = zr[c];
-      const float s = input_sigmoid ? 1.f / (1.f + __expf(-l)) : l;
-      const float p = expf(s - mx) / se;
-      float g = (p * R - yr[c] * p / (p + 1e-8f)) * invB;
-      if (input_sigmoid) g *= s * (1.f - s);
-      dlogits[(int64_t)b * C + c] = g;
-    }
-    if (lane == 0) { lsum += -(double)lrow; hits += (az == ay); }
+    bool hit;
+    const float lrow = soft_ce_row(logits + (int64_t)b * C, y + (int64_t)b * C, C, input_sigmoid, invB,
+                                   dlogits + (int64_t)b * C, lane, &hit);
+    if (lane == 0) { lsum += -(double)lrow; hits += hit; }
+  }
+  if (lane == 0) { wl[wave] = lsum; wc[wave] = hits; }
+  __syncthreads();
+  if (threadIdx.x == 0) {
+    double tl = 0.0;
+    int tc = 0;
+    for (int w = 0; w < CE_NT / 64; ++w) { tl += wl[w]; tc += wc[w]; }
+    loss_out[0] = (float)(tl / (double)B);
+    if (correct_out) correct_out[0] = tc;
+  }
+}
+
+constexpr int CE_MAXB = 8192;
+__device__ double ce_row_loss[CE_MAXB];
+__device__ int ce_row_hit[CE_MAXB];
+__global__ __launch_bounds__(256) void soft_ce_rows_kernel(const float* __restrict__ logits, const float* __restrict__ y,
+                                                           int B, int C, int input_sigmoid,
+                                                           float* __restrict__ dlogits) {
+  const int lane = threadIdx.x & 63, b = blockIdx.x * 4 + (threadIdx.x >> 6);
+  if (b >= B) return;
+  bool hit;
+  const float lrow = soft_ce_row(logits + (int64_t)b * C, y + (int64_t)b * C, C, input_sigmoid, 1.f / (float)B,
+                                 dlogits + (int64_t)b * C, lane, &hit);
+  if (lane == 0) { ce_row_loss[b] = -(double)lrow; ce_row_hit[b] = hit; }
+}
+__global__ __launch_bounds__(CE_NT) void soft_ce_final_kernel(int B, float* loss_out, int* correct_out) {
+  __shared__ double wl[CE_NT / 64];
+  __shared__ int wc[CE_NT / 64];
+  const int lane = threadIdx.x & 63, wave = threadIdx.x >> 6;
+  double lsum = 0.0;
+  int hits = 0;
+  for (int b0 = 0; wave + 16 * b0 < B; b0 += 64) {
+    const int b = wave + 16 * (b0 + lane);
+    const double v = b < B ? ce_row_loss[b] : 0.0;
+    const int h = b < B ? ce_row_hit[b] : 0;
+    const int nrow = min(64, (B - wave - 16 * b0 + 15) / 16);
+    for (int j = 0; j < nrow; ++j) {
+      lsum += __shfl(v, j, 64);
+      hits += __shfl(h, j, 64);
+    }
   }
   if (lane == 0) { wl[wave] = lsum; wc[wave] = hits; }
   __syncthreads();
@@ -610,7 +660,13 @@
 extern "C" int mia_soft_ce(const float* logits, const float* y, int32_t B, int32_t C, int32_t input_sigmoid, float* loss,
                            float* dlogits, int32_t* correct, mia_stream_t stream) {
   MIA_CHECK_ARG(logits && y && loss && dlogits && B > 0 && C > 0, "soft_ce: args");
-  soft_ce_kernel<<<1, CE_NT, 0, as_stream(stream)>>>(logits, y, B, C, input_sigmoid, loss, dlogits, correct);
+  const char* v1 = getenv("MIA_REDUCE_V1");
+  if ((v1 && v1[0] == '1') || B > CE_MAXB) {
+    soft_ce_kernel<<<1, CE_NT, 0, as_stream(stream)>>>(logits, y, B, C, input_sigmoid, loss, dlogits, correct);
+  } else {
+    soft_ce_rows_kernel<<<(unsigned)cdiv(B, 4), 256, 0, as_stream(stream)>>>(logits, y, B, C, input_sigmoid, dlogits);
+    soft_ce_final_kernel<<<1, CE_NT, 0, as_stream(stream)>>>(B, loss, correct);
+  }
   MIA_LAUNCH_CHECK("soft_ce");
   return 0;
 }
diff --git a/dl-sound-classification_amd/csrc/pool.hip b/dl-sound-classification_amd/csrc/pool.hip
--- a/dl-sound-classification_amd/csrc/pool.hip
+++ b/dl-sound-classification_amd/csrc/pool.hip
@@ -23,10 +23,63 @@
   return (((int64_t)b * C + c) * OH + oy) * OW + ox;
 }
 
+bool pool_v1() { const char* e = getenv("MIA_POOL_V1"); return e && e[0] == '1'; }
+
+__device__ __forceinline__ int xcd_block_id() {
+  const int nwg = gridDim.x, q = nwg / 8, r = nwg % 8, x = blockIdx.x % 8;
+  return (x < r ? x * (q + 1) : r * (q + 1) + (x - r) * q) + blockIdx.x / 8;
+}
+
+template <int KH, int KW>
+__device__ __forceinline__ void pool_window_dt(const void* __restrict__ x, int dtype, int64_t off0, int W, int C,
+                                               int kh, int kw, const float (&sc)[8], const float (&sh)[8],
+                                               float (&best)[8], float (&raw)[8], int (&arg)[8]) {
+#pragma unroll
+  for (int i = 0; i < 8; ++i) { best[i] = -INFINITY; raw[i] = 0.f; arg[i] = 0; }
+  if constexpr (KH > 0) {
+    float f[KH * KW][8];
+#pragma unroll
+    for (int dy = 0; dy < KH; ++dy)
+#pragma unroll
+      for (int dx = 0; dx < KW; ++dx) load8(x, dtype, off0 + ((int64_t)dy * W + dx) * C, f[dy * KW + dx]);
+#pragma unroll
+    for (int pos = 0; pos < KH * KW; ++pos)
+#pragma unroll
+      for (int i = 0; i < 8; ++i) {
+        const float v = fmaxf(fmaf(f[pos][i], sc[i], sh[i]), 0.f);
+        if (v > best[i]) { best[i] = v; raw[i] = f[pos][i]; arg[i] = pos; }
+      }
+  } else {
+    for (int dy = 0; dy < kh; ++dy) {
+      for (int dx = 0; dx < kw; ++dx) {
+        float f[8];
+        load8(x, dtype, off0 + ((int64_t)dy * W + dx) * C, f);
+        const int pos = dy * kw + dx;
+#pragma unroll
+        for (int i = 0; i < 8; ++i) {
+          const float v = fmaxf(fmaf(f[i], sc[i], sh[i]), 0.f);
+          if (v > best[i]) { best[i] = v; raw[i] = f[i]; arg[i] = pos; }
+        }
+      }
+    }
+  }
+}
+
+template <int KH, int KW>
+__device__ __forceinline__ void pool_window(const void* __restrict__ x, int dtype, int64_t off0, int W, int C, int kh,
+                                            int kw, const float (&sc)[8], const float (&sh)[8], float (&best)[8],
+                                            float (&raw)[8], int (&arg)[8]) {
+  if (dtype == MIA_BF16) pool_window_dt<KH, KW>(x, MIA_BF16, off0, W, C, kh, kw, sc, sh, best, raw, arg);
+  else if constexpr (KH * KW <= 4) pool_window_dt<KH, KW>(x, MIA_F32, off0, W, C, kh, kw, sc, sh, best, raw, arg);
+  else pool_window_dt<0, 0>(x, MIA_F32, off0, W, C, kh, kw, sc, sh, best, raw, arg);
+}
+
+template <int KH, int KW>
 __global__ __launch_bounds__(NT) void pool_fwd_kernel(const void* __restrict__ x, int dtype, int n, int H, int W,
                                                       int C, int kh, int kw, const float* __restrict__ scale,
                                                       const float* __restrict__ shift, void* out, int layout,
                                                       uint8_t* __restrict__ argmax, void* __restrict__ win) {
+  if constexpr (KH > 0) { kh = KH; kw = KW; }
   const int OH = H / kh, OW = W / kw, G = C / 8;
   const int total = n * OH * OW * G;
   for (int idx = blockIdx.x * NT + threadIdx.x; idx < total; idx += gridDim.x * NT) {
@@ -42,34 +95,9 @@
     for (int i = 0; i < 8; ++i) {
       sc[i] = scale ? scale[cg * 8 + i] : 1.f;
       sh[i] = shift ? shift[cg * 8 + i] : 0.f;
-      best[i] = -INFINITY;
-      raw[i] = 0.f;
-      arg[i] = 0;
-    }
-    for (int dy = 0; dy < kh; ++dy) {
-      const int iy = oy * kh + dy;
-      for (int dx = 0; dx < kw; ++dx) {
-        const int ix = ox * kw + dx;
-        const int64_t off = (((int64_t)b * H + iy) * W + ix) * C + cg * 8;
-        float f[8];
-        if (dtype == MIA_BF16) {
-          uint4 u = *reinterpret_cast<const uint4*>(reinterpret_cast<const bf16*>(x) + off);
-          uint32_t w4[4] = {u.x, u.y, u.z, u.w};
-#pragma unroll
-          for (int i = 0; i < 4; ++i) { f[2 * i] = __uint_as_float(w4[i] << 16); f[2 * i + 1] = __uint_as_float(w4[i] & 0xffff0000u); }
-        } else {
-          const float4* q = reinterpret_cast<const float4*>(reinterpret_cast<const float*>(x) + off);
-          float4 a = q[0], c4 = q[1];
-          f[0] = a.x; f[1] = a.y; f[2] = a.z; f[3] = a.w; f[4] = c4.x; f[5] = c4.y; f[6] = c4.z; f[7] = c4.w;
-        }
-        const int pos = dy * kw + dx;
-#pragma unroll
-        for (int i = 0; i < 8; ++i) {
-          const float v = fmaxf(fmaf(f[i], sc[i], sh[i]), 0.f);
-          if (v > best[i]) { best[i] = v; raw[i] = f[i]; arg[i] = pos; }
-        }
-      }
-    }
+    }
+    pool_window<KH, KW>(x, dtype, (((int64_t)b * H + oy * kh) * W + ox * kw) * C + cg * 8, W, C, kh, kw, sc, sh, best,
+                        raw, arg);
     const int64_t aoff = (((int64_t)b * OH + oy) * OW + ox) * C + cg * 8;
     uint32_t a0 = 0, a1 = 0;
 #pragma unroll
@@ -81,6 +109,84 @@
     } else {
 #pragma unroll
       for (int i = 0; i < 8; ++i) st_elem(out, dtype, out_index(layout, b, oy, ox, cg * 8 + i, OH, OW, C), best[i]);
+    }
+  }
+}
+
+constexpr int PT = 64;
+template <int KH, int KW>
+__global__ __launch_bounds__(NT) void pool_fwd_tr_kernel(const void* __restrict__ x, int dtype, int H, int W, int C,
+                                                         int kh, int kw, const float* __restrict__ scale,
+                                                         const float* __restrict__ shift, void* out,
+                                                         uint8_t* __restrict__ argmax, void* __restrict__ win) {
+  if constexpr (KH > 0) { kh = KH; kw = KW; }
+  __shared__ __attribute__((aligned(16))) float tile_raw[PT * (PT + 1)];
+  float(*tf)[PT + 1] = reinterpret_cast<float(*)[PT + 1]>(tile_raw);
+  bf16(*tb)[PT + 4] = reinterpret_cast<bf16(*)[PT + 4]>(tile_raw);
+  const int OW = W / kw, S = (H / kh) * OW, G = C / 8;
+  const int chunks = (C + PT - 1) / PT, tiles = (S + PT - 1) / PT;
+  int bi = xcd_block_id();
+  const int chunk = bi % chunks;
+  bi /= chunks;
+  const int b = bi / tiles, p0 = (bi - b * tiles) * PT;
+  const int np = min(PT, S - p0);
+  const int t = threadIdx.x;
+#pragma unroll
+  for (int k = 0; k < PT * PT / 8 / NT; ++k) {
+    const int q = t + NT * k, r = q >> 3, ch = q & 7;
+    const int cg = chunk * (PT / 8) + ch;
+    if (r >= np || cg >= G) continue;
+    const int p = p0 + r, oy = p / OW, ox = p - oy * OW;
+    float sc[8], sh[8], best[8], raw[8];
+    int arg[8];
+#pragma unroll
+    for (int i = 0; i < 8; ++i) {
+      sc[i] = scale ? scale[cg * 8 + i] : 1.f;
+      sh[i] = shift ? shift[cg * 8 + i] : 0.f;
+    }
+    pool_window<KH, KW>(x, dtype, (((int64_t)b * H + oy * kh) * W + ox * kw) * C + cg * 8, W, C, kh, kw, sc, sh, best,
+                        raw, arg);
+    const int64_t aoff = ((int64_t)b * S + p) * C + cg * 8;
+    uint32_t a0 = 0, a1 = 0;
+#pragma unroll
+    for (int i = 0; i < 4; ++i) { a0 |= (uint32_t)arg[i] << (8 * i); a1 |= (uint32_t)arg[i + 4] << (8 * i); }
+    *reinterpret_cast<uint2*>(argmax + aoff) = make_uint2(a0, a1);
+    if (win) store8(win, dtype, aoff, raw);
+#pragma unroll
+    for (int i = 0; i < 8; ++i) {
+      if (dtype == MIA_BF16) tb[ch * 8 + i][r] = (bf16)best[i];
+      else tf[ch * 8 + i][r] = best[i];
+    }
+  }
+  __syncthreads();
+  const int nc = min(PT, C - chunk * PT);
+  const int64_t row0 = ((int64_t)b * C + chunk * PT) * S + p0;
+  if (dtype == MIA_BF16) {
+    bf16* o = reinterpret_cast<bf16*>(out) + row0;
+    constexpr int NJ = PT / 4 + 1;
+    for (int q = t; q < PT * NJ; q += NT) {
+      const int c = q / NJ, j = q - c * NJ;
+      if (c >= nc) break;
+      bf16* dst = o + (int64_t)c * S;
+      const int lead = (int)((reinterpret_cast<uintptr_t>(dst) >> 1) & 3);
+      const int lo = 4 * j - lead;
+      if (lo >= 0 && lo + 4 <= np) {
+        bf16x4 w4;
+#pragma unroll
+        for (int i = 0; i < 4; ++i) w4[i] = tb[c][lo + i];
+        *reinterpret_cast<bf16x4*>(dst + lo) = w4;
+      } else {
+#pragma unroll
+        for (int i = 0; i < 4; ++i)
+          if (lo + i >= 0 && lo + i < np) dst[lo + i] = tb[c][lo + i];
+      }
+    }
+  } else {
+    float* o = reinterpret_cast<float*>(out) + row0;
+    for (int q = t; q < PT * PT; q += NT) {
+      const int c = q >> 6, r = q & (PT - 1);
+      if (c >= nc) break;
+      if (r < np) o[(int64_t)c * S + r] = tf[c][r];
     }
   }
 }
@@ -350,6 +456,114 @@
     float acc = 0.f;
     for (int r2 = 0; r2 < rslots; ++r2) acc += red[(r2 * G + g2) * 16 + qq * 8 + ci];
     partial[((int64_t)blockIdx.x * C + c) * 2 + qq] = acc;
+  }
+}
+
+__global__ __launch_bounds__(NT) void pool_bwd_sparse_tr_kernel(const void* __restrict__ dout,
+                                                                const uint8_t* __restrict__ argmax,
+                                                                const void* __restrict__ x,
+                                                                const void* __restrict__ win, int dtype, int cells,
+                                                                int H, int W, int C, int kh, int kw, int lg_nch,
+                                                                const float* __restrict__ scale,
+                                                                const float* __restrict__ shift,
+                                                                const float* __restrict__ mean,
+                                                                const float* __restrict__ invstd,
+                                                                float* __restrict__ gm, float* __restrict__ partial) {
+  const int OW = W / kw, S = (H / kh) * OW, G = C / 8;
+  const int t = threadIdx.x;
+  const int lb = xcd_block_id();
+  const int cg = t % G, rs = t / G, rslots = NT / G;
+  const int LD = C + 4;
+  __shared__ __attribute__((aligned(16))) float red[NT * 16];
+  float* tile = red;
+  float sc[8], sh[8], mu[8], is[8];
+#pragma unroll
+  for (int i = 0; i < 8; ++i) {
+    sc[i] = scale[cg * 8 + i]; sh[i] = shift[cg * 8 + i]; mu[i] = mean[cg * 8 + i]; is[i] = invstd[cg * 8 + i];
+  }
+  float s1[8] = {0}, s2[8] = {0};
+  const int es = dtype == MIA_BF16 ? 1 : 2;
+  const uintptr_t dbase = reinterpret_cast<uintptr_t>(dout) >> es;
+  int pc[2], pk[2];
+#pragma unroll
+  for (int u = 0; u < 2; ++u) { const int q = t + NT * u; pc[u] = q >> lg_nch; pk[u] = q & ((1 << lg_nch) - 1); }
+  float pv[2][4], wx[8] = {0};
+  auto fetch = [&](int cell0) {
+#pragma unroll
+    for (int u = 0; u < 2; ++u) {
+      const int c0 = cell0 + 4 * pk[u];
+      const int b0 = c0 / S, b3 = (c0 + 3) / S;
+      const int64_t i0 = ((int64_t)b0 * C + pc[u]) * S + (c0 - b0 * S);
+      if (c0 + 3 < cells && b0 == b3 && ((dbase + (uintptr_t)i0) & 3) == 0) {
+        if (dtype == MIA_BF16) {
+          const uint2 v = *reinterpret_cast<const uint2*>(reinterpret_cast<const bf16*>(dout) + i0);
+          pv[u][0] = __uint_as_float(v.x << 16); pv[u][1] = __uint_as_float(v.x & 0xffff0000u);
+          pv[u][2] = __uint_as_float(v.y << 16); pv[u][3] = __uint_as_float(v.y & 0xffff0000u);
+        } else {
+          const float4 v = *reinterpret_cast<const float4*>(reinterpret_cast<const float*>(dout) + i0);
+          pv[u][0] = v.x; pv[u][1] = v.y; pv[u][2] = v.z; pv[u][3] = v.w;
+        }
+      } else {
+#pragma unroll
+        for (int j = 0; j < 4; ++j) {
+          const int cj = c0 + j, bj = cj / S;
+          pv[u][j] = cj < cells ? ld_elem(dout, dtype, ((int64_t)bj * C + pc[u]) * S + (cj - bj * S)) : 0.f;
+        }
+      }
+    }
+    if (win && cell0 + rs < cells) load8(win, dtype, (int64_t)(cell0 + rs) * C + cg * 8, wx);
+  };
+  const int64_t step = (int64_t)gridDim.x * rslots;
+  int64_t cell0 = (int64_t)lb * rslots;
+  if (cell0 < cells) fetch((int)cell0);
+  for (; cell0 < cells; cell0 += step) {
+#pragma unroll
+    for (int u = 0; u < 2; ++u)
+#pragma unroll
+      for (int j = 0; j < 4; ++j) tile[(4 * pk[u] + j) * LD + pc[u]] = pv[u][j];
+    float xv[8];
+#pragma unroll
+    for (int i = 0; i < 8; ++i) xv[i] = wx[i];
+    __syncthreads();
+    if (cell0 + step < cells) fetch((int)(cell0 + step));
+    const int64_t cell = cell0 + rs;
+    if (cell < cells) {
+      const float4 d0 = *reinterpret_cast<const float4*>(tile + rs * LD + cg * 8);
+      const float4 d1 = *reinterpret_cast<const float4*>(tile + rs * LD + cg * 8 + 4);
+      const float dv[8] = {d0.x, d0.y, d0.z, d0.w, d1.x, d1.y, d1.z, d1.w};
+      if (!win) {
+        const int b = (int)cell / S, p = (int)cell - b * S, oy = p / OW, ox = p - oy * OW;
+        const uint2 am = *reinterpret_cast<const uint2*>(argmax + cell * C + cg * 8);
+#pragma unroll
+        for (int i = 0; i < 8; ++i) {
+          const uint32_t word = i < 4 ? am.x : am.y;
+          const int a = (int)((word >> (8 * (i & 3))) & 0xffu);
+          const int iy = oy * kh + a / kw, ix = ox * kw + a % kw;
+          xv[i] = ld_elem(x, dtype, (((int64_t)b * H + iy) * W + ix) * C + cg * 8 + i);
+        }
+      }
+      float gv[8];
+#pragma unroll
+      for (int i = 0; i < 8; ++i) {
+        const float g = fmaf(xv[i], sc[i], sh[i]) > 0.f ? dv[i] : 0.f;
+        gv[i] = g;
+        s1[i] += g;
+        s2[i] = fmaf(g, (xv[i] - mu[i]) * is[i], s2[i]);
+      }
+      float4* gq = reinterpret_cast<float4*>(gm + cell * C + cg * 8);
+      gq[0] = make_float4(gv[0], gv[1], gv[2], gv[3]);
+      gq[1] = make_float4(gv[4], gv[5], gv[6], gv[7]);
+    }
+    __syncthreads();
+  }
+#pragma unroll
+  for (int i = 0; i < 8; ++i) { red[t * 16 + i] = s1[i]; red[t * 16 + 8 + i] = s2[i]; }
+  __syncthreads();
+  for (int e = t; e < 2 * C; e += NT) {
+    const int qq = e / C, c = e % C, g2 = c / 8, ci = c % 8;
+    float acc = 0.f;
+    for (int r2 = 0; r2 < rslots; ++r2) acc += red[(r2 * G + g2) * 16 + qq * 8 + ci];
+    partial[((int64_t)lb * C + c) * 2 + qq] = acc;
   }
 }
 
@@ -663,8 +877,24 @@
   MIA_CHECK_ARG((int64_t)n * h * w * (c / 8) < (1ll << 31), "pool_fwd: too many elements for 32-bit indexing");
   const int64_t total = (int64_t)n * (h / kh) * (w / kw) * (c / 8);
   const int nb = (int)std::min<int64_t>(cdiv(total, NT), 16384);
-  pool_fwd_kernel<<<nb, NT, 0, as_stream(stream)>>>(x, dtype, n, h, w, c, kh, kw, scale, shift, out, out_layout, argmax,
-                                                    win);
+  hipStream_t s = as_stream(stream);
+  const bool v1 = pool_v1();
+  const int win_id = v1 ? 0 : (kh == 1 && kw == 2) ? 1 : (kh == 5 && kw == 3) ? 2 : 0;
+  const int64_t tblocks = (int64_t)n * cdiv((int64_t)(h / kh) * (w / kw), PT) * cdiv(c, PT);
+  if (!v1 && out_layout != 0 && tblocks < (1ll << 31)) {
+    if (win_id == 1)
+      pool_fwd_tr_kernel<1, 2><<<(unsigned)tblocks, NT, 0, s>>>(x, dtype, h, w, c, kh, kw, scale, shift, out, argmax, win);
+    else if (win_id == 2)
+      pool_fwd_tr_kernel<5, 3><<<(unsigned)tblocks, NT, 0, s>>>(x, dtype, h, w, c, kh, kw, scale, shift, out, argmax, win);
+    else
+      pool_fwd_tr_kernel<0, 0><<<(unsigned)tblocks, NT, 0, s>>>(x, dtype, h, w, c, kh, kw, scale, shift, out, argmax, win);
+    MIA_LAUNCH_CHECK("pool_fwd_tr");
+    return 0;
+  }
+  if (win_id == 2)
+    pool_fwd_kernel<5, 3><<<nb, NT, 0, s>>>(x, dtype, n, h, w, c, kh, kw, scale, shift, out, out_layout, argmax, win);
+  else
+    pool_fwd_kernel<0, 0><<<nb, NT, 0, s>>>(x, dtype, n, h, w, c, kh, kw, scale, shift, out, out_layout, argmax, win);
   MIA_LAUNCH_CHECK("pool_fwd");
   return 0;
 }
@@ -739,8 +969,16 @@
   const int nb = (int)std::max<int64_t>(1, std::min<int64_t>(cdiv(cells, (int64_t)rslots * 2), 1024));
   hipStream_t s = as_stream(stream);
   MIA_CHECK_ARG(!win || (reinterpret_cast<uintptr_t>(win) & 15) == 0, "pool_bwd_gather: win alignment");
-  pool_bwd_sparse_kernel<<<nb, NT, 0, s>>>(dout, out_layout, argmax, x, win, dtype, n, h, w, c, kh, kw, scale, shift, mean,
-                                           invstd, gm, (float*)partial);
+  if (!pool_v1() && (out_layout == 2 || (out_layout == 1 && h / kh == 1)) && rslots >= 16 &&
+      cells < (1ll << 31) - 1024) {
+    int lg_nch = 0;
+    while ((4 << lg_nch) < rslots) ++lg_nch;
+    pool_bwd_sparse_tr_kernel<<<nb, NT, 0, s>>>(dout, argmax, x, win, dtype, (int)cells, h, w, c, kh, kw, lg_nch, scale,
+                                                shift, mean, invstd, gm, (float*)partial);
+  } else {
+    pool_bwd_sparse_kernel<<<nb, NT, 0, s>>>(dout, out_layout, argmax, x, win, dtype, n, h, w, c, kh, kw, scale, shift,
+                                             mean, invstd, gm, (float*)partial);
+  }
   MIA_LAUNCH_CHECK("pool_bwd_gather");
   partial_final_kernel<<<(unsigned)c, 256, 0, s>>>((const float*)partial, nb, c, dgamma, dbeta);
   MIA_LAUNCH_CHECK("pool_bwd_gather_final");
```

Measured after the change: 15690 clips/s (median of 6 runs). 1.02x the previous value.
